# marella/ctransformers

Measured on NVIDIA H100. Metric: decode tokens/s Llama-2-7B Q4_K_M b=1, higher is better.
Workload: dtype int8 (q4_K/q6_K weights x q8_K activations, mma.sync u8 x s8 -> exact int32), fp32 combine in the reference's order

## Files before the change

ctransformers_b200/csrc/device_types.cuh:

```cuda
#pragma once
#include <cstdint>
#include <cuda_fp16.h>
#include <cuda_runtime.h>
#include <utility>

namespace ctb {

enum : int { GT_F32 = 0, GT_F16 = 1, GT_Q4_0 = 2, GT_Q4_1 = 3, GT_Q5_0 = 6, GT_Q5_1 = 7, GT_Q8_0 = 8, GT_Q3_K = 11, GT_Q4_K = 12, GT_Q5_K = 13, GT_Q6_K = 14 };

struct DevMat {
  int type = -1;
  int K = 0, M = 0;
  int nb = 0;
  const uint8_t* qs = nullptr;
  const uint8_t* qh = nullptr;
  const uint16_t* mn = nullptr;
  const uint16_t* d = nullptr;
  const uint8_t* st = nullptr;
  size_t bytes = 0;
};

__host__ __device__ inline bool type_is_kquant(int t) { return t == GT_Q3_K || t == GT_Q4_K || t == GT_Q5_K || t == GT_Q6_K; }
enum : int { ACT_Q8_K = 0, ACT_Q8_0 = 1, ACT_F16 = 2, ACT_F32 = 3, ACT_Q8_1 = 4 };
__host__ __device__ inline int act_format_for(int t) {
  if (type_is_kquant(t)) return ACT_Q8_K;
  if (t == GT_Q4_0 || t == GT_Q5_0 || t == GT_Q8_0) return ACT_Q8_0;
  if (t == GT_Q4_1 || t == GT_Q5_1) return ACT_Q8_1;
  if (t == GT_F16) return ACT_F16;
  return ACT_F32;
}

__device__ __forceinline__ float h2f(uint16_t h) { return __half2float(__ushort_as_half(h)); }
__device__ __forceinline__ uint16_t f2h(float f) { return __half_as_ushort(__float2half_rn(f)); }

__device__ __forceinline__ void pdl_trigger() { asm volatile("griddepcontrol.launch_dependents;"); }
__device__ __forceinline__ void pdl_wait() { asm volatile("griddepcontrol.wait;" ::: "memory"); }

template <typename... KArgs, typename... Args>
static inline cudaError_t launch_kernel(void (*kernel)(KArgs...), dim3 grid, dim3 block, size_t smem, cudaStream_t st, bool pdl, Args&&... args) {
  cudaLaunchConfig_t cfg{};
  cfg.gridDim = grid; cfg.blockDim = block; cfg.dynamicSmemBytes = smem; cfg.stream = st;
  cudaLaunchAttribute at[1];
  at[0].id = cudaLaunchAttributeProgrammaticStreamSerialization;
  at[0].val.programmaticStreamSerializationAllowed = 1;
  cfg.attrs = at; cfg.numAttrs = pdl ? 1 : 0;
  return cudaLaunchKernelEx(&cfg, kernel, std::forward<Args>(args)...);
}

template <typename Kernel>
static inline size_t max_dyn_smem(Kernel kernel) {
  cudaFuncAttributes fa{};
  if (cudaFuncGetAttributes(&fa, kernel) != cudaSuccess) return 0;
  int dev = 0, optin = 0;
  cudaGetDevice(&dev);
  cudaDeviceGetAttribute(&optin, cudaDevAttrMaxSharedMemoryPerBlockOptin, dev);
  return (size_t)optin > fa.sharedSizeBytes ? (size_t)optin - fa.sharedSizeBytes : 0;
}

template <int BAR, int NT>
__device__ __forceinline__ void bar_sync() { asm volatile("bar.sync %0, %1;" ::"n"(BAR), "n"(NT) : "memory"); }

__device__ __forceinline__ unsigned long long globaltimer_ns() {
  unsigned long long t;
  asm volatile("mov.u64 %0, %%globaltimer;" : "=l"(t));
  return t;
}

__device__ __forceinline__ float warp_sum(float v) {
#pragma unroll
  for (int o = 16; o > 0; o >>= 1) v += __shfl_xor_sync(0xffffffffu, v, o);
  return v;
}
__device__ __forceinline__ double warp_sum(double v) {
#pragma unroll
  for (int o = 16; o > 0; o >>= 1) v += __shfl_xor_sync(0xffffffffu, v, o);
  return v;
}
__device__ __forceinline__ float warp_max(float v) {
#pragma unroll
  for (int o = 16; o > 0; o >>= 1) v = fmaxf(v, __shfl_xor_sync(0xffffffffu, v, o));
  return v;
}

__host__ __device__ inline bool attn_head_dim_ok(int hd) { return hd >= 32 && hd <= 256 && hd % 2 == 0; }
__host__ __device__ inline bool attn_fast_hd(int hd) { return hd == 64 || hd == 128; }

}
```

ctransformers_b200/csrc/engine.cu:

```cuda
#include "engine.cuh"

#include <algorithm>
#include <chrono>
#include <cstdio>
#include <cstring>
#include <stdexcept>

#include "attention.cuh"
#include "grammar.hpp"
#include "grammar_gpu.cuh"
#include "matvec.cuh"
#include "prefill.cuh"
#include "repack.cuh"
#include "sample_gpu.cuh"
#include "score_gpu.cuh"
#include "stream.cuh"
#include "tables.hpp"
#include "tp_nccl.hpp"

namespace ctb {

#define CTB_CUDA(expr)                                                                                         \
  do {                                                                                                         \
    cudaError_t e__ = (expr);                                                                                  \
// ... 528 lines not shown
        MVParams p{};
        p.x = attn_; p.norm_mode = NORM_NONE; p.K = qw; p.act = act_format_for(L.wo.type); p.nseg = 1;
        p.seg[0] = (!tp || tp_lead) ? seg(L.wo, y, EPI_ADD, x) : seg(L.wo, y);
        push_matvec(p, MVK_WO);
        if (tp) push_xchg(y);
      }
      {
        MVParams p{};
        p.x = y; p.norm_w = L.ffn_norm; p.norm_mode = NORM_RMS; p.eps = hp_.eps; p.K = n_embd;
        const size_t first_op = ops_.size();
        take_input(p);
        p.act = act_format_for(L.w1.type); p.nseg = 2;
        p.seg[0] = seg(L.w1, ffn_, EPI_SILU); p.seg[1] = seg(L.w3, ffn2_);
        push_matvec(p, MVK_UP);
        mark_exchange(first_op);
      }
      {
        MVParams p{};
        p.x = ffn_; p.x2 = ffn2_; p.x_mode = 1; p.norm_mode = NORM_NONE; p.K = nff_; p.act = act_format_for(L.w2.type); p.nseg = 1;
        p.seg[0] = (!tp || tp_lead) ? seg(L.w2, x, EPI_ADD, y) : seg(L.w2, x);
        push_matvec(p, MVK_DOWN);
        if (tp) push_xchg(x);
      }
    } else {
      const int qkv_w = (hp_.n_head + 2 * n_kv) * hd;
      float* q = qkv_; float* k = qkv_ + (size_t)hp_.n_head * hd; float* v = k + (size_t)n_kv * hd;
      const bool two_norms = L.attn_norm2 != nullptr;
      const bool fuse = !two_norms && act_format_for(L.wqkv.type) == act_format_for(L.w3.type);
      {
        MVParams p{};
        p.x = x; p.norm_mode = NORM_LAYER; p.eps = hp_.eps; p.K = n_embd;
        p.norm_w = two_norms ? L.attn_norm2 : L.attn_norm; p.norm_b = two_norms ? L.attn_norm2_b : L.attn_norm_b;
        p.act = act_format_for(L.wqkv.type); p.nseg = 1;
        p.seg[0] = seg(L.wqkv, qkv_);
        if (fuse) { p.seg[1] = seg(L.w3, ffn_, EPI_GELU); p.nseg = 2; }
        ap.q = q; ap.k = k; ap.v = v; ap.q_stride = qkv_w; ap.kv_stride = qkv_w;
        push_matvec(p, MVK_QKV);
      }
      if (!fuse) {
        MVParams p{};
        p.x = x; p.norm_mode = NORM_LAYER; p.eps = hp_.eps; p.K = n_embd; p.norm_w = L.attn_norm; p.norm_b = L.attn_norm_b;
        p.act = act_format_for(L.w3.type); p.nseg = 1;
        p.seg[0] = seg(L.w3, ffn_, EPI_GELU);
        push_matvec(p, MVK_UP);
      }
      push_attn();
      {
        MVParams p{};
        p.x = attn_; p.norm_mode = NORM_NONE; p.K = n_embd; p.act = act_format_for(L.wo.type); p.nseg = 1;
        p.seg[0] = seg(L.wo, attn_o_);
        push_matvec(p, MVK_WO);
      }
      {
        MVParams p{};
        p.x = ffn_; p.norm_mode = NORM_NONE; p.K = hp_.n_ff; p.act = act_format_for(L.w2.type); p.nseg = 1;
        p.seg[0] = seg(L.w2, y, EPI_ADD2, attn_o_, x);
        push_matvec(p, MVK_DOWN);
      }
      std::swap(x, y);
    }
  }
  n_body_ = (int)ops_.size();
  {
    MVParams p{};
    p.x = x; p.norm_w = out_norm_; p.norm_b = out_norm_b_; p.norm_mode = hp_.falcon ? NORM_LAYER : NORM_RMS; p.eps = hp_.eps; p.K = n_embd;
    const size_t first_op = ops_.size();
    take_input(p);
    p.norm_out = d_embd_; p.act = act_format_for(output_.type); p.nseg = 1;
    p.seg[0] = seg(output_, d_logits_);
    push_matvec(p, MVK_OUT);
    mark_exchange(first_op);

  }
  {
    StepOp op{};
    op.ph.kind = PH_PICK;
    op.ph.pk.logits = d_logits_; op.ph.pk.state = d_state_; op.ph.pk.out_tokens = nullptr; op.ph.pk.n = hp_.n_vocab;
    ops_.push_back(op);
  }
  bool any_stream = false;
  for (const StepOp& op : ops_) any_stream |= op.ph.kind == PH_MATVEC && op.stream;
  std::vector<Phase> phs;
  for (const StepOp& op : ops_) if (op.ph.kind != PH_XCHG && (op.ph.kind != PH_MATVEC || op.stream)) phs.push_back(op.ph);
  const StepLaunch sl = step_launch_shape(phs.data(), (int)phs.size(), sm_count_, max_dyn_smem(k_step<true, false, false>));
  step_grid_ = sl.grid; step_slots_ = sl.n_slots; step_smem_ = sl.smem; step_q3_ = sl.q3;
  if (const char* e = getenv("CTB_ST_SLOTS")) {
    const int want = atoi(e);
    if (want >= ST_W && want < step_slots_ && want % ST_W == 0) { step_smem_ -= (size_t)(step_slots_ - want) * ST_SLOT; step_slots_ = want; }
  }
  ring_attn_ = st_attn_ring_ok(hp_.n_ctx, step_slots_) && !getenv("CTB_NO_RING_ATTN");
  for (StepOp& op : ops_) if (op.ph.kind == PH_ATTN) op.ph.q6 = ring_attn_ ? 1 : 0;
  if (any_stream && step_slots_ < ST_W) throw std::runtime_error("model rows are too long for the step kernel's shared memory");
  if (any_stream) CTB_CUDA(step_set_smem_limit(step_smem_));
  else fused_ = false;
  d_prog_ = (Phase*)alloc((ops_.size() + 1) * sizeof(Phase), 256);
  d_prog_mv_ = (Phase*)alloc((ops_.size() + 1) * sizeof(Phase), 256);
  d_bounds_ = (int*)alloc((ops_.size() + 1) * (size_t)(sm_count_ + 1) * 4, 256);
  d_bounds_mv_ = (int*)alloc((ops_.size() + 1) * (size_t)(sm_count_ + 1) * 4, 256);
}

void Engine::upload_prog(Phase* dst, int* dst_bounds, const std::vector<StepOp>& ops) {
  std::vector<Phase> phs(ops.size());
  for (size_t i = 0; i < ops.size(); i++) phs[i] = ops[i].ph;
  CTB_CUDA(cudaMemcpy(dst, phs.data(), phs.size() * sizeof(Phase), cudaMemcpyHostToDevice));
  std::vector<Phase> run = phs;
  for (size_t i = 0; i < ops.size(); i++) if (ops[i].ph.kind == PH_XCHG || (ops[i].ph.kind == PH_MATVEC && !ops[i].stream)) run[i].kind = -1;
  const std::vector<int> b = step_bounds(run.data(), (int)run.size(), sm_count_);
  CTB_CUDA(cudaMemcpy(dst_bounds, b.data(), b.size() * 4, cudaMemcpyHostToDevice));
}

struct ProfMark {
  Event ev;
  int kind;
};

long Engine::enqueue_ops(const std::vector<StepOp>& ops, const Phase* d_prog, const int* d_bounds, int n, cudaStream_t st, bool fused,
                         std::vector<ProfMark>* marks) {
  long launches = 0;
  auto mark = [&](int kind) {
    if (!marks) return;
    marks->push_back({Event(cudaEventDefault), kind});
    CTB_CUDA(cudaEventRecord(marks->back().ev, st));
  };
  StepLaunch step_shape_;
  step_shape_.grid = step_grid_; step_shape_.n_slots = step_slots_; step_shape_.smem = step_smem_; step_shape_.gen = !attn_fast_hd(hp_.head_dim());
  step_shape_.q3 = step_q3_;
  auto capable = [&](const StepOp& op) { return op.ph.kind != PH_XCHG && (op.ph.kind != PH_MATVEC || op.stream); };
  int i = 0;
  while (i < n) {
    const StepOp& op = ops[i];
    if (fused && capable(op)) {
      int j = i;
      while (j < n && capable(ops[j])) j++;
      mark(-1);
      CTB_CUDA(launch_step(step_shape_, st, d_prog + i, d_bounds + (size_t)i * (sm_count_ + 1), j - i, d_sync_, false, nullptr, tp_peer_));
      launches++;
      mark(0);
      i = j;
      continue;
    }
    mark(-1);
    switch (op.ph.kind) {
      case PH_EMBED:
        k_embed<<<1, 256, 0, st>>>(op.ph.em);
        launches++;
        mark(3);
        break;
      case PH_ATTN:
        CTB_CUDA(launch_kernel(attn_kernel(hp_.head_dim()), dim3(nh_, 1, attn_groups(hp_.head_dim())), dim3(ATTN_THREADS), attn_smem_bytes(hp_.n_ctx, hp_.head_dim()), st, pdl_, op.ph.at));
        launches++;
        mark(1);
        break;
      case PH_XCHG:
        tp_all_reduce(op.ph.em.out, op.ph.em.K, st);
        mark(3);
        break;
      case PH_PICK:
        k_argmax<<<1, ARGMAX_THREADS, 0, st>>>(d_logits_, hp_.n_vocab, d_state_ + 4);
        k_advance<<<1, 1, 0, st>>>(d_state_, d_tokens_out_.as<int>());
        launches += 2;
        mark(3);
        break;
      default:
        if (op.stream) {
          CTB_CUDA(launch_step(step_shape_, st, d_prog + i, d_bounds + (size_t)i * (sm_count_ + 1), 1, d_sync_));
        } else {
          const MVLaunch L = matvec_launch_shape(op.ph.mv, sm_count_);
          CTB_CUDA(launch_matvec_kernel(L, st, op.ph.mv, pdl_));
        }
        launches++;
        mark(0);
    }
    i++;
  }
  CTB_CUDA(cudaGetLastError());
  return launches;
}

int Engine::profile_step(int token, int n_past, double ms_by_kind[4], int count_by_kind[4]) {
  DeviceGuard dev_guard(device_);
  if (tp_.world > 1) throw std::runtime_error("not available in tensor-parallel mode (every rank must run the same launches)");
  drop_lookahead();
  put_step(token, n_past, n_past + 1);
  std::vector<ProfMark> marks;
  enqueue_ops(ops_, d_prog_, d_bounds_, n_body_ + 1, stream_, false, &marks);
  CTB_CUDA(cudaStreamSynchronize(stream_));
  int n = 0;
  for (size_t i = 1; i < marks.size(); i++) {
    float ms = 0;
    cudaEventElapsedTime(&ms, marks[i - 1].ev, marks[i].ev);
    const int k = marks[i].kind;
    if (k >= 0 && k < 4) { ms_by_kind[k] += ms; count_by_kind[k]++; n++; }
  }
  return n;
}

double Engine::time_matvec_only(int reps, long* launches, unsigned mask) {
  if (!mask) mask = ~0u;
  if (tp_.world > 1) throw std::runtime_error("not available in tensor-parallel mode (every rank must run the same launches)");
  drop_lookahead();
  DeviceGuard dev_guard(device_);
  std::vector<StepOp> sel;
  for (int i = 0; i <= n_body_; i++)
    if (ops_[i].ph.kind == PH_MATVEC && ((mask >> ops_[i].mvk) & 1)) sel.push_back(ops_[i]);
  if (sel.empty()) { if (launches) *launches = 0; return 0.0; }
  upload_prog(d_prog_mv_, d_bounds_mv_, sel);
  GraphExec ex;
  {
    const Stream cap(cudaStreamNonBlocking);
    cudaGraph_t g;
    CTB_CUDA(cudaStreamBeginCapture(cap, cudaStreamCaptureModeThreadLocal));
    enqueue_ops(sel, d_prog_mv_, d_bounds_mv_, (int)sel.size(), cap, fused_);
    CTB_CUDA(cudaStreamEndCapture(cap, &g));
    ex = GraphExec(g);
    cudaGraphDestroy(g);
  }
  if (launches) *launches = (long)sel.size();
  const Event e0(cudaEventDefault), e1(cudaEventDefault);
  for (int i = 0; i < 3; i++) CTB_CUDA(cudaGraphLaunch(ex, stream_));
  CTB_CUDA(cudaEventRecord(e0, stream_));
  for (int i = 0; i < reps; i++) CTB_CUDA(cudaGraphLaunch(ex, stream_));
  CTB_CUDA(cudaEventRecord(e1, stream_));
  CTB_CUDA(cudaStreamSynchronize(stream_));
  float ms = 0;
  cudaEventElapsedTime(&ms, e0, e1);
  return (double)ms / reps;
}

long Engine::trace_step(int token, int n_past, unsigned long long* out, long cap_words) {
  DeviceGuard dev_guard(device_);
  if (tp_.world > 1) throw std::runtime_error("not available in tensor-parallel mode (every rank must run the same launches)");
  drop_lookahead();
  const int n = n_body_ + 1;
  for (int i = 0; i < n; i++)
    if (ops_[i].ph.kind == PH_MATVEC && !ops_[i].stream) return 0;
  const long need = 2L * n + 8L * n * step_grid_;
  if (need > cap_words) return -need;
  const DevMem buf((size_t)n * step_grid_ * 64);
  CTB_CUDA(cudaMemset(buf.get(), 0, (size_t)n * step_grid_ * 64));
  StepLaunch L;
  L.grid = step_grid_; L.n_slots = step_slots_; L.smem = step_smem_; L.gen = !attn_fast_hd(hp_.head_dim()); L.q3 = step_q3_;
  for (int rep = 0; rep < 3; rep++) {
    put_step(token, n_past, n_past + 1);
    CTB_CUDA(launch_step(L, stream_, d_prog_, d_bounds_, n, d_sync_, false, buf.as<unsigned long long>()));
    CTB_CUDA(cudaStreamSynchronize(stream_));
  }
  for (int i = 0; i < n; i++) { out[2 * i] = (unsigned long long)ops_[i].ph.kind; out[2 * i + 1] = (unsigned long long)ops_[i].mvk; }
  CTB_CUDA(cudaMemcpy(out + 2 * n, buf.get(), (size_t)n * step_grid_ * 64, cudaMemcpyDeviceToHost));
  return n;
}

void Engine::build_graphs() {
  tokens_out_cap_ = std::max(hp_.n_ctx, 4096);
  d_tokens_out_ = DevMem((size_t)tokens_out_cap_ * 4);
  h_tokens_out_ = HostMem((size_t)tokens_out_cap_ * 4);
  const Stream cap(cudaStreamNonBlocking);
  ops_.back().ph.pk.out_tokens = d_tokens_out_.as<int>();
  upload_prog(d_prog_, d_bounds_, ops_);
  long launches = 0;
  auto capture = [&](bool logits, bool greedy) {
    cudaGraph_t g;
    CTB_CUDA(cudaStreamBeginCapture(cap, cudaStreamCaptureModeThreadLocal));
    launches = enqueue_ops(ops_, d_prog_, d_bounds_, n_body_ + (logits || tp_peer_ ? 1 : 0) + (greedy ? 1 : 0), cap, fused_);
    CTB_CUDA(cudaStreamEndCapture(cap, &g));
    GraphExec ex(g);
    cudaGraphDestroy(g);
    return ex;
  };
  graph_nolog_ = capture(false, false);
  graph_greedy_ = capture(true, true);
  graph_full_ = capture(true, false);
  stats.launches = launches;
}

void Engine::after_eval(int next_pos) {
  spec_pending_ = false;
  spec_deferred_ = false;
  spec_pos_ = -1;
  if (!spec_on_ || next_pos >= hp_.n_ctx || next_pos < kv_high_) return;
  k_argmax<<<1, ARGMAX_THREADS, 0, stream_>>>(d_logits_, hp_.n_vocab, d_state_ + 4);
  k_advance<<<1, 1, 0, stream_>>>(d_state_, d_tokens_out_.as<int>());
  CTB_CUDA(cudaMemcpyAsync(h_spec_tok_.get(), d_state_ + 4, 8, cudaMemcpyDeviceToHost, stream_));
  CTB_CUDA(cudaEventRecord(ev_pick_, stream_));
  spec_pos_ = next_pos;
  if (spec_streak_ >= 2) {
    if (sampler_mode_) spec_deferred_ = true;
    else {
      CTB_CUDA(cudaGraphLaunch(graph_full_, stream_));
      spec_pending_ = true;
    }
  }
}

void Engine::drop_lookahead() { spec_pending_ = false; spec_deferred_ = false; spec_pos_ = -1; spec_streak_ = 0; }

void Engine::launch_deferred_spec() {
  if (!spec_deferred_) return;
  spec_deferred_ = false;
  CTB_CUDA(cudaGraphLaunch(graph_full_, stream_));
  spec_pending_ = true;
}

int Engine::greedy_pick() {
  if (spec_pos_ < 0) return -1;
  DeviceGuard dev_guard(device_);
  CTB_CUDA(cudaEventSynchronize(ev_pick_));
  sampler_mode_ = false;
  launch_deferred_spec();
  const int* pick = h_spec_tok_.as<int>();
  return pick[1] == 1 ? pick[0] : -1;
}

void Engine::put_step(int token, int pos, int n_total) {
  CTB_CUDA(step_ring_.put(stream_, 4, [&](int* st) { st[0] = token; st[1] = pos; st[2] = 0; st[3] = n_total; }));
}

void Engine::decode_one(int token, int pos, int n_total, bool with_logits) {
  put_step(token, pos, n_total);
  CTB_CUDA(cudaGraphLaunch(with_logits ? graph_full_ : graph_nolog_, stream_));
  single_steps_++;
}

int Engine::paths(int* out, int cap) {
  const int v[6] = {fused_ ? 1 : 0, fused_ && ring_attn_ ? 1 : 0, step_slots_, ensure_prefill() ? 1 : 0, (int)prefill_launches_, (int)single_steps_};
// ... 705 lines not shown
```

ctransformers_b200/csrc/engine.cuh:

```cuda
#pragma once
#include <cmath>
#include <memory>
#include <string>
#include <vector>

#include "cuda_owned.cuh"
#include "device_types.cuh"
#include "gguf.hpp"

namespace ctb {

struct TPShard {
  int rank = 0, world = 1;
  int head0 = 0, head1 = 0, kv0 = 0, kv1 = 0, ff0 = 0, ff1 = 0;
  void* comm = nullptr;
};
TPShard tp_shard(int n_embd, int n_head, int n_head_kv, int n_ff, int rank, int world);

struct HParams {
  bool falcon = false;
  int n_vocab = 0, n_ctx_train = 0, n_embd = 0, n_ff = 0, n_head = 0, n_head_kv = 0, n_layer = 0, n_rot = 0;
  float eps = 1e-5f, rope_base = 10000.f, rope_scale = 1.f;
  int n_ctx = 512;
  int n_seq = 1;
  bool multi = false;
  int head_dim() const { return n_embd / n_head; }
  int n_embd_gqa() const { return head_dim() * n_head_kv; }
};

struct LayerW {
  DevMat wq, wk, wv, wqkv, wo, w1, w2, w3;
  const float* attn_norm = nullptr; const float* attn_norm_b = nullptr;
  const float* attn_norm2 = nullptr; const float* attn_norm2_b = nullptr;
  const float* ffn_norm = nullptr;
};

struct Phase;
struct StepOp;
struct ProfMark;
struct MVParams;
struct Uploader;
struct PrefillState;

struct MultiTok { int slot, token, pos, n_total; bool last; };
constexpr int MULTI_LAUNCH_TOKENS = 32;

struct SampleRow { int slot; const int* last; int n_last; float penalty; int k; };

struct Grammar;
struct GrammarState;
struct GrammarRow { int slot; const Grammar* g; const GrammarState* s; const int* last; int n_last; float penalty; int k; };

struct RowSink {
  float* host = nullptr;
  const int* targets = nullptr;
  double* logprob = nullptr;
  int* greedy = nullptr;
};

struct KvCopy { int src, dst, lo, hi; };

struct EvalStats { double last_eval_ms = 0; long launches = 0; size_t weight_bytes_per_token = 0; long spec_hits = 0; double load_ms = 0; size_t load_bytes = 0; };

class Engine {
 public:
  Engine(const GGUFFile& g, const HParams& hp, int device, const TPShard& tp = TPShard());
  ~Engine();
  Engine(const Engine&) = delete;
  Engine& operator=(const Engine&) = delete;

  void eval_list(const int* tokens, const int* pos, const int* n_total, int n, const RowSink* rows = nullptr);
  void score_kept(int target, double* logprob, int* greedy);
  double decode_greedy(int first_token, int n_past, int n_steps, int* out_tokens);
  double time_matvec_only(int reps, long* launches, unsigned mask = 0);
  int profile_step(int token, int n_past, double ms_by_kind[4], int count_by_kind[4]);
  long trace_step(int token, int n_past, unsigned long long* out, long cap_words);
  std::string multi_refusal();
  void multi_eval(const std::vector<MultiTok>& toks, const std::vector<int>& starts, const RowSink* rows = nullptr);
  void multi_fetch(int slot, float* logits, float* embd);
  const struct SampleGpuOut* multi_sample(const SampleRow* rows, int R, int* picks);
  void multi_reset(int slot);
  long multi_launches() const;
  size_t state_bytes(int n_past, bool results) const;
  int state_k_stride() const;
  void state_save(int slot, int n_past, bool results, void* out);
  void state_load(int slot, int n_past, bool results, const void* in, int last_token);
  void state_fork(int src, const int* dsts, int n);
  size_t kv_reparent(const std::vector<KvCopy>& copies);
  const float* multi_rows(int slot0, int n);
  int paths(int* out, int cap);

  float* logits() { host_views(); return h_logits_.as<float>(); }
  float* embeddings() { host_views(); return h_embd_.as<float>(); }
  bool lazy_logits() const { return !eager_; }
  std::vector<float> logits_copy();
  int topk_candidates(const int* last, int n_last, float penalty, int k, int* ids, float* logits);
  int greedy_pick();
  bool has_grammar_pieces() const { return pieces_ready_; }
  void grammar_pieces(const std::vector<int>& off, const std::vector<uint8_t>& bytes);
  const struct SampleGpuOut* grammar_rows(const GrammarRow* rows, int R, int eos, int* stats, unsigned* bits = nullptr);
  std::vector<std::vector<float>> grammar_scratch(const std::vector<int>& rows);
  std::vector<float> slot_logits(int slot);
  const HParams& hparams() const { return hp_; }
  EvalStats stats;
  void set_stream(cudaStream_t s);
  cudaStream_t stream() const { return stream_; }

 private:
  Engine(const HParams& hp, int device, const TPShard& tp);
  HParams hp_;
  TPShard tp_;
  int nh_ = 0, nkv_ = 0, nff_ = 0;
  void tp_all_reduce(float* buf, int n, cudaStream_t st);
  bool tp_peer_ = false;
  uint8_t* xc_region_ = nullptr;
  uint2* xc_ll_[8] = {nullptr};
  void tp_setup_peer();
  int device_ = 0;
  Stream stream_;
  DevMem arena_;
  size_t arena_size_ = 0, arena_used_ = 0;
  void* alloc(size_t bytes, size_t align = 256);

  DevMat output_;
  const uint8_t* tok_embd_ = nullptr; int tok_type_ = 0; size_t tok_row_bytes_ = 0;
  const float* out_norm_ = nullptr; const float* out_norm_b_ = nullptr;
  std::vector<LayerW> layers_;
  uint16_t *silu_tab_ = nullptr, *gelu_tab_ = nullptr, *exp_tab_ = nullptr;
  float2* rope_ = nullptr;
  uint16_t *kc_ = nullptr, *vc_ = nullptr;
  int* d_state_ = nullptr;
  float *xa_ = nullptr, *xb_ = nullptr, *qkv_ = nullptr, *attn_ = nullptr, *attn_o_ = nullptr, *ffn_ = nullptr, *ffn2_ = nullptr, *d_logits_ = nullptr, *d_embd_ = nullptr;
  float *kept_logits_ = nullptr, *kept_embd_ = nullptr;
  int* kept_pick_ = nullptr;
  float* kept_logits(int slot) const { return kept_logits_ + (size_t)slot * hp_.n_vocab; }
  float* kept_embd(int slot) const { return kept_embd_ + (size_t)slot * hp_.n_embd; }
  HostMem h_logits_, h_embd_;
  StateRing step_ring_;
  void put_step(int token, int pos, int n_total);
  HostMem h_tokens_out_;
  DevMem d_tokens_out_;
  int tokens_out_cap_ = 0;

  Event ev0_, ev1_, ev_pick_;
  bool spec_on_ = true, spec_pending_ = false;
  bool spec_deferred_ = false;
  bool sampler_mode_ = false;
  Event ev_sample_;
  void launch_deferred_spec();
  int spec_pos_ = -1, spec_streak_ = 0;
  void drop_lookahead();
  int kv_high_ = 0;
  HostMem h_spec_tok_;
  HostMem h_dbg_;
  void after_eval(int next_pos);
  int sm_count_ = 132;

  void init(const GGUFFile& g);
  DevMat upload_matrix(const GGUFTensor& t, struct Uploader& up, int want_K, int want_M, int row0 = 0, int row1 = -1, int k0 = 0, int k1 = -1);
  const float* upload_vector(const GGUFFile& g, const std::string& name, bool required, int want_n);
  std::vector<StepOp> ops_;
  int n_body_ = 0;
  Phase* d_prog_ = nullptr;
  Phase* d_prog_mv_ = nullptr;
  int *d_bounds_ = nullptr, *d_bounds_mv_ = nullptr;
  unsigned* d_sync_ = nullptr;
  int step_grid_ = 0, step_slots_ = 0;
  size_t step_smem_ = 0;
  bool fused_ = true;
  bool step_q3_ = false;
  bool ring_attn_ = false;
  void build_ops();
  void push_matvec(struct MVParams& p, int kind);
  void upload_prog(Phase* dst, int* dst_bounds, const std::vector<StepOp>& ops);
  long enqueue_ops(const std::vector<StepOp>& ops, const Phase* d_prog, const int* d_bounds, int n, cudaStream_t st, bool fused,
                   std::vector<ProfMark>* marks = nullptr);
  void build_graphs();
  bool eager_ = false;
  bool host_fresh_ = true;
  void host_views();
  DevMem d_sample_;
  HostMem h_sample_;
  void sample_enqueue(const SampleRow* rows, int R, bool picks);
  bool pieces_ready_ = false;
  DevMem d_pieces_, d_gm_, d_gm_rows_;
  HostMem h_gm_;
  std::unique_ptr<PrefillState> pf_;
  bool multi_ready();
  void need_multi();
  bool prefill_on_ = true;
  int prefill_min_ = 4;
  long prefill_launches_ = 0;
  long single_steps_ = 0;
  bool ensure_prefill();
  void prefill_batch(const int* tokens, const int* pos, const int* n_total, int n, bool last, bool rows = false);
  void launch_batch(const MultiTok* toks, int n, bool whole);
  const RowSink* sink_ = nullptr;
  DevMem d_rows_;
  int rows_pending_ = 0, rows_done_ = 0;
  int rows_n_ = 0;
  DevMem d_score_;
  HostMem h_score_;
  int score_cap_ = 0;
  double* d_lp_ = nullptr;
  int *d_tgt_ = nullptr, *d_gr_ = nullptr;
  struct SinkGuard { Engine* e; ~SinkGuard() { e->sink_ = nullptr; } };
  SinkGuard rows_begin(const RowSink* rows, int n);
  void rows_finish();
  void rows_take(const float* src, int m);
  void rows_push(const float* row);
  void rows_drain();
  void rows_end();
  void decode_one(int token, int pos, int n_total, bool with_logits);
  void head_from(const float* row);
  void finish_eval(int next_pos, bool hit);
  enum : int { MVK_QKV = 0, MVK_WO = 1, MVK_UP = 2, MVK_DOWN = 3, MVK_OUT = 4 };
  bool pdl_ = true;
  HostMem h_stage_;
  DevMem d_copies_;
  HostMem h_copies_;
  void kv_slot_elems(size_t& k, size_t& v) const;
  void zero_slot(int slot);
  void copy_results(int src, int dst);
  GraphExec graph_full_, graph_nolog_, graph_greedy_;
};

size_t engine_arena_bytes(const GGUFFile& g, const HParams& hp);

}
```

ctransformers_b200/csrc/llm_abi.cu:

```cuda
#include <algorithm>
#include <atomic>
#include <cctype>
#include <cmath>
#include <chrono>
#include <cstdio>
#include <cstring>
#include <ctime>
#include <memory>
#include <random>
#include <string>
#include <vector>

#include "../../include/ctransformers_b200.h"
#include "beam.hpp"
#include "engine.cuh"
#include "gguf.hpp"
#include "grammar.hpp"
#include "sample_gpu.cuh"
#include "sampler.hpp"
#include "tp_nccl.hpp"
#include "vocab.hpp"

using namespace ctb;

// ... 337 lines not shown
int ctransformers_llm_bos_token_id(LLM* llm) { return llm->vocab.bos; }
int ctransformers_llm_vocab_size(LLM* llm) { return llm->hp.n_vocab; }
int ctransformers_llm_context_length(LLM* llm) { return llm->hp.n_ctx; }
const char* ctransformers_llm_architecture(LLM* llm) { return llm->arch.c_str(); }

bool ctransformers_llm_batch_eval(LLM* llm, const int* tokens, const int n_tokens, const int n_past, const int batch_size, const int threads) {
  (void)threads;
  return llm_eval(llm, tokens, n_tokens, n_past, batch_size, nullptr, "eval") == 0;
}

float* ctransformers_llm_logits_data(LLM* llm) { return llm->engine->logits(); }
int ctransformers_llm_logits_size(LLM* llm) { return llm->has_logits ? llm->hp.n_vocab : 0; }
const float* ctransformers_llm_embeddings_data(LLM* llm) { return llm->engine->embeddings(); }
int ctransformers_llm_embeddings_size(LLM* llm) { return llm->has_logits ? llm->hp.n_embd : 0; }

int ctransformers_llm_sample(LLM* llm, const int* last_tokens, const int n_last, const int top_k, const float top_p, const float temperature,
                             const float repetition_penalty, int seed) {
  try {
    if (seed < 0) seed = (int)time(nullptr);
    llm->rng.seed((unsigned)seed);
    if (llm->engine->lazy_logits()) {
      Engine& e = *llm->engine;
      bool used_device = false;
      const int t = sample_lazy(
          llm->hp.n_vocab, last_tokens, n_last, top_k, top_p, temperature, repetition_penalty, llm->rng, used_device, [&] { return e.greedy_pick(); },
          [&](const int* last, int nl, float pen, int k, int* ids, float* lg) { return e.topk_candidates(last, nl, pen, k, ids, lg); },
          [&] { return e.logits_copy(); });
      if (used_device) llm->gpu_samples++;
      return t;
    }
    return sample_token(llm->engine->logits(), llm->hp.n_vocab, last_tokens, n_last, top_k, top_p, temperature, repetition_penalty, llm->rng);
  } catch (...) { return llm->vocab.eos; }
}

void ctransformers_llm_reset(LLM* llm) { (void)llm;  }

int ctb_abi_version(void) { return 1; }

double ctb_llm_last_eval_ms(LLM* llm) { return llm->engine->stats.last_eval_ms; }
long ctb_llm_launches_per_token(LLM* llm) { return llm->engine->stats.launches; }
long ctb_llm_speculative_hits(LLM* llm) { return llm->engine->stats.spec_hits; }
unsigned long long ctb_llm_weight_bytes_per_token(LLM* llm) { return (unsigned long long)llm->engine->stats.weight_bytes_per_token; }
long ctb_llm_device_samples(LLM* llm) { return llm->gpu_samples; }
double ctb_llm_load_ms(LLM* llm) { return llm->engine->stats.load_ms; }
void ctb_llm_set_stream(LLM* llm, void* cuda_stream) { llm->engine->set_stream((cudaStream_t)cuda_stream); }

double ctb_llm_decode_greedy(LLM* llm, int first_token, int n_past, int n_steps, int* out_tokens) {
  try {
    const double ms = llm->engine->decode_greedy(first_token, n_past, n_steps, out_tokens);
    llm->has_logits = true;
    return ms;
  } catch (const std::exception& e) {
    fprintf(stderr, "ctransformers-b200: decode_greedy failed: %s\n", e.what());
    return -1.0;
  }
}

int ctb_llm_profile_step(LLM* llm, int token, int n_past, double* ms_by_kind, int* count_by_kind) {
  try {
    return llm->engine->profile_step(token, n_past, ms_by_kind, count_by_kind);
  } catch (const std::exception& e) {
    fprintf(stderr, "ctransformers-b200: profile_step failed: %s\n", e.what());
    return -1;
  }
}

long ctb_llm_trace_step(LLM* llm, int token, int n_past, unsigned long long* out, long cap_words) {
  try {
    return llm->engine->trace_step(token, n_past, out, cap_words);
  } catch (const std::exception& e) {
    fprintf(stderr, "ctransformers-b200: trace_step failed: %s\n", e.what());
    return 0;
  }
}

long ctb_llm_paths(LLM* llm, int* out, int cap) {
  try {
    return llm->engine->paths(out, cap);
  } catch (const std::exception& e) {
    fprintf(stderr, "ctransformers-b200: paths failed: %s\n", e.what());
    return -100;
  }
}

double ctb_llm_time_matvec_only(LLM* llm, int reps, long* launches) { return ctb_llm_time_matvec_kinds(llm, reps, launches, 0); }

double ctb_llm_time_matvec_kinds(LLM* llm, int reps, long* launches, unsigned kind_mask) {
  try {
    return llm->engine->time_matvec_only(reps < 1 ? 1 : reps, launches, kind_mask);
  } catch (const std::exception& e) {
    fprintf(stderr, "ctransformers-b200: time_matvec_only failed: %s\n", e.what());
    return -1.0;
  }
}

int ctb_state_info(const void* buf, size_t size, ctb_state_header* out) {
  ctb_state_header s;
  const std::string why = state_check(buf, size, s);
  if (!why.empty()) {
    fprintf(stderr, "ctransformers-b200: %s\n", why.c_str());
    return -1;
  }
  if (out) *out = s;
  return 0;
}

size_t ctb_llm_state_size(LLM* llm, int n_tokens) {
  try {
    not_sharded(llm, "has no sequence states");
    return state_size_for(*llm, n_tokens);
  } catch (...) { return 0; }
}

int ctb_llm_save_state(LLM* llm, const int* tokens, int n_tokens, void* buf, size_t cap) {
  try {
    not_sharded(llm, "has no sequence states");
    save_state(*llm, 0, tokens, n_tokens, llm->has_logits, buf, cap);
    return 0;
  } catch (const std::exception& e) { return state_error("cannot save the state", e); }
}

int ctb_llm_load_state(LLM* llm, const void* buf, size_t size) {
  try {
    not_sharded(llm, "has no sequence states");
    llm->has_logits = restore_state(*llm, 0, buf, size).has_results != 0;
    return 0;
  } catch (const std::exception& e) { return state_error("cannot load the state", e); }
}

int ctb_llm_batch_eval_rows(LLM* llm, const int* tokens, int n_tokens, int n_past, int batch_size, float* rows) {
  RowSink s;
  s.host = rows;
  return llm_eval(llm, tokens, n_tokens, n_past, batch_size, &s, "eval with rows");
}

int ctb_llm_batch_eval_scored(LLM* llm, const int* tokens, int n_tokens, int n_past, int batch_size, const int* targets, double* logprob, int* greedy) {
  RowSink s;
  s.targets = targets; s.logprob = logprob; s.greedy = greedy;
  if (n_tokens > 0 && (!logprob || !greedy)) {
    fprintf(stderr, "ctransformers-b200: scored eval failed: no memory for the scores\n");
    return -1;
  }
  return llm_eval(llm, tokens, n_tokens, n_past, batch_size, &s, "scored eval");
}

int ctb_llm_score_last(LLM* llm, int target, double* logprob, int* greedy) {
  try {
    not_sharded(llm, "keeps no per-token rows");
    if (!llm->has_logits) throw std::invalid_argument("nothing has been evaluated");
    check_targets(&target, 1, llm->hp.n_vocab);
    llm->engine->score_kept(target, logprob, greedy);
    return 0;
  } catch (const std::exception& e) {
    fprintf(stderr, "ctransformers-b200: scoring the last logits failed: %s\n", e.what());
    return -1;
  } catch (...) { return -1; }
}

struct ctb_vocab { std::unique_ptr<GGUFFile> file; Vocab vocab; };

ctb_vocab* ctb_vocab_load(const char* gguf_path) {
  try {
    std::unique_ptr<ctb_vocab> v(new ctb_vocab);
    v->file.reset(new GGUFFile(gguf_path));
    v->vocab.load(*v->file);
    return v.release();
// ... 825 lines not shown
```

ctransformers_b200/csrc/matvec.cuh:

```cuda
#pragma once
#include "device_types.cuh"
#include "attention.cuh"

namespace ctb {

#ifndef CTB_THREADS
#define CTB_THREADS 512
#endif
constexpr int MV_THREADS = CTB_THREADS;
constexpr int MV_WARPS = MV_THREADS / 32;
constexpr int MV_ROWS = 4;
constexpr int MV_MAX_SEG = 3;

enum : int { NORM_NONE = 0, NORM_RMS = 1, NORM_LAYER = 2 };
enum : int { EPI_STORE = 0, EPI_ADD = 1, EPI_GELU = 2, EPI_ADD2 = 3, EPI_SILU = 4 };

#ifndef ST_WATCHDOG_NS
#define ST_WATCHDOG_NS 4000000000ull
#endif
#ifndef XC_WATCHDOG_NS
#define XC_WATCHDOG_NS 30000000000ull
#endif
enum WaitCode : int {
  W_GRID_BARRIER = 1, W_FOLD_FLAG, W_FREE_WEIGHT_SLOT, W_WEIGHT_ITEM, W_FREE_K_SLOT, W_FREE_V_SLOT, W_K_ITEM, W_V_ITEM, W_XCHG,
  W_PF_GRID_BARRIER, W_PF_FREE_SLOT, W_PF_WEIGHT_ITEM, W_CODES
};
constexpr const char* WAIT_TEXT[] = {"?", "grid barrier (aux = phase)", "fold hand-off flag (aux = chunk)", "producer: free weight slot (aux = item)",
                                     "consumer: weight item (aux = item)", "producer: free K slot (attention)", "producer: free V slot (attention)",
                                     "consumer: K item (attention)", "consumer: V item (attention)", "tensor-parallel exchange: a peer's element (aux = exchange number)",
                                     "prefill grid barrier (aux = phase)", "prefill producer: free slot (aux = item)", "prefill consumer: weight item (aux = item)"};
static_assert(sizeof(WAIT_TEXT) / sizeof(WAIT_TEXT[0]) == W_CODES, "one text per wait code");

static __device__ int* g_st_dbg = nullptr;
static __device__ __noinline__ void st_fail(WaitCode code, int aux) {
  int* d = g_st_dbg;
  if (d) { d[0] = code; d[1] = (int)blockIdx.x; d[2] = aux; d[3] = (int)threadIdx.x; __threadfence_system(); }
  __trap();
}
template <typename Done>
__device__ __forceinline__ void bounded_wait(Done&& done, WaitCode code, int aux, unsigned long long limit_ns = ST_WATCHDOG_NS) {
  if (done()) return;
  const unsigned long long t0 = globaltimer_ns();
  while (!done())
    if (globaltimer_ns() - t0 > limit_ns) st_fail(code, aux);
}

struct MVSeg {
  DevMat w;
  float* out;
  const float* res;
  const float* res2;
  int epi;
};

struct MVParams {
  const float* x;
  const float* x2;
  int x_mode;
  int x_parts, x_stride;
  float* sum_out;
  const float* norm_w;
  const float* norm_b;
  float* norm_out;
  float eps;
  int norm_mode;
  int K;
  int act;
  int nseg;
  MVSeg seg[MV_MAX_SEG];
  const uint16_t* silu_tab;
  const uint16_t* gelu_tab;
};

struct ActView {
  const int8_t* qs;
  const float* d;
  const int16_t* bs;
};

__host__ __device__ inline size_t act_smem_bytes(int act, int K) {
  switch (act) {
    case ACT_Q8_K: return (size_t)K + (((size_t)(K / 256) * 4 + 15) & ~(size_t)15) + (size_t)(K / 16) * 2 + 16;
    case ACT_Q8_0: return (size_t)K + (size_t)(K / 32) * 4 + 16;
    case ACT_Q8_1: return (size_t)K + (size_t)(K / 32) * 8 + 16;
    case ACT_F16: return (size_t)K * 2;
    default: return (size_t)K * 4;
  }
}

__host__ __device__ inline size_t q8k_d_bytes(int K) { return ((size_t)(K / 256) * 4 + 15) & ~(size_t)15; }

__device__ __forceinline__ ActView act_view(int act, int K, uint8_t* smem) {
  ActView a;
  a.qs = (const int8_t*)smem;
  const size_t off = ((size_t)K + 15) & ~(size_t)15;
  a.d = (const float*)(smem + off);
  a.bs = (const int16_t*)(smem + off + q8k_d_bytes(K));
  return a;
}

__device__ __forceinline__ int q8k_word_offset(int b, int s, int l) { return ((b * 2 + (s >> 2)) * 8 + l) * 16 + (s & 3) * 4; }


template <bool CG = false>
__device__ __forceinline__ void load16(const float* p, int valid, float (&v)[16]) {
  if (valid >= 16) {
    float4 a, b, c, d;
    if (CG) { a = __ldcg((const float4*)p); b = __ldcg((const float4*)p + 1); c = __ldcg((const float4*)p + 2); d = __ldcg((const float4*)p + 3); }
    else { a = __ldg((const float4*)p); b = __ldg((const float4*)p + 1); c = __ldg((const float4*)p + 2); d = __ldg((const float4*)p + 3); }
    v[0] = a.x; v[1] = a.y; v[2] = a.z; v[3] = a.w; v[4] = b.x; v[5] = b.y; v[6] = b.z; v[7] = b.w;
    v[8] = c.x; v[9] = c.y; v[10] = c.z; v[11] = c.w; v[12] = d.x; v[13] = d.y; v[14] = d.z; v[15] = d.w;
  } else {
#pragma unroll
    for (int e = 0; e < 16; e++) v[e] = e < valid ? (CG ? __ldcg(p + e) : __ldg(p + e)) : 0.f;
  }
}

template <int NT, int BAR>
__device__ __forceinline__ double block_sum_f64(double s, double* red ) {
  s = warp_sum(s);
  bar_sync<BAR, NT>();
  if ((threadIdx.x & 31) == 0) red[threadIdx.x >> 5] = s;
  bar_sync<BAR, NT>();
  double t = 0.0;
#pragma unroll
  for (int w = 0; w < NT / 32; w++) t += red[w];
  return t;
}
template <int NT, int BAR>
__device__ __forceinline__ void block_sum2_max_f64(double& s, double& a, double& g, double* red) {
  constexpr int NW = NT / 32;
#pragma unroll
  for (int o = 16; o > 0; o >>= 1) {
    s += __shfl_xor_sync(0xffffffffu, s, o);
    a += __shfl_xor_sync(0xffffffffu, a, o);
    g = fmax(g, __shfl_xor_sync(0xffffffffu, g, o));
  }
  bar_sync<BAR, NT>();
  if ((threadIdx.x & 31) == 0) { red[threadIdx.x >> 5] = s; red[NW + (threadIdx.x >> 5)] = a; red[2 * NW + (threadIdx.x >> 5)] = g; }
  bar_sync<BAR, NT>();
  s = 0.0;
  a = 0.0;
#pragma unroll
  for (int w = 0; w < NW; w++) { s += red[w]; a += red[NW + w]; g = fmax(g, red[2 * NW + w]); }
}

__device__ __forceinline__ uint32_t pack4(const int* q) {
  return (uint32_t)(q[0] & 0xff) | ((uint32_t)(q[1] & 0xff) << 8) | ((uint32_t)(q[2] & 0xff) << 16) | ((uint32_t)(q[3] & 0xff) << 24);
}

__device__ __forceinline__ void load16_ll(const uint2* p, unsigned epoch, float (&u)[16]) {
  uint4 q[8];
  bounded_wait([&] {
    bool ok = true;
#pragma unroll
    for (int j = 0; j < 8; j++) {
      asm volatile("ld.volatile.global.v4.u32 {%0,%1,%2,%3}, [%4];" : "=r"(q[j].x), "=r"(q[j].y), "=r"(q[j].z), "=r"(q[j].w) : "l"(p + 2 * j) : "memory");
    }
#pragma unroll
    for (int j = 0; j < 8; j++) ok &= q[j].y == epoch && q[j].w == epoch;
    return ok;
  }, W_XCHG, (int)epoch, XC_WATCHDOG_NS);
#pragma unroll
  for (int j = 0; j < 8; j++) { u[2 * j] = __uint_as_float(q[j].x); u[2 * j + 1] = __uint_as_float(q[j].z); }
}

template <bool XC = false>
__device__ __forceinline__ void load16x(const MVParams& xs, int base, int valid, float (&v)[16], unsigned epoch = 0) {
  if (XC && xs.x_mode == 2) {
    if (valid <= 0) {
#pragma unroll
      for (int e = 0; e < 16; e++) v[e] = 0.f;
      return;
    }
    const uint2* ll = (const uint2*)xs.x + (size_t)(epoch & 1u) * xs.x_parts * xs.x_stride;
    load16_ll(ll + base, epoch, v);
    for (int r = 1; r < xs.x_parts; r++) {
      float u[16];
      load16_ll(ll + (size_t)r * xs.x_stride + base, epoch, u);
#pragma unroll
      for (int e = 0; e < 16; e++) v[e] = __fadd_rn(v[e], u[e]);
    }
    return;
  }
  load16<true>(xs.x + base, valid, v);
  if (xs.x_mode == 1) {
    float u[16];
    load16<true>(xs.x2 + base, valid, u);
#pragma unroll
    for (int e = 0; e < 16; e++) v[e] = __fmul_rn(v[e], u[e]);
  }
}

struct NormPre { float w0[16], bias0[16]; };
__device__ __forceinline__ void preload_norm(NormPre& np, const MVParams& p) {
  const int t = threadIdx.x;
  if (p.norm_mode != NORM_NONE && p.norm_w) load16(p.norm_w + t * 16, p.K - t * 16, np.w0);
  if (p.norm_mode != NORM_NONE && p.norm_b) load16(p.norm_b + t * 16, p.K - t * 16, np.bias0);
}

__device__ __forceinline__ unsigned min_exp(unsigned emin, float t) {
  const unsigned bits = __float_as_uint(t) & 0x7fffffffu;
  return bits ? min(emin, max(bits >> 23, 1u)) : emin;
}
__device__ __forceinline__ double lsb_inv(unsigned emin) { return ldexp(1.0, 150 - (int)emin); }

enum : int { NORM_TERM_SQ = 0, NORM_TERM_X = 1, NORM_TERM_DEV = 2 };
template <bool XC>
static __device__ __noinline__ double seq_sum_warp0(const float* x, const float* x2, int x_mode, int x_parts, int x_stride, int K, int kind,
                                                    float mean, unsigned epoch) {
  MVParams xs;
  xs.x = x; xs.x2 = x2; xs.x_mode = x_mode; xs.x_parts = x_parts; xs.x_stride = x_stride;
  const int lane = threadIdx.x & 31;
  double seq = 0.0;
  for (int base = 0; base < K; base += 512) {
    float v[16];
    load16x<XC>(xs, base + lane * 16, K - base - lane * 16, v, epoch);
    for (int l = 0; l < 32; l++)
#pragma unroll
      for (int i = 0; i < 16; i++) {
        float t = __shfl_sync(0xffffffffu, v[i], l);
        if (kind == NORM_TERM_DEV) t = __fsub_rn(t, mean);
        if (base + l * 16 + i < K) seq += kind == NORM_TERM_X ? (double)t : (double)__fmul_rn(t, t);
      }
  }
  return seq;
}

template <int NT, int BAR, bool XC>
__device__ __forceinline__ float norm_stat(double s, double a, double g, bool a_is_s, int kind, float mean, const MVParams& xs, double* red,
                                           unsigned epoch) {
  const int K = xs.K;
  if (a_is_s) a = s = block_sum_f64<NT, BAR>(s, red);
  else block_sum2_max_f64<NT, BAR>(s, a, g, red);
  if (!isfinite(s) || (!a_is_s && __dmul_ru(a, g) < 0x1p52)) return (float)(s / (double)K);
  const double e = __dmul_ru(a, (double)K * 0x1.0000001p-52);
  const float lo = (float)(__dsub_rd(s, e) / (double)K), hi = (float)(__dadd_ru(s, e) / (double)K);
  if (lo == hi) return lo;
  const double seq = threadIdx.x < 32 ? seq_sum_warp0<XC>(xs.x, xs.x2, xs.x_mode, xs.x_parts, xs.x_stride, K, kind, mean, epoch) : 0.0;
  bar_sync<BAR, NT>();
  if (threadIdx.x == 0) red[0] = seq;
  bar_sync<BAR, NT>();
  return (float)(red[0] / (double)K);
}

template <int NT, int BAR, bool XC = false>
__device__ __forceinline__ void stage_activation(const MVParams& xs, const NormPre& np, int act, uint8_t* smem, double* red, bool write_norm, unsigned epoch = 0) {
  const float* nw = xs.norm_w;
  const float* nb_ = xs.norm_b;
  float* norm_out = xs.norm_out;
  const int norm_mode = xs.norm_mode, K = xs.K;
  const float eps = xs.eps;
  const int t = threadIdx.x, lane = t & 31;
  const int passes = (K + NT * 16 - 1) / (NT * 16);
  float mean = 0.f, scale = 1.f;
  float v0[16];
  load16x<XC>(xs, t * 16, K - t * 16, v0, epoch);
  if (norm_mode == NORM_RMS) {
    double ss = 0.0;
    for (int ps = 0; ps < passes; ps++) {
      const int base = (ps * NT + t) * 16;
      if ((base & ~511) >= K) continue;
      float v[16];
      if (ps == 0) {
#pragma unroll
        for (int e = 0; e < 16; e++) v[e] = v0[e];
      } else load16x<XC>(xs, base, K - base, v, epoch);
#pragma unroll
      for (int e = 0; e < 16; e++) ss += (double)__fmul_rn(v[e], v[e]);
    }
    const float m = norm_stat<NT, BAR, XC>(ss, ss, 0.0, true, NORM_TERM_SQ, 0.f, xs, red, epoch);
    scale = __fdiv_rn(1.0f, __fsqrt_rn(__fadd_rn(m, eps)));
  } else if (norm_mode == NORM_LAYER) {
    double s1 = 0.0, a1 = 0.0;
    unsigned emin = 255;
    for (int ps = 0; ps < passes; ps++) {
      const int base = (ps * NT + t) * 16;
      if ((base & ~511) >= K) continue;
      float v[16];
      load16x<XC>(xs, base, K - base, v, epoch);
#pragma unroll
      for (int e = 0; e < 16; e++) {
        s1 += (double)v[e];
        a1 += (double)fabsf(v[e]);
        emin = min_exp(emin, v[e]);
      }
    }
    mean = norm_stat<NT, BAR, XC>(s1, a1, lsb_inv(emin), false, NORM_TERM_X, 0.f, xs, red, epoch);
    double s2 = 0.0;
    for (int ps = 0; ps < passes; ps++) {
      const int base = (ps * NT + t) * 16;
      if ((base & ~511) >= K) continue;
      float v[16];
      load16x<XC>(xs, base, K - base, v, epoch);
#pragma unroll
      for (int e = 0; e < 16; e++) { const float d = (base + e < K) ? __fsub_rn(v[e], mean) : 0.f; s2 += (double)__fmul_rn(d, d); }
    }
    const float var = norm_stat<NT, BAR, XC>(s2, s2, 0.0, true, NORM_TERM_DEV, mean, xs, red, epoch);
    scale = __fdiv_rn(1.0f, __fsqrt_rn(__fadd_rn(var, eps)));
  }
  int8_t* qs = (int8_t*)smem;
  const size_t off = ((size_t)K + 15) & ~(size_t)15;
  float* dd = (float*)(smem + off);
  int16_t* bs = (int16_t*)(smem + off + q8k_d_bytes(K));
  for (int ps = 0; ps < passes; ps++) {
    const int base = (ps * NT + t) * 16;
    const int valid = K - base;
    if ((base & ~511) >= K) continue;
    float v[16];
    if (ps == 0) {
#pragma unroll
      for (int e = 0; e < 16; e++) v[e] = v0[e];
    } else load16x<XC>(xs, base, valid, v, epoch);
    if (XC && write_norm && xs.x_mode == 2 && xs.sum_out && valid > 0) {
#pragma unroll
      for (int e = 0; e < 16; e++) if (e < valid) xs.sum_out[base + e] = v[e];
    }
    if (norm_mode != NORM_NONE) {
      float w[16], bb[16];
      if (ps == 0) {
#pragma unroll
        for (int e = 0; e < 16; e++) { w[e] = np.w0[e]; bb[e] = np.bias0[e]; }
      } else {
        if (nw) load16(nw + base, valid, w);
        if (nb_) load16(nb_ + base, valid, bb);
      }
#pragma unroll
      for (int e = 0; e < 16; e++) {
        float y = v[e];
        if (norm_mode == NORM_LAYER) y = __fsub_rn(y, mean);
        y = __fmul_rn(y, scale);
        if (nw) y = __fmul_rn(y, w[e]);
        if (nb_) y = __fadd_rn(y, bb[e]);
        v[e] = y;
      }
    }
    if (write_norm && norm_out && valid > 0) {
#pragma unroll
      for (int e = 0; e < 16; e++) if (e < valid) norm_out[base + e] = v[e];
    }
    if (act == ACT_Q8_K) {
      float amax = 0.f, mx = 0.f;
#pragma unroll
      for (int e = 0; e < 16; e++) { const float ax = fabsf(v[e]); if (ax > amax) { amax = ax; mx = v[e]; } }
      float gmax = amax;
#pragma unroll
      for (int o = 8; o > 0; o >>= 1) gmax = fmaxf(gmax, __shfl_xor_sync(0xffffffffu, gmax, o));
      const unsigned who = __ballot_sync(0xffffffffu, amax == gmax);
      const int hbase = lane & 16, hl = lane & 15;
      const unsigned mine = (who >> hbase) & 0xffffu;
      const float maxv = __shfl_sync(0xffffffffu, mx, hbase + __ffs(mine) - 1);
      if (valid > 0) {
        const int b = base >> 8;
        int q[16];
        int sum = 0;
        if (gmax == 0.f) {
#pragma unroll
          for (int e = 0; e < 16; e++) q[e] = 0;
          if (hl == 0) dd[b] = 0.f;
        } else {
          const float iscale = __fdiv_rn(-128.f, maxv);
#pragma unroll
          for (int e = 0; e < 16; e++) {
            const float val = __fmaf_rn(iscale, v[e], 12582912.f);
            q[e] = min(127, (__float_as_int(val) & 0x007fffff) - 0x00400000);
            sum += q[e];
          }
          if (hl == 0) dd[b] = __fdiv_rn(1.f, iscale);
        }
        bs[b * 16 + hl] = (int16_t)sum;
#pragma unroll
        for (int j = 0; j < 4; j++) {
          const int wi = hl * 4 + j;
          *(uint32_t*)(qs + q8k_word_offset(b, wi >> 3, wi & 7)) = pack4(q + 4 * j);
        }
      }
    } else if (act == ACT_Q8_0) {
      float amax = 0.f;
#pragma unroll
      for (int e = 0; e < 16; e++) amax = fmaxf(amax, fabsf(v[e]));
      amax = fmaxf(amax, __shfl_xor_sync(0xffffffffu, amax, 1));
      if (valid > 0) {
        const float d = __fdiv_rn(amax, 127.f);
        const float id = amax != 0.f ? __fdiv_rn(127.f, amax) : 0.f;
        int q[16];
#pragma unroll
        for (int e = 0; e < 16; e++) q[e] = __float2int_rn(__fmul_rn(v[e], id));
        *(uint4*)(qs + base) = make_uint4(pack4(q), pack4(q + 4), pack4(q + 8), pack4(q + 12));
        if ((lane & 1) == 0) dd[base >> 5] = h2f(f2h(d));
      }
    } else if (act == ACT_Q8_1) {
      float amax = 0.f;
#pragma unroll
      for (int e = 0; e < 16; e++) amax = fmaxf(amax, fabsf(v[e]));
      amax = fmaxf(amax, __shfl_xor_sync(0xffffffffu, amax, 1));
      const float d = __fdiv_rn(amax, 127.f);
      const float id = amax != 0.f ? __fdiv_rn(127.f, amax) : 0.f;
      int q[16];
      int sum = 0;
#pragma unroll
      for (int e = 0; e < 16; e++) { q[e] = __float2int_rn(__fmul_rn(v[e], id)); sum += q[e]; }
      sum += __shfl_xor_sync(0xffffffffu, sum, 1);
      if (valid > 0) {
        *(uint4*)(qs + base) = make_uint4(pack4(q), pack4(q + 4), pack4(q + 8), pack4(q + 12));
        if ((lane & 1) == 0) *(float2*)(dd + (base >> 4)) = make_float2(d, __fmul_rn(d, (float)sum));
      }
    } else if (act == ACT_F16) {
      uint16_t* h = (uint16_t*)smem;
#pragma unroll
      for (int e = 0; e < 16; e++) if (e < valid) h[base + e] = f2h(v[e]);
    } else {
      float* f = (float*)smem;
#pragma unroll
      for (int e = 0; e < 16; e++) if (e < valid) f[base + e] = v[e];
    }
  }
  bar_sync<BAR, NT>();
}

__device__ __forceinline__ float group_hsum8(float v) {
  v = v + __shfl_xor_sync(0xffffffffu, v, 4);
  v = v + __shfl_xor_sync(0xffffffffu, v, 2);
  v = v + __shfl_xor_sync(0xffffffffu, v, 1);
  return v;
}

__device__ __forceinline__ float dot_q40(const DevMat& w, int row, const ActView& a, int l) {
  const int nb = w.nb;
  const uint8_t* qrow = w.qs + (size_t)row * nb * 16 + (l & 3) * 4;
  const uint16_t* drow = w.d + (size_t)row * nb;
  const int shift = (l >> 2) * 4;
  float acc = 0.f;
#pragma unroll 8
  for (int b = 0; b < nb; b++) {
    const uint32_t q = (uint32_t)__ldg((const int*)(qrow + (size_t)b * 16));
    const float dw = h2f(__ldg(drow + b));
    const int aw = *(const int*)(a.qs + b * 32 + l * 4);
    const float yd = a.d[b];
    const uint32_t nib = (q >> shift) & 0x0f0f0f0fu;
    const uint32_t bx = ((nib | 0x80808080u) - 0x08080808u) ^ 0x80808080u;
    acc = __fmaf_rn(__fmul_rn(dw, yd), (float)__dp4a((int)bx, aw, 0), acc);
  }
  return group_hsum8(acc);
}

__device__ __forceinline__ float dot_q50(const DevMat& w, int row, const ActView& a, int l) {
  const int nb = w.nb;
  const uint8_t* qrow = w.qs + (size_t)row * nb * 16 + (l & 3) * 4;
  const uint32_t* hrow = (const uint32_t*)w.qh + (size_t)row * nb;
  const uint16_t* drow = w.d + (size_t)row * nb;
  const int shift = (l >> 2) * 4;
  float acc = 0.f;
#pragma unroll 8
  for (int b = 0; b < nb; b++) {
    const uint32_t q = (uint32_t)__ldg((const int*)(qrow + (size_t)b * 16));
    const uint32_t h4 = (__ldg(hrow + b) >> (4 * l)) & 0xfu;
    const float dw = h2f(__ldg(drow + b));
    const int aw = *(const int*)(a.qs + b * 32 + l * 4);
    const float yd = a.d[b];
    const uint32_t nib = (q >> shift) & 0x0f0f0f0fu;
    const uint32_t set = (h4 * 0x00204081u) & 0x01010101u;
    const uint32_t bx = nib | ((set ^ 0x01010101u) * 0xf0u);
    acc = __fmaf_rn(__fmul_rn(dw, yd), (float)__dp4a((int)bx, aw, 0), acc);
  }
  return group_hsum8(acc);
}

__device__ __forceinline__ float dot_q80(const DevMat& w, int row, const ActView& a, int l) {
  const int nb = w.nb;
  const uint8_t* qrow = w.qs + (size_t)row * nb * 32 + l * 4;
  const uint16_t* drow = w.d + (size_t)row * nb;
  float acc = 0.f;
#pragma unroll 8
  for (int b = 0; b < nb; b++) {
    const int q = __ldg((const int*)(qrow + (size_t)b * 32));
    const float dw = h2f(__ldg(drow + b));
    const int aw = *(const int*)(a.qs + b * 32 + l * 4);
    acc = __fmaf_rn(__fmul_rn(dw, a.d[b]), (float)__dp4a(q, aw, 0), acc);
  }
  return group_hsum8(acc);
}

template <bool Q5>
__device__ __forceinline__ float dot_q1(const DevMat& w, int row, const ActView& a, int l) {
  const int nb = w.nb;
  const uint8_t* qrow = w.qs + (size_t)row * nb * 16 + (l & 3) * 4;
  const uint32_t* hrow = (const uint32_t*)w.qh + (size_t)row * nb;
  const uint16_t* drow = w.d + (size_t)row * nb;
  const uint16_t* mrow = w.mn + (size_t)row * nb;
  const int shift = (l >> 2) * 4;
  float acc = 0.f, summs = 0.f;
#pragma unroll 8
  for (int b = 0; b < nb; b++) {
    const uint32_t q = (uint32_t)__ldg((const int*)(qrow + (size_t)b * 16));
    const float dw = h2f(__ldg(drow + b));
    const float mw = h2f(__ldg(mrow + b));
    const int aw = *(const int*)(a.qs + b * 32 + l * 4);
    const float2 ds = *(const float2*)(a.d + 2 * b);
    uint32_t bx = (q >> shift) & 0x0f0f0f0fu;
    if (Q5) bx |= ((((__ldg(hrow + b) >> (4 * l)) & 0xfu) * 0x00204081u) & 0x01010101u) << 4;
// ... 111 lines not shown
```

ctransformers_b200/csrc/ops_abi.cu:

```cuda
#include <cmath>
#include <cstdio>
#include <cstring>
#include <ctime>
#include <functional>
#include <stdexcept>
#include <string>
#include <vector>

#include "../../include/ctransformers_b200.h"
#include "attention.cuh"
#include "cuda_owned.cuh"
#include "matvec.cuh"
#include "prefill.cuh"
#include "repack.cuh"
#include "sample_gpu.cuh"
#include "sampler.hpp"
#include "score_gpu.cuh"
#include "stream.cuh"
#include "tables.hpp"

using namespace ctb;

namespace {

#define OPS_CUDA(expr)                                                                                     \
  do {                                                                                                     \
    cudaError_t e__ = (expr);                                                                              \
    if (e__ != cudaSuccess) throw std::runtime_error(std::string("CUDA error: ") + cudaGetErrorString(e__) + " (" #expr ")"); \
  } while (0)

struct OpsTables {
  uint16_t *silu = nullptr, *gelu = nullptr, *ex = nullptr;
};

OpsTables& tables() {
  static OpsTables t;
  if (!t.silu) {
    const HostTables h = host_tables();
    OPS_CUDA(cudaMalloc(&t.silu, 65536 * 2)); OPS_CUDA(cudaMalloc(&t.gelu, 65536 * 2)); OPS_CUDA(cudaMalloc(&t.ex, 65536 * 2));
    OPS_CUDA(cudaMemcpy(t.silu, h.silu.data(), 65536 * 2, cudaMemcpyHostToDevice));
    OPS_CUDA(cudaMemcpy(t.gelu, h.gelu.data(), 65536 * 2, cudaMemcpyHostToDevice));
    OPS_CUDA(cudaMemcpy(t.ex, h.ex.data(), 65536 * 2, cudaMemcpyHostToDevice));
  }
  return t;
}

size_t raw_row_bytes(int type, int K) {
  switch (type) {
    case GT_F32: return (size_t)K * 4; case GT_F16: return (size_t)K * 2;
    case GT_Q4_0: return (size_t)K / 32 * 18; case GT_Q5_0: return (size_t)K / 32 * 22; case GT_Q8_0: return (size_t)K / 32 * 34;
    case GT_Q4_1: return (size_t)K / 32 * 20; case GT_Q5_1: return (size_t)K / 32 * 24;
    case GT_Q3_K: return (size_t)K / 256 * 110;
    case GT_Q4_K: return (size_t)K / 256 * 144; case GT_Q5_K: return (size_t)K / 256 * 176; case GT_Q6_K: return (size_t)K / 256 * 210;
  }
  throw std::runtime_error("unsupported ggml type " + std::to_string(type));
}
int block_elems(int type) {
  if (type_is_kquant(type)) return 256;
  return (type == GT_Q4_0 || type == GT_Q5_0 || type == GT_Q8_0 || type == GT_Q4_1 || type == GT_Q5_1) ? 32 : 1;
}

DevMat upload(std::vector<DevMem>& keep, int type, const void* blocks, int K, int M) {
  if (K % block_elems(type)) throw std::runtime_error("K is not a multiple of the block size");
  const size_t bytes = raw_row_bytes(type, K) * M;
  DevMem raw(bytes);
  OPS_CUDA(cudaMemcpy(raw.get(), blocks, bytes, cudaMemcpyHostToDevice));
  DevMat m;
  m.type = type; m.K = K; m.M = M; m.nb = K / block_elems(type); m.bytes = bytes;
  if (type_is_kquant(type)) {
    const size_t sb = st_matrix_bytes(type, M, m.nb);
    keep.emplace_back(sb);
    uint16_t* st = keep.back().as<uint16_t>();
    k_repack_stream<<<(int)std::min<size_t>((sb / 2 + 255) / 256, 4096), 256>>>(type, raw.as<uint8_t>(), M, m.nb, st);
    OPS_CUDA(cudaDeviceSynchronize());
    m.st = (const uint8_t*)st;
    return m;
  }
  const PlaneSizes ps = plane_sizes(type, M, m.nb, bytes);
  uint16_t* pl[4] = {nullptr, nullptr, nullptr, nullptr};
  const size_t sz[4] = {ps.qs, ps.qh, ps.d, ps.mn};
  for (int i = 0; i < 4; i++)
    if (sz[i]) { keep.emplace_back(sz[i]); pl[i] = keep.back().as<uint16_t>(); }
  k_repack<<<(int)std::min<size_t>((bytes / 2 + 255) / 256, 4096), 256>>>(type, raw.as<uint16_t>(), bytes / 2, pl[0], pl[1], pl[2], pl[3]);
  OPS_CUDA(cudaDeviceSynchronize());
  m.qs = (const uint8_t*)pl[0]; m.qh = (const uint8_t*)pl[1]; m.d = pl[2]; m.mn = pl[3];
  return m;
}

int sm_count() {
  int n_sm = 132;
  cudaDeviceGetAttribute(&n_sm, cudaDevAttrMultiProcessorCount, 0);
  return n_sm;
}

unsigned* sync_words() {
  static unsigned* d_sync = nullptr;
  if (!d_sync) { OPS_CUDA(cudaMalloc((void**)&d_sync, 64)); OPS_CUDA(cudaMemset(d_sync, 0, 64)); }
  return d_sync;
}

void run_phases(std::vector<Phase> phs) {
  unsigned* d_sync = sync_words();
  const StepLaunch L = step_launch_shape(phs.data(), (int)phs.size(), sm_count(), max_dyn_smem(k_step<true, false, false>));
  const std::vector<int> hb = step_bounds(phs.data(), (int)phs.size(), L.grid);
  DevMem dbounds(hb.size() * 4);
  OPS_CUDA(cudaMemcpy(dbounds.get(), hb.data(), hb.size() * 4, cudaMemcpyHostToDevice));
  if (L.n_slots < ST_W) throw std::runtime_error("rows too long for the step kernel's shared memory");
  OPS_CUDA(step_set_smem_limit(L.smem));
  DevMem dprog((phs.size() + 1) * sizeof(Phase));
  OPS_CUDA(cudaMemcpy(dprog.get(), phs.data(), phs.size() * sizeof(Phase), cudaMemcpyHostToDevice));
  OPS_CUDA(launch_step(L, 0, dprog.as<Phase>(), dbounds.as<int>(), (int)phs.size(), d_sync));
  OPS_CUDA(cudaGetLastError());
  OPS_CUDA(cudaDeviceSynchronize());
}

void run_matvec(MVParams& p) {
  p.silu_tab = tables().silu;
  p.gelu_tab = tables().gelu;
  if (step_supports(p)) {
    run_phases({matvec_phase(p)});
    return;
  }
  static bool attr = false;
  if (!attr) {
    OPS_CUDA(matvec_set_smem_limit(MV_SMEM_LIMIT));
    attr = true;
  }
  const MVLaunch L = matvec_launch_shape(p, sm_count());
  OPS_CUDA(launch_matvec_kernel(L, 0, p));
  OPS_CUDA(cudaGetLastError());
}

__global__ void __launch_bounds__(MV_THREADS) k_stage_dump(const __grid_constant__ MVParams q, int act, uint8_t* dump) {
  extern __shared__ __align__(16) uint8_t smem[];
  __shared__ double red[3 * MV_WARPS];
  NormPre np;
  preload_norm(np, q);
  stage_activation<MV_THREADS, 0>(q, np, act, smem, red, true);
  const size_t n = act_smem_bytes(act, q.K);
  for (size_t i = threadIdx.x; i < n; i += MV_THREADS) dump[i] = smem[i];
}

__global__ void __launch_bounds__(MV_THREADS) k_gate_dump(const __grid_constant__ MVParams q, float* out) {
  extern __shared__ __align__(16) uint8_t smem[];
  __shared__ double red[3 * MV_WARPS];
  NormPre np;
  preload_norm(np, q);
  stage_activation<MV_THREADS, 0>(q, np, ACT_F32, smem, red, false);
  const float* f = (const float*)smem;
  for (int i = threadIdx.x; i < q.K; i += MV_THREADS) out[i] = f[i];
}

__global__ void k_rope_dump(float* x, const float2* rope, int pos, int hd, int neox) {
  float* row = x + (size_t)blockIdx.x * hd;
  int i0, i1;
  float o0, o1;
  rope_head_pair(row, threadIdx.x, hd, neox, rope[(size_t)pos * (hd / 2) + threadIdx.x], i0, i1, o0, o1);
  row[i0] = o0; row[i1] = o1;
}

int guarded(const char* what, const std::function<void()>& fn) {
  try {
    int ndev = 0;
    if (cudaGetDeviceCount(&ndev) != cudaSuccess || ndev == 0) throw std::runtime_error("no CUDA device available (no CPU fallback)");
    fn();
    return 0;
  } catch (const std::exception& e) {
    fprintf(stderr, "ctransformers-b200: %s failed: %s\n", what, e.what());
    return -1;
  }
}

void stage_to_host(const float* x, const float* w, const float* b, float* y_norm, int mode, float eps, int K, int act, std::vector<uint8_t>& dump) {
  DevMem dx((size_t)K * 4), dw((size_t)K * 4), db((size_t)K * 4), dy((size_t)K * 4);
  OPS_CUDA(cudaMemcpy(dx.get(), x, (size_t)K * 4, cudaMemcpyHostToDevice));
  if (w) OPS_CUDA(cudaMemcpy(dw.get(), w, (size_t)K * 4, cudaMemcpyHostToDevice));
  if (b) OPS_CUDA(cudaMemcpy(db.get(), b, (size_t)K * 4, cudaMemcpyHostToDevice));
  const size_t n = act_smem_bytes(act, K);
  DevMem dd(n);
  if (n > 48 * 1024) OPS_CUDA(cudaFuncSetAttribute(k_stage_dump, cudaFuncAttributeMaxDynamicSharedMemorySize, (int)n));
  MVParams q{};
  q.x = dx.as<float>(); q.norm_w = w ? dw.as<float>() : nullptr; q.norm_b = b ? db.as<float>() : nullptr; q.norm_out = dy.as<float>();
  q.norm_mode = mode; q.eps = eps; q.K = K;
  k_stage_dump<<<1, MV_THREADS, n>>>(q, act, dd.as<uint8_t>());
  OPS_CUDA(cudaGetLastError());
  dump.resize(n);
  OPS_CUDA(cudaMemcpy(dump.data(), dd.get(), n, cudaMemcpyDeviceToHost));
  if (y_norm) OPS_CUDA(cudaMemcpy(y_norm, dy.get(), (size_t)K * 4, cudaMemcpyDeviceToHost));
}

void kv_to_device(const uint16_t* kref, const uint16_t* vref, int v_ld, int n_pos, int n_kv, int hd, int n_ctx, std::vector<uint16_t>& kp,
// ... 79 lines not shown
  return guarded("ctb_quantize_row_q8_K", [&] {
    if (k % 256) throw std::runtime_error("k must be a multiple of 256");
    std::vector<uint8_t> dump;
    stage_to_host(x, nullptr, nullptr, nullptr, NORM_NONE, 0.f, k, ACT_Q8_K, dump);
    const int nb = k / 256;
    const size_t off = ((size_t)k + 15) & ~(size_t)15;
    const float* d = (const float*)(dump.data() + off);
    const int16_t* bs = (const int16_t*)(dump.data() + off + q8k_d_bytes(k));
    uint8_t* out = (uint8_t*)y;
    for (int b = 0; b < nb; b++) {
      memcpy(out + (size_t)b * 292, d + b, 4);
      for (int e = 0; e < 256; e++) {
        const int wd = e >> 2, sb = wd >> 3, ln = wd & 7;
        out[(size_t)b * 292 + 4 + e] = dump[(size_t)((b * 2 + (sb >> 2)) * 8 + ln) * 16 + (sb & 3) * 4 + (e & 3)];
      }
      memcpy(out + (size_t)b * 292 + 260, bs + (size_t)b * 16, 32);
    }
  });
}

int ctb_quantize_row_q8_0(const float* x, void* y, int k) {
  return guarded("ctb_quantize_row_q8_0", [&] {
    if (k % 32) throw std::runtime_error("k must be a multiple of 32");
    std::vector<uint8_t> dump;
    stage_to_host(x, nullptr, nullptr, nullptr, NORM_NONE, 0.f, k, ACT_Q8_0, dump);
    const int nb = k / 32;
    const size_t off = ((size_t)k + 15) & ~(size_t)15;
    const float* d = (const float*)(dump.data() + off);
    uint8_t* out = (uint8_t*)y;
    for (int b = 0; b < nb; b++) {
      const uint16_t h = __half_as_ushort(__float2half_rn(d[b]));
      memcpy(out + (size_t)b * 34, &h, 2);
      memcpy(out + (size_t)b * 34 + 2, dump.data() + (size_t)b * 32, 32);
    }
  });
}

int ctb_quantize_row_q8_1(const float* x, void* y, int k) {
  return guarded("ctb_quantize_row_q8_1", [&] {
    if (k % 32) throw std::runtime_error("k must be a multiple of 32");
    std::vector<uint8_t> dump;
    stage_to_host(x, nullptr, nullptr, nullptr, NORM_NONE, 0.f, k, ACT_Q8_1, dump);
    const size_t off = ((size_t)k + 15) & ~(size_t)15;
    uint8_t* out = (uint8_t*)y;
    for (int b = 0; b < k / 32; b++) {
      memcpy(out + (size_t)b * 40, dump.data() + off + (size_t)b * 8, 8);
      memcpy(out + (size_t)b * 40 + 8, dump.data() + (size_t)b * 32, 32);
    }
  });
}

int ctb_norm(int mode, const float* x, const float* w, const float* b, float* y, int n, float eps) {
  return guarded("ctb_norm", [&] {
    std::vector<uint8_t> dump;
    stage_to_host(x, w, b, y, mode, eps, n, ACT_F32, dump);
  });
}

int ctb_norm_path(int path, int mode, const float* x, const float* w, const float* b, float* y, int n, float eps) {
  return guarded("ctb_norm_path", [&] {
    if (path < 0 || path > 1) throw std::runtime_error("unknown norm path " + std::to_string(path));
    if (mode != NORM_RMS && mode != NORM_LAYER) throw std::runtime_error("norm mode 1 or 2");
    if (path == 0) {
      std::vector<uint8_t> dump;
      stage_to_host(x, w, b, y, mode, eps, n, ACT_F32, dump);
      return;
    }
    if (n < 256 || n % 256) throw std::runtime_error("the step kernel takes n a positive multiple of 256");
    const std::vector<uint8_t> zeros(raw_row_bytes(GT_Q4_K, n) * 16, 0);
    std::vector<DevMem> keep;
    const DevMat wm = upload(keep, GT_Q4_K, zeros.data(), n, 16);
    DevMem dx((size_t)n * 4), dw((size_t)n * 4), db((size_t)n * 4), dy((size_t)n * 4), dout(16 * 4);
    OPS_CUDA(cudaMemcpy(dx.get(), x, (size_t)n * 4, cudaMemcpyHostToDevice));
    if (w) OPS_CUDA(cudaMemcpy(dw.get(), w, (size_t)n * 4, cudaMemcpyHostToDevice));
    if (b) OPS_CUDA(cudaMemcpy(db.get(), b, (size_t)n * 4, cudaMemcpyHostToDevice));
    MVParams p{};
    p.x = dx.as<float>(); p.norm_w = w ? dw.as<float>() : nullptr; p.norm_b = b && mode == NORM_LAYER ? db.as<float>() : nullptr;
    p.norm_out = dy.as<float>(); p.norm_mode = mode; p.eps = eps; p.K = n; p.act = ACT_Q8_K; p.nseg = 1;
    p.seg[0].w = wm; p.seg[0].out = dout.as<float>(); p.seg[0].epi = EPI_STORE;
    p.silu_tab = tables().silu; p.gelu_tab = tables().gelu;
    run_phases({matvec_phase(p)});
    OPS_CUDA(cudaMemcpy(y, dy.get(), (size_t)n * 4, cudaMemcpyDeviceToHost));
  });
}

int ctb_rope(float* x, int n_heads, int head_dim, int pos, int mode, float freq_base, float freq_scale) {
  return guarded("ctb_rope", [&] {
    const int half = head_dim / 2;
    const std::vector<float2> tab = rope_table(pos + 1, head_dim, head_dim, freq_base, freq_scale);
    const size_t nq = (size_t)n_heads * head_dim;
    DevMem dq(nq * 4), dtab(tab.size() * 8);
    OPS_CUDA(cudaMemcpy(dq.get(), x, nq * 4, cudaMemcpyHostToDevice));
    OPS_CUDA(cudaMemcpy(dtab.get(), tab.data(), tab.size() * 8, cudaMemcpyHostToDevice));
    k_rope_dump<<<n_heads, half>>>(dq.as<float>(), dtab.as<float2>(), pos, head_dim, (mode & 2) ? 1 : 0);
    OPS_CUDA(cudaGetLastError());
    OPS_CUDA(cudaMemcpy(x, dq.get(), nq * 4, cudaMemcpyDeviceToHost));
  });
}

int ctb_attention(const float* q, const uint16_t* kcache, const uint16_t* vcache, float* out, int n_head, int n_kv, int head_dim, int T,
                  int n_total, float kq_scale) {
  return guarded("ctb_attention", [&] {
    if (!attn_head_dim_ok(head_dim)) throw std::runtime_error("head_dim must be even, from 32 to 256");
    if (n_total < T) n_total = T;
    const size_t nq = (size_t)n_head * head_dim;
    std::vector<uint16_t> kp, vp;
    kv_to_device(kcache, vcache, T, T, n_kv, head_dim, n_total, kp, vp);
    const int pos = T - 1;
    std::vector<float> kcur((size_t)n_kv * head_dim), vcur((size_t)n_kv * head_dim);
    for (int kh = 0; kh < n_kv; kh++)
      for (int e = 0; e < head_dim; e++) {
        kcur[(size_t)kh * head_dim + e] = __half2float(__ushort_as_half(kcache[((size_t)pos * n_kv + kh) * head_dim + e]));
        vcur[(size_t)kh * head_dim + e] = __half2float(__ushort_as_half(vcache[((size_t)kh * head_dim + e) * T + pos]));
      }
    std::vector<float2> ident((size_t)n_total * (head_dim / 2), make_float2(1.f, 0.f));
    DevMem dq(nq * 4), dk(kp.size() * 2), dv(vp.size() * 2), dout(nq * 4), dst(16), dkc(kcur.size() * 4), dvc(vcur.size() * 4), dtab(ident.size() * 8);
    OPS_CUDA(cudaMemcpy(dq.get(), q, nq * 4, cudaMemcpyHostToDevice));
    OPS_CUDA(cudaMemcpy(dk.get(), kp.data(), kp.size() * 2, cudaMemcpyHostToDevice));
    OPS_CUDA(cudaMemcpy(dv.get(), vp.data(), vp.size() * 2, cudaMemcpyHostToDevice));
    OPS_CUDA(cudaMemcpy(dkc.get(), kcur.data(), kcur.size() * 4, cudaMemcpyHostToDevice));
    OPS_CUDA(cudaMemcpy(dvc.get(), vcur.data(), vcur.size() * 4, cudaMemcpyHostToDevice));
    OPS_CUDA(cudaMemcpy(dtab.get(), ident.data(), ident.size() * 8, cudaMemcpyHostToDevice));
    const int st[4] = {0, pos, 0, n_total};
    OPS_CUDA(cudaMemcpy(dst.get(), st, 16, cudaMemcpyHostToDevice));
    AttnParams ap{};
    ap.q = dq.as<float>(); ap.k = dkc.as<float>(); ap.v = dvc.as<float>(); ap.kc = dk.as<uint16_t>(); ap.vc = dv.as<uint16_t>();
    ap.out = dout.as<float>(); ap.exp_tab = tables().ex; ap.rope = dtab.as<float2>(); ap.state = dst.as<int>(); ap.kq_scale = kq_scale;
    ap.n_head = n_head; ap.n_kv = n_kv; ap.hd = head_dim; ap.n_ctx = n_total; ap.q_stride = (int)nq; ap.kv_stride = n_kv * head_dim; ap.neox = 0;
    const size_t smem = attn_smem_bytes(n_total, head_dim);
    OPS_CUDA(cudaFuncSetAttribute(attn_kernel(head_dim), cudaFuncAttributeMaxDynamicSharedMemorySize, (int)std::max<size_t>(smem, 48 * 1024)));
    attn_kernel(head_dim)<<<dim3(n_head, 1, attn_groups(head_dim)), ATTN_THREADS, smem>>>(ap);
    OPS_CUDA(cudaGetLastError());
    OPS_CUDA(cudaMemcpy(out, dout.get(), nq * 4, cudaMemcpyDeviceToHost));
  });
}

int ctb_attention_path(int path, const float* q, const float* k_new, const float* v_new, uint16_t* kcache, uint16_t* vcache, float* out,
                       int n_head, int n_kv, int head_dim, int n_ctx, int pos0, int n_tok, const int* n_total, int rope_mode, float freq_base,
                       float kq_scale) {
  return guarded("ctb_attention_path", [&] {
    const int hd = head_dim;
    if (path < 0 || path > 3) throw std::runtime_error("unknown attention path " + std::to_string(path));
    if (!attn_head_dim_ok(hd)) throw std::runtime_error("head_dim must be even, from 32 to 256");
    if (n_head < 1 || n_kv < 1 || n_head % n_kv) throw std::runtime_error("n_head must be a multiple of n_kv");
    if (n_tok < 1 || pos0 < 0 || pos0 + n_tok > n_ctx) throw std::runtime_error("the tokens' positions must lie inside the context");
    for (int i = 0; i < n_tok; i++)
      if (n_total[i] <= pos0 + i || n_total[i] > n_ctx) throw std::runtime_error("n_total[i] must lie in [position + 1, n_ctx]");
    const size_t nq = (size_t)n_head * hd, nkv = (size_t)n_kv * hd;
    std::vector<uint16_t> kp, vp;
    kv_to_device(kcache, vcache, n_ctx, n_ctx, n_kv, hd, n_ctx, kp, vp);
    const std::vector<float2> tab = rope_table(n_ctx, hd, hd, freq_base, 1.0f);
    std::vector<int> st((size_t)std::max(n_tok, PB_T) * 4 + 4, 0);
    for (int i = 0; i < std::max(n_tok, PB_T); i++) {
      const int k = std::min(i, n_tok - 1);
      st[(size_t)i * 4 + 1] = pos0 + k; st[(size_t)i * 4 + 3] = n_total[k];
    }
    if (path == 3) st[(size_t)PB_T * 4] = n_tok;
    DevMem dq(nq * n_tok * 4), dk(nkv * n_tok * 4), dv(nkv * n_tok * 4), dkc(kp.size() * 2), dvc(vp.size() * 2), dout(nq * n_tok * 4),
        dtab(tab.size() * 8), dst(st.size() * 4);
    OPS_CUDA(cudaMemcpy(dq.get(), q, nq * n_tok * 4, cudaMemcpyHostToDevice));
    OPS_CUDA(cudaMemcpy(dk.get(), k_new, nkv * n_tok * 4, cudaMemcpyHostToDevice));
    OPS_CUDA(cudaMemcpy(dv.get(), v_new, nkv * n_tok * 4, cudaMemcpyHostToDevice));
    OPS_CUDA(cudaMemcpy(dkc.get(), kp.data(), kp.size() * 2, cudaMemcpyHostToDevice));
    OPS_CUDA(cudaMemcpy(dvc.get(), vp.data(), vp.size() * 2, cudaMemcpyHostToDevice));
    OPS_CUDA(cudaMemcpy(dtab.get(), tab.data(), tab.size() * 8, cudaMemcpyHostToDevice));
    OPS_CUDA(cudaMemcpy(dst.get(), st.data(), st.size() * 4, cudaMemcpyHostToDevice));
    OPS_CUDA(cudaMemset(dout.get(), 0, nq * n_tok * 4));
    AttnParams ap{};
    ap.q = dq.as<float>(); ap.k = dk.as<float>(); ap.v = dv.as<float>(); ap.kc = dkc.as<uint16_t>(); ap.vc = dvc.as<uint16_t>();
    ap.out = dout.as<float>(); ap.exp_tab = tables().ex; ap.rope = dtab.as<float2>(); ap.state = dst.as<int>(); ap.kq_scale = kq_scale;
    ap.n_head = n_head; ap.n_kv = n_kv; ap.hd = hd; ap.n_ctx = n_ctx; ap.q_stride = (int)nq; ap.kv_stride = (int)nkv; ap.neox = (rope_mode & 2) ? 1 : 0;
    if (path == 3) {
      if (n_tok > PB_T) throw std::runtime_error("the batched kernel takes at most 32 tokens");
      int n_slots = 0;
      size_t smem = 0;
      if (!pstep_shape(pb_work_bytes((int)nq, n_ctx, hd), n_slots, smem)) throw std::runtime_error("n_ctx too long for the batched kernel's attention scratch");
      PPhase ph{};
      ph.at = ap; ph.state = dst.as<int>();
      PPhase prog[2] = {ph, ph};
      prog[0].kind = PP_KV; prog[1].kind = PP_ATTN;
      DevMem dprog(sizeof(prog));
      OPS_CUDA(cudaMemcpy(dprog.get(), prog, sizeof(prog), cudaMemcpyHostToDevice));
      OPS_CUDA(pstep_set_smem_limit(smem));
      OPS_CUDA(launch_pstep(sm_count(), n_slots, smem, 0, dprog.as<PPhase>(), 2, sync_words()));
    } else {
      if (path == 1) {
        Phase ph{};
        ph.kind = PH_ATTN; ph.q6 = 1; ph.at = ap;
        const StepLaunch L = step_launch_shape(&ph, 1, sm_count(), max_dyn_smem(k_step<true, false, false>));
        if (!st_attn_ring_ok(n_ctx, L.n_slots)) throw std::runtime_error("the step kernel's ring cannot carry K / V at this n_ctx");
      }
      const size_t smem = attn_smem_bytes(n_ctx, hd);
      if (path == 0) OPS_CUDA(cudaFuncSetAttribute(attn_kernel(hd), cudaFuncAttributeMaxDynamicSharedMemorySize, (int)std::max<size_t>(smem, 48 * 1024)));
      for (int i = 0; i < n_tok; i++) {
        AttnParams a = ap;
        a.q += (size_t)i * nq; a.k += (size_t)i * nkv; a.v += (size_t)i * nkv; a.out += (size_t)i * nq; a.state += (size_t)i * 4;
        if (path == 0) {
          attn_kernel(hd)<<<dim3(n_head, 1, attn_groups(hd)), ATTN_THREADS, smem>>>(a);
          OPS_CUDA(cudaGetLastError());
        } else {
          Phase ph{};
          ph.kind = PH_ATTN; ph.q6 = path == 1 ? 1 : 0; ph.at = a;
          run_phases({ph});
        }
      }
    }
    OPS_CUDA(cudaDeviceSynchronize());
    OPS_CUDA(cudaMemcpy(out, dout.get(), nq * n_tok * 4, cudaMemcpyDeviceToHost));
    OPS_CUDA(cudaMemcpy(kp.data(), dkc.get(), kp.size() * 2, cudaMemcpyDeviceToHost));
    OPS_CUDA(cudaMemcpy(vp.data(), dvc.get(), vp.size() * 2, cudaMemcpyDeviceToHost));
    kv_from_device(kp, vp, n_kv, hd, n_ctx, kcache, vcache);
  });
}

int ctb_prefill_mul_mat(int nseg, const int* types, const void* const* w_blocks, const int* rows, int K, int n_tok, const float* x,
                        const float* x2, int norm_mode, const float* norm_w, const float* norm_b, float eps, const int* epi,
                        const float* res, const float* res2, float* out, int n_ctx, int head_dim, int* n_slots) {
  return guarded("ctb_prefill_mul_mat", [&] {
    if (nseg < 1 || nseg > MV_MAX_SEG) throw std::runtime_error("1 to 3 segments");
    if (K < 256 || K % 256) throw std::runtime_error("K must be a positive multiple of 256");
    if (n_tok < 1) throw std::runtime_error("n_tok must be at least 1");
    if (norm_mode < NORM_NONE || norm_mode > NORM_LAYER || (x2 && norm_mode != NORM_NONE)) throw std::runtime_error("norm mode 0, 1 or 2, and 0 with x2");
    if ((norm_mode != NORM_NONE && !norm_w) || (norm_mode == NORM_LAYER && !norm_b)) throw std::runtime_error("RMSNorm needs norm_w, LayerNorm norm_w and norm_b");
    if (norm_mode == NORM_NONE) norm_w = nullptr;
    if (norm_mode != NORM_LAYER) norm_b = nullptr;
    if (!attn_head_dim_ok(head_dim)) throw std::runtime_error("head_dim must be even, from 32 to 256");
    if (n_ctx < 1) throw std::runtime_error("n_ctx must be at least 1");
    int off[MV_MAX_SEG + 1] = {0};
    for (int s = 0; s < nseg; s++) {
      if (!type_is_kquant(types[s])) throw std::runtime_error("the batched kernel takes K-quant weights only");
      if (rows[s] < 1) throw std::runtime_error("every segment needs at least one row");
      if (epi[s] < EPI_STORE || epi[s] > EPI_SILU) throw std::runtime_error("unknown epilogue");
      if ((epi[s] == EPI_ADD || epi[s] == EPI_ADD2) && !res) throw std::runtime_error("ADD / ADD2 need res");
      if (epi[s] == EPI_ADD2 && !res2) throw std::runtime_error("ADD2 needs res2");
      off[s + 1] = off[s] + rows[s];
    }
    const int W = off[nseg];
    int slots = 0;
    size_t smem = 0;
    if (!pstep_shape(pb_work_bytes(K, n_ctx, head_dim), slots, smem)) throw std::runtime_error("no batched prefill at this n_ctx: its attention scratch does not fit");
    std::vector<DevMem> keep;
    DevMat mats[MV_MAX_SEG];
    for (int s = 0; s < nseg; s++) mats[s] = upload(keep, types[s], w_blocks[s], K, rows[s]);
    DevMem dx((size_t)PB_T * K * 4), dx2((size_t)PB_T * K * 4), dout((size_t)PB_T * W * 4), dres((size_t)PB_T * W * 4), dres2((size_t)PB_T * W * 4),
        dnw((size_t)K * 4), dnb((size_t)K * 4), dq(pb_qbuf_bytes(K)), dst((PB_T * 4 + 4) * 4);
    OPS_CUDA(cudaMemset(dq.get(), 0, pb_qbuf_bytes(K)));
    OPS_CUDA(cudaMemset(dout.get(), 0, (size_t)PB_T * W * 4));
    if (norm_w) OPS_CUDA(cudaMemcpy(dnw.get(), norm_w, (size_t)K * 4, cudaMemcpyHostToDevice));
    if (norm_b) OPS_CUDA(cudaMemcpy(dnb.get(), norm_b, (size_t)K * 4, cudaMemcpyHostToDevice));
    MVParams m{};
    m.x = dx.as<float>(); m.x2 = x2 ? dx2.as<float>() : nullptr; m.x_mode = x2 ? 1 : 0;
    m.norm_w = norm_w ? dnw.as<float>() : nullptr; m.norm_b = norm_b ? dnb.as<float>() : nullptr; m.norm_mode = norm_mode; m.eps = eps;
    m.K = K; m.act = ACT_Q8_K; m.nseg = nseg; m.silu_tab = tables().silu; m.gelu_tab = tables().gelu;
    for (int s = 0; s < nseg; s++) {
      m.seg[s].w = mats[s]; m.seg[s].out = dout.as<float>() + off[s]; m.seg[s].epi = epi[s];
      if (epi[s] == EPI_ADD || epi[s] == EPI_ADD2) m.seg[s].res = dres.as<float>() + off[s];
      if (epi[s] == EPI_ADD2) m.seg[s].res2 = dres2.as<float>() + off[s];
    }
    struct Rows { const float* p; int ld; };
    const Rows bufs[5] = {{dx.as<float>(), K}, {dx2.as<float>(), K}, {dout.as<float>(), W}, {dres.as<float>(), W}, {dres2.as<float>(), W}};
    auto bat = [&](const float* p, int& ld) -> float* {
      ld = 0;
      if (!p) return nullptr;
      for (const Rows& b : bufs)
        if (p >= b.p && p < b.p + (size_t)PB_T * b.ld) { ld = b.ld; return const_cast<float*>(p); }
      throw std::runtime_error("pointer outside the token buffers");
    };
    std::vector<PPhase> prog;
    pb_matvec_phases(m, dq.as<uint8_t>(), dst.as<int>(), bat, prog);
    DevMem dprog((prog.size() + 1) * sizeof(PPhase));
    OPS_CUDA(cudaMemcpy(dprog.get(), prog.data(), prog.size() * sizeof(PPhase), cudaMemcpyHostToDevice));
    OPS_CUDA(pstep_set_smem_limit(smem));
    for (int b = 0; b < n_tok; b += PB_T) {
      const int n = std::min(PB_T, n_tok - b);
      std::vector<int> st(PB_T * 4 + 4, 0);
      for (int i = 0; i < PB_T; i++) {
        const int k = std::min(i, n - 1);
        st[i * 4 + 1] = b + k; st[i * 4 + 3] = b + k + 1;
      }
      st[PB_T * 4] = n;
      OPS_CUDA(cudaMemcpy(dst.get(), st.data(), st.size() * 4, cudaMemcpyHostToDevice));
      OPS_CUDA(cudaMemcpy(dx.get(), x + (size_t)b * K, (size_t)n * K * 4, cudaMemcpyHostToDevice));
      if (x2) OPS_CUDA(cudaMemcpy(dx2.get(), x2 + (size_t)b * K, (size_t)n * K * 4, cudaMemcpyHostToDevice));
      if (res) OPS_CUDA(cudaMemcpy(dres.get(), res + (size_t)b * W, (size_t)n * W * 4, cudaMemcpyHostToDevice));
      if (res2) OPS_CUDA(cudaMemcpy(dres2.get(), res2 + (size_t)b * W, (size_t)n * W * 4, cudaMemcpyHostToDevice));
      OPS_CUDA(launch_pstep(sm_count(), slots, smem, 0, dprog.as<PPhase>(), (int)prog.size(), sync_words(), pstep_q3(prog)));
      OPS_CUDA(cudaDeviceSynchronize());
      OPS_CUDA(cudaMemcpy(out + (size_t)b * W, dout.get(), (size_t)n * W * 4, cudaMemcpyDeviceToHost));
    }
    if (n_slots) *n_slots = slots;
  });
}

int ctb_ffn_gate(int type, const void* w1_blocks, const void* w3_blocks, const float* x, float* out, int K, int M) {
  return guarded("ctb_ffn_gate", [&] {
    std::vector<DevMem> keep;
    const DevMat w1 = upload(keep, type, w1_blocks, K, M), w3 = upload(keep, type, w3_blocks, K, M);
    DevMem dx((size_t)K * 4), dg((size_t)M * 4), du((size_t)M * 4), dy((size_t)M * 4);
    OPS_CUDA(cudaMemcpy(dx.get(), x, (size_t)K * 4, cudaMemcpyHostToDevice));
    MVParams p{};
    p.x = dx.as<float>(); p.norm_mode = NORM_NONE; p.K = K; p.act = act_format_for(type); p.nseg = 2;
    p.seg[0].w = w1; p.seg[0].out = dg.as<float>(); p.seg[0].epi = EPI_SILU; p.seg[1].w = w3; p.seg[1].out = du.as<float>();
    run_matvec(p);
    const size_t smem = (size_t)M * 4 + 64;
    OPS_CUDA(cudaFuncSetAttribute(k_gate_dump, cudaFuncAttributeMaxDynamicSharedMemorySize, (int)std::max<size_t>(smem, 48 * 1024)));
    MVParams q{};
    q.x = dg.as<float>(); q.x2 = du.as<float>(); q.x_mode = 1; q.norm_mode = NORM_NONE; q.K = M;
    k_gate_dump<<<1, MV_THREADS, smem>>>(q, dy.as<float>());
    OPS_CUDA(cudaGetLastError());
    OPS_CUDA(cudaMemcpy(out, dy.get(), (size_t)M * 4, cudaMemcpyDeviceToHost));
  });
}

int ctb_matvec_partition(const int* types, const int* rows, int nseg, int K, int n_sm, int* first_tile, int* meta) {
  if (nseg < 1 || nseg > MV_MAX_SEG || K <= 0 || K % 256 != 0 || n_sm < 1) return -1;
  MVParams p{};
  p.K = K; p.nseg = nseg; p.act = ACT_Q8_K;
  for (int s = 0; s < nseg; s++) {
    if (!type_is_kquant(types[s]) || rows[s] < 1) return -1;
    p.seg[s].w.type = types[s]; p.seg[s].w.K = K; p.seg[s].w.M = rows[s]; p.seg[s].w.nb = K / 256;
  }
  TileSpace ts;
  ts.init(p);
  const int nb = K / 256;
  long max_items = 0;
  for (int c = 0; c <= n_sm; c++) first_tile[c] = ts.boundary(c, n_sm);
  for (int c = 0; c < n_sm; c++) {
    long items = 0;
    for (int tile = first_tile[c]; tile < first_tile[c + 1]; tile++) {
      int tl = tile;
      items += st_chunks(types[ts.locate(tl)], nb);
    }
    max_items = std::max(max_items, items);
  }
  meta[0] = n_sm; meta[1] = ST_SLOT; meta[2] = ST_MAXT; meta[3] = ts.ntiles; meta[4] = ST_W; meta[5] = ST_ROWS; meta[6] = (int)max_items;
  meta[7] = st_chunk_blocks(GT_Q4_K) | (st_chunk_blocks(GT_Q5_K) << 8) | (st_chunk_blocks(GT_Q6_K) << 16) | (st_chunk_blocks(GT_Q3_K) << 24);
  return 0;
}

int ctb_get_row(int type, const void* table_blocks, int K, int n_rows, int row, float* out) {
  return guarded("ctb_get_row", [&] {
    const size_t rb = raw_row_bytes(type, K);
    DevMem dt(rb * n_rows), dtok(4), dout((size_t)K * 4);
    OPS_CUDA(cudaMemcpy(dt.get(), table_blocks, rb * n_rows, cudaMemcpyHostToDevice));
    OPS_CUDA(cudaMemcpy(dtok.get(), &row, 4, cudaMemcpyHostToDevice));
    EmbedParams em{};
    em.table = dt.as<uint8_t>(); em.row_bytes = rb; em.tokens = dtok.as<int>(); em.out = dout.as<float>(); em.type = type; em.K = K; em.n_vocab = n_rows;
    k_embed<<<1, 256>>>(em);
    OPS_CUDA(cudaGetLastError());
    OPS_CUDA(cudaMemcpy(out, dout.get(), (size_t)K * 4, cudaMemcpyDeviceToHost));
  });
}

int ctb_argmax_path(int path, const float* logits, int n, int* out) {
  return guarded("ctb_argmax_path", [&] {
    if (path < 0 || path > 1) throw std::runtime_error("unknown argmax path " + std::to_string(path));
    if (n < 1) throw std::runtime_error("no logits");
    DevMem dlog((size_t)n * 4);
    OPS_CUDA(cudaMemcpy(dlog.get(), logits, (size_t)n * 4, cudaMemcpyHostToDevice));
    if (path == 0) {
      argmax_on_device(dlog.as<float>(), n, out);
      return;
    }
    const int step = out[2];
    if (step < 0 || step >= (1 << 20)) throw std::runtime_error("step out of range");
    DevMem dstate(5 * 4), dtok((size_t)(step + 1) * 4);
    OPS_CUDA(cudaMemcpy(dstate.get(), out, 5 * 4, cudaMemcpyHostToDevice));
    OPS_CUDA(cudaMemset(dtok.get(), 0xff, (size_t)(step + 1) * 4));
    Phase ph{};
    ph.kind = PH_PICK;
    ph.pk.logits = dlog.as<float>(); ph.pk.state = dstate.as<int>(); ph.pk.out_tokens = dtok.as<int>(); ph.pk.n = n;
    run_phases({ph});
    OPS_CUDA(cudaMemcpy(out, dstate.get(), 5 * 4, cudaMemcpyDeviceToHost));
    OPS_CUDA(cudaMemcpy(out + 5, dtok.as<int>() + step, 4, cudaMemcpyDeviceToHost));
  });
}

int ctb_sample_topk(const float* logits, int n, const int* last_tokens, int n_last, float repetition_penalty, int k, int* ids, float* lg) {
  int count = -1;
  const int rc = guarded("ctb_sample_topk", [&] {
    if (n < 1 || !sg_accepts(n_last, k)) throw std::runtime_error("n < 1, or a window or k the device sampler does not take");
    DevMem dlog((size_t)n * 4);
    OPS_CUDA(cudaMemcpy(dlog.get(), logits, (size_t)n * 4, cudaMemcpyHostToDevice));
    const SampleGpuOut o = topk_on_device(dlog.as<float>(), n, last_tokens, n_last, repetition_penalty, k);
    if (o.nan) { count = -2; return; }
    count = o.count;
    for (int i = 0; i < std::min(o.count, SG_MAX_OUT); i++) { ids[i] = o.id[i]; lg[i] = o.logit[i]; }
  });
  return rc == 0 ? count : -1;
}

int ctb_sample_device(const float* logits, int n, const int* last_tokens, int n_last, int top_k, float top_p, float temperature,
                      float repetition_penalty, int seed, int* used_device) {
  int tok = -1;
  const int rc = guarded("ctb_sample_device", [&] {
    if (n < 1) throw std::runtime_error("no logits");
    if (seed < 0) seed = (int)time(nullptr);
    std::mt19937 rng((unsigned)seed);
    DevMem dlog((size_t)n * 4);
    OPS_CUDA(cudaMemcpy(dlog.get(), logits, (size_t)n * 4, cudaMemcpyHostToDevice));
    bool dev = false;
    tok = sample_lazy(
        n, last_tokens, n_last, top_k, top_p, temperature, repetition_penalty, rng, dev,
        [&] {
          int pk[2];
          argmax_on_device(dlog.as<float>(), n, pk);
          return pk[1] == 1 ? pk[0] : -1;
        },
        [&](const int* last, int nl, float pen, int k, int* i, float* l) {
          if (!sg_accepts(nl, k)) return -1;
          return sg_take(topk_on_device(dlog.as<float>(), n, last, nl, pen, k), i, l);
        },
        [&] { return std::vector<float>(logits, logits + n); });
    *used_device = dev ? 1 : 0;
  });
  return rc == 0 ? tok : -1;
}

int ctb_sample_topk_rows(const float* logits, int n_rows, int n, const int* last_off, const int* last_tokens, const float* repetition_penalty,
                         const int* k, int* count, int* ids, float* lg) {
  return guarded("ctb_sample_topk_rows", [&] {
    check_rows(n_rows, n, last_off, last_tokens);
// ... 65 lines not shown
```

ctransformers_b200/csrc/stream.cuh:

```cuda
#pragma once
#include "matvec.cuh"

namespace ctb {

#ifndef CTB_ST_WARPS
#define CTB_ST_WARPS 10
#endif
constexpr int ST_W = CTB_ST_WARPS;
constexpr int ST_NT = ST_W * 32;
constexpr int ST_THREADS = ST_NT + 32;
constexpr int ST_SLOT = 9216;
#ifndef CTB_ST_DEPTH
#define CTB_ST_DEPTH 2
#endif
constexpr int ST_MAX_DEPTH = CTB_ST_DEPTH;
constexpr int ST_MAX_SLOTS = ST_W * ST_MAX_DEPTH;
constexpr int ST_MAXT = 16;
constexpr int ST_ROWS = 16;
constexpr int ST_BAR = 1;
constexpr int ST_STATE = 6;

#ifndef CTB_CHUNK_Q3
#define CTB_CHUNK_Q3 5
#endif
#ifndef CTB_CHUNK_Q4
#define CTB_CHUNK_Q4 4
#endif
#ifndef CTB_CHUNK_Q5
#define CTB_CHUNK_Q5 3
#endif
#ifndef CTB_CHUNK_Q6
#define CTB_CHUNK_Q6 2
#endif
struct StType { int rb, kb, nm; };
template <bool Q3 = true>
__host__ __device__ constexpr StType st_type(int type) {
  return Q3 && type == GT_Q3_K ? StType{110, CTB_CHUNK_Q3, 0}
                               : (type == GT_Q4_K ? StType{144, CTB_CHUNK_Q4, 2} : (type == GT_Q5_K ? StType{176, CTB_CHUNK_Q5, 1} : StType{210, CTB_CHUNK_Q6, 0}));
}
template <int TYPE> struct StTraits {
  static constexpr int KB = st_type(TYPE).kb, BB = ST_ROWS * st_type(TYPE).rb, NM = st_type(TYPE).nm;
  static_assert(KB * BB <= ST_SLOT, "a work item must fit one ring slot");
};
__host__ __device__ inline int st_row_block_bytes(int type) { return st_type(type).rb; }
template <bool Q3 = true>
__host__ __device__ inline int st_block_bytes(int type) { return ST_ROWS * st_type<Q3>(type).rb; }
template <bool Q3 = true>
__host__ __device__ inline int st_chunk_blocks(int type) { return st_type<Q3>(type).kb; }
template <bool Q3 = true>
__host__ __device__ inline int st_tile_cost(int type) { return st_type<Q3>(type).rb / 2; }
template <bool Q3 = true>
__host__ __device__ inline int st_chunks(int type, int nb) {
  constexpr int K3 = StTraits<GT_Q3_K>::KB, K4 = StTraits<GT_Q4_K>::KB, K5 = StTraits<GT_Q5_K>::KB, K6 = StTraits<GT_Q6_K>::KB;
  if (Q3 && type == GT_Q3_K) return (nb + K3 - 1) / K3;
  return type == GT_Q4_K ? (nb + K4 - 1) / K4 : (type == GT_Q5_K ? (nb + K5 - 1) / K5 : (nb + K6 - 1) / K6);
}
__host__ __device__ inline size_t st_matrix_bytes(int type, int M, int nb) { return (size_t)((M + ST_ROWS - 1) / ST_ROWS) * nb * st_block_bytes(type); }

__device__ __forceinline__ void st_decode(int type, int o, int& rl, int& src) {
  if (type == GT_Q3_K) {
    if (o < 1536) {
      const bool qs = o < 1024;
      const int r = qs ? o : o - 1024, q = qs ? r >> 3 : r >> 2, hr = q >> 5, lane = q & 31, h = hr >> 1, rr = hr & 1, g = lane >> 2, t = lane & 3;
      rl = rr * 8 + g;
      src = (qs ? 32 + ((r >> 2) & 1) * 32 : 0) + 4 * (t + 4 * h) + (r & 3);
      return;
    }
    if (o < 1728) { const int r = o - 1536; rl = r / 12; src = 96 + r % 12; return; }
    rl = (o - 1728) >> 1; src = 108; return;
  }
  const int q4 = (type == GT_Q6_K) ? 0 : (type == GT_Q5_K ? 48 : 16);
  if (o < 2048) {
    const int q = o >> 4, hr = q >> 5, lane = q & 31, h = hr >> 1, rr = hr & 1, g = lane >> 2, t = lane & 3, l = t + 4 * h;
    const int wi = (o >> 2) & 3, byte = o & 3;
    rl = rr * 8 + g;
    src = type == GT_Q6_K ? ((wi >> 1) * 64 + (wi & 1) * 32 + 4 * l + byte) : (q4 + 32 * wi + 4 * l + byte);
    return;
  }
  if (type == GT_Q4_K) { const int r = o - 2048; rl = r >> 4; src = r & 15; return; }
  if (type == GT_Q5_K) {
    if (o < 2560) {
      const int q = (o - 2048) >> 2, hr = q >> 5, lane = q & 31, h = hr >> 1, rr = hr & 1, g = lane >> 2, t = lane & 3;
      rl = rr * 8 + g; src = 16 + 4 * (t + 4 * h) + (o & 3);
// ... 532 lines not shown
    for (int i0 = 0; i0 < g.n_k; i0 += step) {
      const int i = i0 + lane;
      if (lane < step && i < g.n_k) {
        const uint32_t n = seq + (uint32_t)i;
        const RingPos rp = st_ring(n, S);
        const int rows = min(g.rpi, g.pos - i * g.rpi);
        mbar_wait(&empty_bar[rp.slot], rp.parity ^ 1u, W_FREE_K_SLOT, (int)n);
        mbar_expect_tx(&full_bar[rp.slot], (uint32_t)(rows * row_bytes));
        bulk_g2s(ring + (size_t)rp.slot * ST_SLOT, p.kc + k_row<GEN>(kvh, i * g.rpi, p.n_ctx, p.hd), (uint32_t)(rows * row_bytes), &full_bar[rp.slot]);
      }
      __syncwarp();
    }
    seq += (uint32_t)g.n_k;
    const int n_v = attn_ring_nv<GEN>(g, p.hd, cg), ch_g = GEN ? attn_group_ch(p.hd, cg) : ATTN_CH;
    for (int iv = lane; iv < n_v; iv += 32) {
      const uint32_t n = seq + (uint32_t)iv;
      const RingPos rp = st_ring(n, S);
      const int nch = min(g.cv, ch_g - iv * g.cv);
      const uint32_t bytes = (uint32_t)(g.nchv * 512);
      mbar_wait(&empty_bar[rp.slot], rp.parity ^ 1u, W_FREE_V_SLOT, (int)n);
      mbar_expect_tx(&full_bar[rp.slot], bytes * nch);
      for (int q = 0; q < nch; q++)
        bulk_g2s(ring + (size_t)rp.slot * ST_SLOT + (size_t)q * bytes, p.vc + v_chan(kvh, cg * ATTN_CH + iv * g.cv + q, p.n_ctx, p.hd), bytes,
                 &full_bar[rp.slot]);
    }
    __syncwarp();
    seq += (uint32_t)n_v;
  }
}

template <bool GEN>
__device__ __forceinline__ void st_attn_task(const AttnParams& p, uint8_t* smem, const uint8_t* ring, uint64_t* full_bar, uint64_t* empty_bar, uint32_t S, uint32_t seq0,
                                             const AttnRing& g, int h, int cg, float* red_f, double* red_d) {
  const int warp = threadIdx.x >> 5, lane = threadIdx.x & 31, nch = GEN ? attn_group_ch(p.hd, cg) : ATTN_CH;
  const AttnScratch s = attn_scratch<GEN>(smem, p.n_ctx, p.hd, true);
  attn_stage<ST_NT, GEN>(p, s, 0, h, cg, g.pos, attn_cs0<ST_NT>(p, g.pos));
  bar_sync<ST_BAR, ST_NT>();
  for (int i = (int)(((uint32_t)warp + ST_W - seq0 % ST_W) % ST_W); i < g.n_k; i += ST_W) {
    const uint32_t n = seq0 + (uint32_t)i;
    const RingPos rp = st_ring(n, S);
    const int r0 = i * g.rpi;
    mbar_wait(&full_bar[rp.slot], rp.parity, W_K_ITEM, (int)n);
    attn_scores<GEN>(p.hd, (const uint16_t*)(ring + (size_t)rp.slot * ST_SLOT), min(g.rpi, g.pos - r0), 0, 8, s.q16, p.kq_scale, s.sc + r0);
    __syncwarp();
    if (lane == 0) mbar_arrive(&empty_bar[rp.slot]);
  }
  if (warp == (int)((seq0 + (uint32_t)g.n_k) % ST_W)) attn_scores<GEN>(p.hd, s.k16, 1, 0, 8, s.q16, p.kq_scale, s.sc + g.pos);
  bar_sync<ST_BAR, ST_NT>();
  attn_softmax<ST_NT, ST_BAR>(s.sc, s.p16, g.T, p.exp_tab, red_f, red_d);
  for (int cc = warp; cc < nch; cc += ST_W) {
    const int c = cg * ATTN_CH + cc;
    const uint32_t n = seq0 + (uint32_t)(g.n_k + cc / g.cv);
    const RingPos rp = st_ring(n, S);
    mbar_wait(&full_bar[rp.slot], rp.parity, W_V_ITEM, (int)n);
    const uint16_t* vrow = (const uint16_t*)(ring + (size_t)rp.slot * ST_SLOT + (size_t)(cc % g.cv) * g.nchv * 512);
    const float o = attn_vp(vrow, s.p16, g, g.pos, s.v16[c]);
    if (lane == 0) p.out[(size_t)h * p.hd + c] = o;
  }
  bar_sync<ST_BAR, ST_NT>();
  if ((int)threadIdx.x < attn_ring_nv<GEN>(g, p.hd, cg)) {
    const uint32_t n = seq0 + (uint32_t)(g.n_k + threadIdx.x);
    mbar_arrive(&empty_bar[st_ring(n, S).slot]);
  }
}

template <bool GEN>
__device__ __forceinline__ void st_attn_phase(const Phase& ph, uint8_t* act_smem, uint8_t* ring, uint64_t* full_bar, uint64_t* empty_bar, int n_slots,
                                              uint32_t& seq, float* pick_v, double* red) {
  const int n_cg = GEN ? attn_groups(ph.at.hd) : ph.at.hd / ATTN_CH, n_tasks = ph.at.n_head * n_cg, G = (int)gridDim.x;
  if (ph.q6) {
    const AttnRing ag = attn_ring_geom<GEN>(ph.at);
    for (int task = blockIdx.x; task < n_tasks; task += G) {
      if (task != (int)blockIdx.x) bar_sync<ST_BAR, ST_NT>();
      if (ag.T > 0) st_attn_task<GEN>(ph.at, act_smem, ring, full_bar, empty_bar, (uint32_t)(n_slots / ST_W), seq, ag, task / n_cg, task % n_cg, pick_v, red);
      seq += (uint32_t)(ag.n_k + attn_ring_nv<GEN>(ag, ph.at.hd, task % n_cg));
    }
  } else {
    for (int task = blockIdx.x; task < n_tasks; task += G) {
      if (task != (int)blockIdx.x) bar_sync<ST_BAR, ST_NT>();
      attn_body<ST_NT, ST_BAR, false, GEN>(ph.at, act_smem, task / n_cg, 0, task % n_cg, ph.at.state);
    }
  }
}
template <bool Q3>
static __device__ __noinline__ uint32_t st_attn_phase_gen(const Phase& ph, uint8_t* act_smem, uint8_t* ring, uint64_t* full_bar, uint64_t* empty_bar, int n_slots,
                                                   uint32_t seq, float* pick_v, double* red) {
  st_attn_phase<true>(ph, act_smem, ring, full_bar, empty_bar, n_slots, seq, pick_v, red);
  return seq;
}

template <bool XC, bool GEN, bool Q3>
__device__ __forceinline__ void st_producer(const StepArgs& args, uint8_t* ring, uint64_t* full_bar, uint64_t* empty_bar) {
  const int lane = threadIdx.x & 31;
  const uint32_t S = (uint32_t)(args.n_slots / ST_W);
  const uint64_t weight_pol = l2_policy_evict_first();
  uint32_t seq = 0;
  for (int ip = 0; ip < args.n_phases; ip++) {
    const Phase* ph = args.prog + ip;
    if (ph->kind == PH_ATTN) {
      if (ph->q6) {
        if (GEN) st_attn_produce<true>(ph->at, ring, full_bar, empty_bar, S, seq);
        else st_attn_produce<false>(ph->at, ring, full_bar, empty_bar, S, seq);
      }
      continue;
    }
    if (ph->kind != PH_MATVEC) continue;
    const MVParams& p = ph->mv;
    TileSpace ts;
    ts.init<Q3>(p);
    const int* bnd = args.bounds + (size_t)ip * (gridDim.x + 1) + blockIdx.x;
    const int T0 = __ldg(bnd), T1 = __ldg(bnd + 1);
    const int nb = p.K >> 8;
    for (int w0 = T0; w0 < T1; w0 += ST_MAXT) {
      const int ntw = min(ST_MAXT, T1 - w0);
      const TileInfo ti = tile_info<Q3>(ts, p, w0 + lane, nb, lane < ntw);
      for (int kc = 0;; kc++) {
        const unsigned mask = __ballot_sync(0xffffffffu, kc < ti.nch);
        if (!mask) break;
        const int rank = __popc(mask & ((1u << lane) - 1u)), cnt = __popc(mask);
        for (int base = 0; base < cnt; base += ST_W * (int)S) {
          if (((mask >> lane) & 1u) && rank >= base && rank < base + ST_W * (int)S) {
            const uint32_t n = seq + (uint32_t)rank;
            const RingPos rp = st_ring(n, S);
            const StItem it = st_item<Q3>(p, ti.seg, ti.type, ti.til, kc, nb);
            mbar_wait(&empty_bar[rp.slot], rp.parity ^ 1u, W_FREE_WEIGHT_SLOT, (int)n);
            mbar_expect_tx(&full_bar[rp.slot], it.bytes);
            bulk_g2s_hint(ring + (size_t)rp.slot * ST_SLOT, it.src, it.bytes, &full_bar[rp.slot], weight_pol);
          }
          __syncwarp();
        }
        __syncwarp();
        seq += (uint32_t)__popc(mask);
      }
    }
  }
}

template <bool XC, bool Q3>
__device__ __forceinline__ void st_matvec_phase(const Phase& ph, const NormPre& np, uint8_t* ring, uint8_t* act_smem, double* red, uint64_t* full_bar, uint64_t* empty_bar,
                                                float (*mailbox)[ST_STATE * 32], int* flags, uint32_t S, uint32_t& seq, const int* tb, unsigned long long* tr,
                                                unsigned xc_base) {
  const MVParams& p = ph.mv;
  const int warp = threadIdx.x >> 5, lane = threadIdx.x & 31;
  const unsigned epoch = XC ? xc_base + (unsigned)ph.xc.index + 1u : 0u;
  stage_activation<ST_NT, ST_BAR, XC>(p, np, ACT_Q8_K, act_smem, red, blockIdx.x == 0, epoch);
  StAct a = st_act_extras<ST_NT, ST_BAR>(act_smem, p.K, ph.q6 != 0);
  a.xc = XC && ph.xc.role == 2 ? &ph.xc : nullptr;
  a.epoch = epoch;
  if (tr && threadIdx.x == 0) tr[1] = globaltimer_ns();
  bool first_item = tr != nullptr && threadIdx.x == 0;
  TileSpace ts;
  ts.init<Q3>(p);
  const int nb = p.K >> 8;
  const int T0 = tb[0], T1 = tb[1];
#pragma unroll 1
  for (int w0 = T0; w0 < T1; w0 += ST_MAXT) {
    if (w0 != T0) {
      bar_sync<ST_BAR, ST_NT>();
      if (threadIdx.x < ST_MAXT) flags[threadIdx.x] = 0;
      bar_sync<ST_BAR, ST_NT>();
    }
    const int ntw = min(ST_MAXT, T1 - w0);
    const TileInfo ti = tile_info<Q3>(ts, p, w0 + lane, nb, lane < ntw);
#pragma unroll 1
    for (int kc = 0;; kc++) {
      const unsigned mask = __ballot_sync(0xffffffffu, kc < ti.nch);
      if (!mask) break;
      const int cnt = __popc(mask);
#pragma unroll 1
      for (int r = (int)(((uint32_t)warp + ST_W - seq % ST_W) % ST_W); r < cnt; r += ST_W) {
        unsigned mr = mask;
        for (int q = 0; q < r; q++) mr &= mr - 1;
        const int j = __ffs(mr) - 1;
        const int seg = __shfl_sync(0xffffffffu, ti.seg, j), til = __shfl_sync(0xffffffffu, ti.til, j), type = __shfl_sync(0xffffffffu, ti.type, j);
        const int nch = __shfl_sync(0xffffffffu, ti.nch, j);
        const uint32_t n = seq + (uint32_t)r;
        const RingPos rp = st_ring(n, S);
        const int kb = st_chunk_blocks<Q3>(type);
        const int b0 = kc * kb, nblk = min(kb, nb - b0);
        const MVSeg& sg = p.seg[seg];
        const uint8_t* sp = ring + (size_t)rp.slot * ST_SLOT;
        mbar_wait(&full_bar[rp.slot], rp.parity, W_WEIGHT_ITEM, (int)n);
        if (first_item) { tr[2] = globaltimer_ns(); first_item = false; }
        volatile float* mail = mailbox[j];
        volatile int* flag = flags + j;
        const bool last = kc == nch - 1;
        if (type == GT_Q4_K) run_item<GT_Q4_K, XC>(sp, &empty_bar[rp.slot], nblk, b0, kc, last, a, lane, mail, flag, sg, p, til * ST_ROWS);
        else if (type == GT_Q6_K) run_item<GT_Q6_K, XC>(sp, &empty_bar[rp.slot], nblk, b0, kc, last, a, lane, mail, flag, sg, p, til * ST_ROWS);
        else if (Q3 && type == GT_Q3_K) run_item<GT_Q3_K, XC>(sp, &empty_bar[rp.slot], nblk, b0, kc, last, a, lane, mail, flag, sg, p, til * ST_ROWS);
        else run_item<GT_Q5_K, XC>(sp, &empty_bar[rp.slot], nblk, b0, kc, last, a, lane, mail, flag, sg, p, til * ST_ROWS);
      }
      seq += (uint32_t)cnt;
    }
  }
}

__device__ __forceinline__ void st_pick_phase(const PickParams& pk, float* bv, int* bi) {
  float best;
  int idx;
  block_argmax<ST_NT, ST_BAR, true>(pk.logits, pk.n, bv, bi, best, idx);
  if (threadIdx.x == 0) {
    pk.state[4] = idx;
    advance_state(pk.state, pk.out_tokens, idx);
  }
}

__device__ __forceinline__ void grid_rearm(unsigned* sync, bool set_xc = false, unsigned xc = 0) {
  if (threadIdx.x == 0) {
    __threadfence();
    if (atomicAdd(sync + 1, 1u) == gridDim.x - 1) {
      sync[0] = 0u;
      sync[1] = 0u;
      if (set_xc) sync[2] = xc;
      __threadfence();
    }
  }
}

template <bool XC, bool GEN, bool Q3>
static __global__ void __launch_bounds__(ST_THREADS, 1) k_step(const __grid_constant__ StepArgs args) {
  extern __shared__ __align__(16) uint8_t smem[];
  __shared__ __align__(8) uint64_t full_bar[ST_MAX_SLOTS];
  __shared__ __align__(8) uint64_t empty_bar[ST_MAX_SLOTS];
  __shared__ double red[3 * ST_W];
  __shared__ __align__(16) float mailbox[ST_MAXT][ST_STATE * 32];
  __shared__ int flags[ST_MAXT];
  __shared__ float pick_v[ST_W];
  __shared__ int pick_i[ST_W];
  __shared__ __align__(16) Phase ph_s[2];
  __shared__ int tb_s[2][2];
  const int warp = threadIdx.x >> 5;
  uint8_t* ring = smem;
  uint8_t* act_smem = smem + (size_t)args.n_slots * ST_SLOT;
  ring_init(full_bar, empty_bar, args.n_slots, 1);
  pdl_trigger();
  pdl_wait();
  if (warp == ST_W) {
    st_producer<XC, GEN, Q3>(args, ring, full_bar, empty_bar);
    return;
  }
  const unsigned G = gridDim.x;
  uint32_t seq = 0;
  const unsigned xc_base = XC ? ld_relaxed_u32(args.sync + 2) : 0u;
  unsigned xc_done = 0;
  auto fetch_phase = [&](int ip) {
    if (ip >= args.n_phases) return;
    const uint4* src = (const uint4*)(args.prog + ip);
    const uint32_t dst = st_smem(&ph_s[ip & 1]);
    const int i = (int)threadIdx.x - 32;
    if (i >= 0 && i < (int)(sizeof(Phase) / 16)) asm volatile("cp.async.ca.shared.global [%0], [%1], 16;" ::"r"(dst + i * 16), "l"(src + i) : "memory");
    if (i >= 64 && i < 66)
      asm volatile("cp.async.ca.shared.global [%0], [%1], 4;" ::"r"(st_smem(&tb_s[ip & 1][i - 64])), "l"(args.bounds + (size_t)ip * (gridDim.x + 1) + blockIdx.x + (i - 64)) : "memory");
    asm volatile("cp.async.commit_group;" ::: "memory");
  };
  fetch_phase(0);
#pragma unroll 1
  for (int ip = 0; ip < args.n_phases; ip++) {
    bar_sync<ST_BAR, ST_NT>();
    unsigned long long* const tr = args.trace ? args.trace + ((size_t)ip * G + blockIdx.x) * 8 : nullptr;
    if (tr && threadIdx.x == 0) tr[4] = globaltimer_ns();
    if (threadIdx.x == 0 && ip > 0) {
      const unsigned target = (unsigned)ip * G;
      asm volatile("red.release.gpu.global.add.u32 [%0], 1;" ::"l"(args.sync) : "memory");
      if (tr) tr[5] = globaltimer_ns();
      bounded_wait([&] { return ld_relaxed_u32(args.sync) >= target; }, W_GRID_BARRIER, ip);
      if (tr) { tr[6] = globaltimer_ns(); tr[7] = tr[6]; }
    } else {
      asm volatile("cp.async.wait_all;" ::: "memory");
      if (threadIdx.x >= 32 && threadIdx.x < 32 + ST_MAXT) flags[threadIdx.x - 32] = 0;
    }
    bar_sync<ST_BAR, ST_NT>();
    const Phase& ph = ph_s[ip & 1];
    fetch_phase(ip + 1);
    NormPre np;
    if (ph.kind == PH_MATVEC) preload_norm(np, ph.mv);
    if (tr && threadIdx.x == 0) tr[0] = globaltimer_ns();
    if (XC && ph.kind == PH_MATVEC && ph.xc.role == 1) xc_done++;
    if (ph.kind == PH_MATVEC) {
      st_matvec_phase<XC, Q3>(ph, np, ring, act_smem, red, full_bar, empty_bar, mailbox, flags, (uint32_t)(args.n_slots / ST_W), seq, &tb_s[ip & 1][0], tr, xc_base);
    } else if (ph.kind == PH_ATTN) {
      if (GEN) seq = st_attn_phase_gen<Q3>(ph, act_smem, ring, full_bar, empty_bar, args.n_slots, seq, pick_v, red);
      else st_attn_phase<false>(ph, act_smem, ring, full_bar, empty_bar, args.n_slots, seq, pick_v, red);
    } else if (ph.kind == PH_EMBED) {
      if (blockIdx.x == 0) embed_row<Q3>(ph.em, ph.em.tokens[0], ph.em.out, threadIdx.x, ST_NT);
    } else if (ph.kind == PH_PICK) {
      if (blockIdx.x == 0) st_pick_phase(ph.pk, pick_v, pick_i);
    }
    if (tr) {
      bar_sync<ST_BAR, ST_NT>();
      if (threadIdx.x == 0) tr[3] = globaltimer_ns();
    }
  }
  bar_sync<ST_BAR, ST_NT>();
  grid_rearm(args.sync, XC, xc_base + xc_done);
}

struct StepLaunch { int grid; int n_slots; size_t smem; bool gen = false, q3 = false;  };

inline StepLaunch step_launch_shape(const Phase* phases, int n, int n_sm, size_t max_dyn_smem, size_t extra_act = 0) {
  size_t act = extra_act;
  for (int i = 0; i < n; i++) {
    if (phases[i].kind == PH_MATVEC) act = std::max(act, st_act_bytes(phases[i].mv.K, phases[i].q6 != 0));
    if (phases[i].kind == PH_ATTN) act = std::max(act, attn_smem_bytes(phases[i].at.n_ctx, phases[i].at.hd));
  }
  bool gen = false, q3 = false;
  for (int i = 0; i < n; i++) {
    gen |= phases[i].kind == PH_ATTN && !attn_fast_hd(phases[i].at.hd);
    if (phases[i].kind == PH_MATVEC)
      for (int s = 0; s < phases[i].mv.nseg; s++) q3 |= phases[i].mv.seg[s].w.type == GT_Q3_K;
    q3 |= phases[i].kind == PH_EMBED && phases[i].em.type == GT_Q3_K;
  }
  act = (act + 127) & ~(size_t)127;
  StepLaunch L;
  L.grid = n_sm;
  L.gen = gen;
  L.q3 = q3;
  if (act + (size_t)ST_W * ST_SLOT > max_dyn_smem) { L.n_slots = 0; L.smem = 0; return L; }
  L.n_slots = ST_W * (int)std::min<size_t>(ST_MAX_DEPTH, (max_dyn_smem - act) / ((size_t)ST_W * ST_SLOT));
  L.smem = (size_t)L.n_slots * ST_SLOT + act;
  return L;
}

inline std::vector<int> step_bounds(const Phase* phs, int n, int grid) {
  std::vector<int> b((size_t)n * (grid + 1), 0);
  for (int i = 0; i < n; i++) {
    if (phs[i].kind != PH_MATVEC) continue;
    TileSpace ts;
    ts.init(phs[i].mv);
    for (int c = 0; c <= grid; c++) b[(size_t)i * (grid + 1) + c] = ts.boundary(c, grid);
  }
  return b;
}

inline bool st_attn_ring_ok(int n_ctx, int n_slots) { return attn_ring_v(n_ctx).n_v <= n_slots; }

inline bool step_supports(const MVParams& p) {
  if (p.K % 256) return false;
  for (int s = 0; s < p.nseg; s++)
    if (!type_is_kquant(p.seg[s].w.type) || !p.seg[s].w.st) return false;
  return p.nseg >= 1;
}
inline Phase matvec_phase(const MVParams& p) {
  Phase ph{};
  ph.kind = PH_MATVEC;
  ph.mv = p;
  ph.mv.act = ACT_Q8_K;
  for (int s = 0; s < p.nseg; s++) ph.q6 |= p.seg[s].w.type == GT_Q6_K || p.seg[s].w.type == GT_Q3_K;
  return ph;
}

static inline cudaError_t st_set_debug_words(int* dev_ptr) { return cudaMemcpyToSymbol(g_st_dbg, &dev_ptr, sizeof(int*)); }
static inline cudaError_t step_set_smem_limit(size_t bytes) {
  void (*const kernels[])(StepArgs) = {k_step<false, false, false>, k_step<false, true, false>, k_step<true, false, false>,
                                        k_step<false, false, true>, k_step<false, true, true>, k_step<true, false, true>};
  for (auto k : kernels) {
    const cudaError_t e = cudaFuncSetAttribute(k, cudaFuncAttributeMaxDynamicSharedMemorySize, (int)bytes);
    if (e != cudaSuccess) return e;
  }
  return cudaSuccess;
}

static inline cudaError_t launch_step(const StepLaunch& L, cudaStream_t st, const Phase* d_prog, const int* d_bounds, int n_phases, unsigned* d_sync, bool pdl = false,
                                      unsigned long long* trace = nullptr, bool xchg = false) {
  StepArgs a;
  a.prog = d_prog; a.bounds = d_bounds; a.n_phases = n_phases; a.n_slots = L.n_slots; a.sync = d_sync; a.trace = trace;
  auto kernel = L.q3 ? (xchg ? k_step<true, false, true> : (L.gen ? k_step<false, true, true> : k_step<false, false, true>))
                     : (xchg ? k_step<true, false, false> : (L.gen ? k_step<false, true, false> : k_step<false, false, false>));
  return launch_kernel(kernel, dim3(L.grid), dim3(ST_THREADS), L.smem, st, pdl, a);
}

}
```

ctransformers_b200/lib.py:

```python
import ctypes as C
from pathlib import Path
from typing import Optional

LIB_DIR = Path(__file__).resolve().parent / "lib"
LIB_NAME = "libctransformers.so"


class ConfigStruct(C.Structure):
    _fields_ = [("context_length", C.c_int), ("gpu_layers", C.c_int), ("mmap", C.c_bool), ("mlock", C.c_bool)]


def find_library(path: Optional[str] = None) -> str:
    if path:
        return str(path)
    lib = LIB_DIR / LIB_NAME
    if not lib.is_file():
        raise OSError(
            f"{lib} has not been built. Build it with `python -m ctransformers_b200.build` "
            "(needs nvcc; compiles for sm_90a). There is no CPU fallback library."
        )
    return str(lib)


_P = C.c_void_p
_IP = C.POINTER(C.c_int)
_FP = C.POINTER(C.c_float)
_DP = C.POINTER(C.c_double)

PROTOTYPES = {
    "ctransformers_llm_create": (_P, [C.c_char_p, C.c_char_p, ConfigStruct]),
    "ctransformers_llm_delete": (None, [_P]),
    "ctransformers_llm_tokenize": (C.c_int, [_P, C.c_char_p, C.c_bool, _IP]),
    "ctransformers_llm_detokenize": (C.c_char_p, [_P, C.c_int]),
    "ctransformers_llm_is_eos_token": (C.c_bool, [_P, C.c_int]),
    "ctransformers_llm_eos_token_id": (C.c_int, [_P]),
    "ctransformers_llm_bos_token_id": (C.c_int, [_P]),
    "ctransformers_llm_vocab_size": (C.c_int, [_P]),
    "ctransformers_llm_context_length": (C.c_int, [_P]),
    "ctransformers_llm_architecture": (C.c_char_p, [_P]),
    "ctransformers_llm_batch_eval": (C.c_bool, [_P, _IP, C.c_int, C.c_int, C.c_int, C.c_int]),
    "ctransformers_llm_logits_data": (_FP, [_P]),
    "ctransformers_llm_logits_size": (C.c_int, [_P]),
    "ctransformers_llm_embeddings_data": (_FP, [_P]),
    "ctransformers_llm_embeddings_size": (C.c_int, [_P]),
    "ctransformers_llm_sample": (C.c_int, [_P, _IP, C.c_int, C.c_int, C.c_float, C.c_float, C.c_float, C.c_int]),
    "ctransformers_llm_reset": (None, [_P]),
}
EXTRA_PROTOTYPES = {
    "ctb_abi_version": (C.c_int, []),
    "ctb_llm_last_eval_ms": (C.c_double, [_P]),
    "ctb_llm_launches_per_token": (C.c_long, [_P]),
    "ctb_llm_speculative_hits": (C.c_long, [_P]),
    "ctb_llm_weight_bytes_per_token": (C.c_ulonglong, [_P]),
    "ctb_llm_trace_step": (C.c_long, [_P, C.c_int, C.c_int, C.POINTER(C.c_ulonglong), C.c_long]),
    "ctb_llm_load_ms": (C.c_double, [_P]),
    "ctb_llm_device_samples": (C.c_long, [_P]),
    "ctb_llm_set_stream": (None, [_P, C.c_void_p]),
    "ctb_tp_unique_id": (C.c_int, [_P, C.c_int]),
    "ctb_llm_create_tp": (_P, [C.c_char_p, C.c_char_p, ConfigStruct, C.c_int, C.c_int, _P]),
    "ctb_tp_shard": (C.c_int, [C.c_int, C.c_int, C.c_int, C.c_int, C.c_int, C.c_int, _IP]),
    "ctb_llm_decode_greedy": (C.c_double, [_P, C.c_int, C.c_int, C.c_int, _IP]),
    "ctb_llm_profile_step": (C.c_int, [_P, C.c_int, C.c_int, C.POINTER(C.c_double), _IP]),
    "ctb_llm_time_matvec_only": (C.c_double, [_P, C.c_int, C.POINTER(C.c_long)]),
    "ctb_llm_time_matvec_kinds": (C.c_double, [_P, C.c_int, C.POINTER(C.c_long), C.c_uint]),
    "ctb_mul_mat": (C.c_int, [C.c_int, _P, _P, _P, C.c_int, C.c_int, C.c_int]),
    "ctb_quantize_row_q8_K": (C.c_int, [_P, _P, C.c_int]),
    "ctb_quantize_row_q8_0": (C.c_int, [_P, _P, C.c_int]),
    "ctb_quantize_row_q8_1": (C.c_int, [_P, _P, C.c_int]),
    "ctb_norm": (C.c_int, [C.c_int, _P, _P, _P, _P, C.c_int, C.c_float]),
    "ctb_norm_path": (C.c_int, [C.c_int, C.c_int, _P, _P, _P, _P, C.c_int, C.c_float]),
    "ctb_rope": (C.c_int, [_P, C.c_int, C.c_int, C.c_int, C.c_int, C.c_float, C.c_float]),
    "ctb_attention": (C.c_int, [_P, _P, _P, _P, C.c_int, C.c_int, C.c_int, C.c_int, C.c_int, C.c_float]),
    "ctb_attention_path": (C.c_int, [C.c_int, _P, _P, _P, _P, _P, _P, C.c_int, C.c_int, C.c_int, C.c_int, C.c_int, C.c_int, _P, C.c_int,
                                     C.c_float, C.c_float]),
    "ctb_prefill_mul_mat": (C.c_int, [C.c_int, _P, _P, _P, C.c_int, C.c_int, _P, _P, C.c_int, _P, _P, C.c_float, _P, _P, _P, _P, C.c_int,
                                      C.c_int, _P]),
    "ctb_llm_paths": (C.c_long, [_P, _IP, C.c_int]),
    "ctb_ffn_gate": (C.c_int, [C.c_int, _P, _P, _P, _P, C.c_int, C.c_int]),
    "ctb_matvec_partition": (C.c_int, [_IP, _IP, C.c_int, C.c_int, C.c_int, _IP, _IP]),
    "ctb_get_row": (C.c_int, [C.c_int, _P, C.c_int, C.c_int, C.c_int, _P]),
    "ctb_argmax_path": (C.c_int, [C.c_int, _P, C.c_int, _IP]),
    "ctb_sample_topk": (C.c_int, [_P, C.c_int, _IP, C.c_int, C.c_float, C.c_int, _IP, _P]),
    "ctb_sample_device": (C.c_int, [_P, C.c_int, _IP, C.c_int, C.c_int, C.c_float, C.c_float, C.c_float, C.c_int, _IP]),
    "ctb_sample_topk_rows": (C.c_int, [_P, C.c_int, C.c_int, _IP, _IP, _FP, _IP, _IP, _IP, _FP]),
    "ctb_sample_device_rows": (C.c_int, [_P, C.c_int, C.c_int, _IP, _IP, _IP, _FP, _FP, _FP, _IP, _IP, _IP]),
    "ctb_vocab_load": (_P, [C.c_char_p]),
    "ctb_vocab_free": (None, [_P]),
    "ctb_vocab_size": (C.c_int, [_P]),
    "ctb_vocab_tokenize": (C.c_int, [_P, C.c_char_p, C.c_bool, _IP, C.c_int]),
    "ctb_vocab_piece": (C.c_int, [_P, C.c_int, C.c_char_p, C.c_int]),
    "ctb_sample": (C.c_int, [_FP, C.c_int, _IP, C.c_int, C.c_int, C.c_float, C.c_float, C.c_float, C.c_int]),
    "ctb_multi_create": (_P, [C.c_char_p, C.c_char_p, ConfigStruct, C.c_int]),
    "ctb_multi_delete": (None, [_P]),
    "ctb_multi_info": (C.c_int, [_P, _IP]),
    "ctb_multi_eval": (C.c_bool, [_P, C.c_int, _IP, _IP, _IP, _IP, C.c_int]),
    "ctb_multi_logits": (_FP, [_P, C.c_int]),
    "ctb_multi_embeddings": (_FP, [_P, C.c_int]),
    "ctb_multi_greedy": (C.c_int, [_P, C.c_int, _IP, _IP]),
    "ctb_multi_sample": (C.c_int, [_P, C.c_int, _IP, C.c_int, C.c_int, C.c_float, C.c_float, C.c_float, C.c_int]),
    "ctb_multi_sample_many": (C.c_int, [_P, C.c_int, _IP, _IP, _IP, _IP, _FP, _FP, _FP, _IP, _IP]),
    "ctb_multi_device_samples": (C.c_long, [_P]),
    "ctb_multi_reset": (C.c_int, [_P, C.c_int]),
    "ctb_multi_launches": (C.c_long, [_P]),
    "ctb_multi_last_eval_ms": (C.c_double, [_P]),
    "ctb_multi_pack": (C.c_int, [C.c_int, _IP, _IP, _IP, C.c_int, C.c_int, _IP, C.c_int]),
    "ctb_state_info": (C.c_int, [_P, C.c_size_t, _P]),
    "ctb_llm_state_size": (C.c_size_t, [_P, C.c_int]),
    "ctb_llm_save_state": (C.c_int, [_P, _IP, C.c_int, _P, C.c_size_t]),
    "ctb_llm_load_state": (C.c_int, [_P, _P, C.c_size_t]),
    "ctb_multi_state_size": (C.c_size_t, [_P, C.c_int]),
    "ctb_multi_save": (C.c_int, [_P, C.c_int, _IP, C.c_int, _P, C.c_size_t]),
    "ctb_multi_restore": (C.c_int, [_P, C.c_int, _P, C.c_size_t]),
    "ctb_multi_fork": (C.c_int, [_P, C.c_int, C.c_int, _IP]),
    "ctb_llm_batch_eval_rows": (C.c_int, [_P, _IP, C.c_int, C.c_int, C.c_int, _FP]),
    "ctb_llm_batch_eval_scored": (C.c_int, [_P, _IP, C.c_int, C.c_int, C.c_int, _IP, _DP, _IP]),
    "ctb_llm_score_last": (C.c_int, [_P, C.c_int, _DP, _IP]),
    "ctb_row_logprob": (C.c_int, [_P, C.c_int, C.c_int, _IP, _DP, _IP]),
    "ctb_multi_eval_rows": (C.c_int, [_P, C.c_int, _IP, _IP, _IP, _IP, C.c_int, _FP]),
    "ctb_multi_eval_scored": (C.c_int, [_P, C.c_int, _IP, _IP, _IP, _IP, C.c_int, _IP, _DP, _IP]),
    "ctb_beam_step": (C.c_int, [C.c_int, C.c_int, C.c_int, _FP, _P, _FP, C.c_int, _IP, _IP, _FP, _P]),
    "ctb_multi_reparent": (C.c_long, [_P, C.c_int, _IP, _IP, _IP, _IP]),
    "ctb_multi_beam_search": (C.c_int, [_P, C.c_int, _IP, _IP, C.c_int, C.c_int, C.c_int, _IP, _IP, _FP]),
    "ctb_multi_beam_stats": (C.c_int, [_P, _DP]),
    "ctb_grammar_parse": (_P, [C.c_char_p, C.c_char_p, C.c_int, C.POINTER(C.c_long)]),
    "ctb_grammar_free": (None, [_P]),
    "ctb_grammar_info": (C.c_int, [_P, _IP]),
    "ctb_grammar_rules": (C.c_int, [_P, _IP, C.POINTER(C.c_uint)]),
    "ctb_grammar_symbol": (C.c_int, [_P, C.c_int, C.c_char_p, C.c_int, C.POINTER(C.c_uint)]),
    "ctb_grammar_start": (_P, [_P]),
    "ctb_grammar_state_copy": (_P, [_P]),
    "ctb_grammar_state_free": (None, [_P]),
    "ctb_grammar_state_eos_ok": (C.c_int, [_P]),
    "ctb_grammar_state_stacks": (C.c_int, [_P, _IP, C.c_int, _IP]),
    "ctb_grammar_accept_piece": (C.c_int, [_P, C.c_char_p, C.c_int, C.c_int]),
    "ctb_llm_grammar_accept": (C.c_int, [_P, _P, C.c_int]),
    "ctb_multi_grammar_accept": (C.c_int, [_P, _P, C.c_int]),
    "ctb_grammar_mask_pieces": (C.c_int, [_P, C.c_int, _IP, C.c_char_p, C.c_int, _P]),
    "ctb_llm_grammar_mask": (C.c_int, [_P, _P, _P]),
    "ctb_multi_grammar_mask": (C.c_int, [_P, C.c_int, _P, _P]),
    "ctb_llm_sample_grammar": (C.c_int, [_P, _IP, C.c_int, C.c_int, C.c_float, C.c_float, C.c_float, C.c_int, _P]),
    "ctb_multi_sample_grammar_many": (C.c_int, [_P, C.c_int, _IP, _IP, _IP, _IP, _FP, _FP, _FP, _IP, C.POINTER(_P), _IP]),
    "ctb_llm_grammar_paths": (C.c_int, [_P, C.POINTER(C.c_long)]),
    "ctb_multi_grammar_paths": (C.c_int, [_P, C.POINTER(C.c_long)]),
}


class StateHeader(C.Structure):
    _fields_ = [("magic", C.c_uint32), ("version", C.c_uint32), ("n_layer", C.c_int32), ("n_head_kv", C.c_int32), ("head_dim", C.c_int32),
                ("k_stride", C.c_int32), ("n_embd", C.c_int32), ("n_vocab", C.c_int32), ("n_tokens", C.c_int32), ("has_results", C.c_int32),
                ("fingerprint", C.c_uint64)]


def load_library(path: Optional[str] = None):
    lib = C.CDLL(find_library(path))
    for table, required in ((PROTOTYPES, True), (EXTRA_PROTOTYPES, False)):
        for name, (res, args) in table.items():
            try:
                fn = getattr(lib, name)
            except AttributeError:
                if required:
                    raise OSError(f"{path or LIB_NAME} does not export '{name}'")
                continue
# ... 3 lines not shown
```

include/ctransformers_b200.h:

```cpp
#ifndef CTRANSFORMERS_B200_H_
#define CTRANSFORMERS_B200_H_

#include <stdbool.h>
#include <stddef.h>
#include <stdint.h>

#ifdef __cplusplus
extern "C" {
#endif

typedef struct LLM LLM;

typedef struct ctransformers_config {
  int context_length;
  int gpu_layers;
  bool mmap;
  bool mlock;
} ctransformers_config;

LLM* ctransformers_llm_create(const char* model_path, const char* model_type, const ctransformers_config config);
void ctransformers_llm_delete(LLM* llm);
int ctransformers_llm_tokenize(LLM* llm, const char* text, const bool add_bos_token, int* output);
const char* ctransformers_llm_detokenize(LLM* llm, const int token);
bool ctransformers_llm_is_eos_token(LLM* llm, const int token);
int ctransformers_llm_eos_token_id(LLM* llm);
int ctransformers_llm_bos_token_id(LLM* llm);
int ctransformers_llm_vocab_size(LLM* llm);
int ctransformers_llm_context_length(LLM* llm);
const char* ctransformers_llm_architecture(LLM* llm);
bool ctransformers_llm_batch_eval(LLM* llm, const int* tokens, const int n_tokens, const int n_past, const int batch_size,
                                  const int threads);
float* ctransformers_llm_logits_data(LLM* llm);
int ctransformers_llm_logits_size(LLM* llm);
const float* ctransformers_llm_embeddings_data(LLM* llm);
int ctransformers_llm_embeddings_size(LLM* llm);
int ctransformers_llm_sample(LLM* llm, const int* last_tokens, const int n_last, const int top_k, const float top_p,
                             const float temperature, const float repetition_penalty, int seed);
void ctransformers_llm_reset(LLM* llm);

int ctb_abi_version(void);
double ctb_llm_last_eval_ms(LLM* llm);
long ctb_llm_launches_per_token(LLM* llm);
long ctb_llm_speculative_hits(LLM* llm);
unsigned long long ctb_llm_weight_bytes_per_token(LLM* llm);
long ctb_llm_device_samples(LLM* llm);
double ctb_llm_load_ms(LLM* llm);
int ctb_tp_unique_id(void* out, int cap);
LLM* ctb_llm_create_tp(const char* model_path, const char* model_type, const ctransformers_config config, int rank, int world,
                       const void* unique_id);
int ctb_tp_shard(int n_embd, int n_head, int n_head_kv, int n_ff, int rank, int world, int* out6);
void ctb_llm_set_stream(LLM* llm, void* cuda_stream);
double ctb_llm_decode_greedy(LLM* llm, int first_token, int n_past, int n_steps, int* out_tokens);

int ctb_llm_profile_step(LLM* llm, int token, int n_past, double* ms_by_kind, int* count_by_kind);
long ctb_llm_trace_step(LLM* llm, int token, int n_past, unsigned long long* out, long cap_words);
double ctb_llm_time_matvec_only(LLM* llm, int reps, long* launches);
double ctb_llm_time_matvec_kinds(LLM* llm, int reps, long* launches, unsigned kind_mask);
long ctb_llm_paths(LLM* llm, int* out, int cap);

typedef struct ctb_vocab ctb_vocab;
ctb_vocab* ctb_vocab_load(const char* gguf_path);
void ctb_vocab_free(ctb_vocab* v);
int ctb_vocab_size(ctb_vocab* v);
int ctb_vocab_tokenize(ctb_vocab* v, const char* text, bool add_bos, int* out, int cap);
int ctb_vocab_piece(ctb_vocab* v, int token, char* buf, int cap);
int ctb_sample(const float* logits, int n_vocab, const int* last_tokens, int n_last, int top_k, float top_p, float temperature,
               float repetition_penalty, int seed);

int ctb_mul_mat(int type, const void* w_blocks, const float* x, float* dst, int K, int M, int N);
int ctb_quantize_row_q8_K(const float* x, void* y, int k);
int ctb_quantize_row_q8_0(const float* x, void* y, int k);
int ctb_quantize_row_q8_1(const float* x, void* y, int k);
int ctb_norm(int mode, const float* x, const float* w, const float* b, float* y, int n, float eps);
int ctb_norm_path(int path, int mode, const float* x, const float* w, const float* b, float* y, int n, float eps);
int ctb_rope(float* x, int n_heads, int head_dim, int pos, int mode, float freq_base, float freq_scale);
int ctb_attention(const float* q, const uint16_t* kcache, const uint16_t* vcache, float* out, int n_head, int n_kv, int head_dim,
                  int T, int n_total, float kq_scale);
int ctb_attention_path(int path, const float* q, const float* k_new, const float* v_new, uint16_t* kcache, uint16_t* vcache,
                       float* out, int n_head, int n_kv, int head_dim, int n_ctx, int pos0, int n_tok, const int* n_total,
                       int rope_mode, float freq_base, float kq_scale);
int ctb_prefill_mul_mat(int nseg, const int* types, const void* const* w_blocks, const int* rows, int K, int n_tok, const float* x,
                        const float* x2, int norm_mode, const float* norm_w, const float* norm_b, float eps, const int* epi,
                        const float* res, const float* res2, float* out, int n_ctx, int head_dim, int* n_slots);
int ctb_ffn_gate(int type, const void* w1_blocks, const void* w3_blocks, const float* x, float* out, int K, int M);
int ctb_matvec_partition(const int* types, const int* rows, int nseg, int K, int n_sm, int* first_tile, int* meta);

int ctb_get_row(int type, const void* table_blocks, int K, int n_rows, int row, float* out);

int ctb_argmax_path(int path, const float* logits, int n, int* out);
int ctb_sample_topk(const float* logits, int n, const int* last_tokens, int n_last, float repetition_penalty, int k, int* ids, float* lg);
int ctb_sample_device(const float* logits, int n, const int* last_tokens, int n_last, int top_k, float top_p, float temperature,
                      float repetition_penalty, int seed, int* used_device);
int ctb_sample_topk_rows(const float* logits, int n_rows, int n, const int* last_off, const int* last_tokens, const float* repetition_penalty,
                         const int* k, int* count, int* ids, float* lg);
int ctb_sample_device_rows(const float* logits, int n_rows, int n, const int* last_off, const int* last_tokens, const int* top_k, const float* top_p,
                           const float* temperature, const float* repetition_penalty, const int* seed, int* tokens, int* used_device);

typedef struct ctb_multi ctb_multi;
ctb_multi* ctb_multi_create(const char* model_path, const char* model_type, const ctransformers_config config, int n_slots);
void ctb_multi_delete(ctb_multi* m);
int ctb_multi_info(ctb_multi* m, int* out6);
bool ctb_multi_eval(ctb_multi* m, int n, const int* slots, const int* off, const int* tokens, const int* n_past, int batch_size);
const float* ctb_multi_logits(ctb_multi* m, int slot);
const float* ctb_multi_embeddings(ctb_multi* m, int slot);
int ctb_multi_greedy(ctb_multi* m, int n, const int* slots, int* out);
int ctb_multi_sample(ctb_multi* m, int slot, const int* last_tokens, int n_last, int top_k, float top_p, float temperature,
                     float repetition_penalty, int seed);
int ctb_multi_sample_many(ctb_multi* m, int n, const int* slots, const int* last_off, const int* last_tokens, const int* top_k, const float* top_p,
                          const float* temperature, const float* repetition_penalty, const int* seed, int* out);
long ctb_multi_device_samples(ctb_multi* m);
int ctb_multi_reset(ctb_multi* m, int slot);
long ctb_multi_launches(ctb_multi* m);
double ctb_multi_last_eval_ms(ctb_multi* m);
int ctb_multi_pack(int n, const int* slots, const int* off, const int* n_past, int batch_size, int n_ctx, int* out, int cap);

#define CTB_STATE_MAGIC 0x53425443u
#define CTB_STATE_VERSION 1u
typedef struct ctb_state_header {
  uint32_t magic, version;
  int32_t n_layer, n_head_kv, head_dim, k_stride, n_embd, n_vocab;
  int32_t n_tokens;
  int32_t has_results;
  uint64_t fingerprint;
} ctb_state_header;
int ctb_state_info(const void* buf, size_t size, ctb_state_header* out);
size_t ctb_llm_state_size(LLM* llm, int n_tokens);
int ctb_llm_save_state(LLM* llm, const int* tokens, int n_tokens, void* buf, size_t cap);
int ctb_llm_load_state(LLM* llm, const void* buf, size_t size);
size_t ctb_multi_state_size(ctb_multi* m, int n_tokens);
int ctb_multi_save(ctb_multi* m, int slot, const int* tokens, int n_tokens, void* buf, size_t cap);
int ctb_multi_restore(ctb_multi* m, int slot, const void* buf, size_t size);
int ctb_multi_fork(ctb_multi* m, int src, int n, const int* dsts);

int ctb_multi_beam_search(ctb_multi* m, int n_prompts, const int* prompt_off, const int* prompt_tokens, int n_beams, int n_predict, int batch_size,
                          int* out_off, int* out_tokens, float* out_p);
int ctb_multi_beam_stats(ctb_multi* m, double* out8);
int ctb_beam_step(int n_beams, int n_in, int n_next, const float* in_p, const unsigned char* in_eob, const float* rows, int n_vocab, int* out_parent,
                  int* out_token, float* out_p, unsigned char* out_eob);
long ctb_multi_reparent(ctb_multi* m, int n, const int* src, const int* dst, const int* lo, const int* hi);

int ctb_llm_batch_eval_rows(LLM* llm, const int* tokens, int n_tokens, int n_past, int batch_size, float* rows);
int ctb_llm_batch_eval_scored(LLM* llm, const int* tokens, int n_tokens, int n_past, int batch_size, const int* targets, double* logprob,
                              int* greedy);
int ctb_llm_score_last(LLM* llm, int target, double* logprob, int* greedy);
int ctb_row_logprob(const float* rows, int n_rows, int n_vocab, const int* targets, double* logprob, int* greedy);
int ctb_multi_eval_rows(ctb_multi* m, int n, const int* slots, const int* off, const int* tokens, const int* n_past, int batch_size, float* rows);
int ctb_multi_eval_scored(ctb_multi* m, int n, const int* slots, const int* off, const int* tokens, const int* n_past, int batch_size,
                          const int* targets, double* logprob, int* greedy);

typedef struct ctb_grammar ctb_grammar;
typedef struct ctb_grammar_state ctb_grammar_state;
ctb_grammar* ctb_grammar_parse(const char* text, char* err, int cap, long* err_pos);
void ctb_grammar_free(ctb_grammar* g);
int ctb_grammar_info(const ctb_grammar* g, int* out3);
int ctb_grammar_rules(const ctb_grammar* g, int* off, unsigned* elems);
int ctb_grammar_symbol(const ctb_grammar* g, int i, char* name, int cap, unsigned* id);
ctb_grammar_state* ctb_grammar_start(const ctb_grammar* g);
ctb_grammar_state* ctb_grammar_state_copy(const ctb_grammar_state* s);
void ctb_grammar_state_free(ctb_grammar_state* s);
int ctb_grammar_state_eos_ok(const ctb_grammar_state* s);
int ctb_grammar_state_stacks(const ctb_grammar_state* s, int* out, int cap, int* partial2);
int ctb_grammar_accept_piece(ctb_grammar_state* s, const char* piece, int len, int is_eos);
int ctb_llm_grammar_accept(LLM* llm, ctb_grammar_state* s, int token);
int ctb_multi_grammar_accept(ctb_multi* m, ctb_grammar_state* s, int token);
int ctb_grammar_mask_pieces(const ctb_grammar_state* s, int n_vocab, const int* off, const char* bytes, int eos, unsigned char* allowed);
int ctb_llm_grammar_mask(LLM* llm, const ctb_grammar_state* s, unsigned char* allowed);
int ctb_multi_grammar_mask(ctb_multi* m, int slot, const ctb_grammar_state* s, unsigned char* allowed);
int ctb_llm_sample_grammar(LLM* llm, const int* last_tokens, int n_last, int top_k, float top_p, float temperature, float repetition_penalty,
// ... 12 lines not shown
```

Measured before the change: 364.4.

## Pair step-kernel CTAs into 2-CTA clusters sharing activation staging via DSMEM

Launches the persistent step kernel as clusters of two CTAs. Each CTA normalizes and quantizes half of the input vector to q8_K and writes the result into both its own and its peer's shared memory, with norm statistics reduced across the pair through DSMEM and an mbarrier. This halves the per-CTA staging work that every CTA previously repeated over the full activation row before each matvec phase. In exchange it adds cluster barriers on each phase and constrains scheduling; pairing is used only when occupancy allows every cluster to be resident.

New measurement: 376.9 (median of 6 runs). +3.4%, better.

```diff
diff --git a/ctransformers_b200/csrc/device_types.cuh b/ctransformers_b200/csrc/device_types.cuh
--- a/ctransformers_b200/csrc/device_types.cuh
+++ b/ctransformers_b200/csrc/device_types.cuh
@@ -37,14 +37,26 @@
 __device__ __forceinline__ void pdl_wait() { asm volatile("griddepcontrol.wait;" ::: "memory"); }
 
 template <typename... KArgs, typename... Args>
-static inline cudaError_t launch_kernel(void (*kernel)(KArgs...), dim3 grid, dim3 block, size_t smem, cudaStream_t st, bool pdl, Args&&... args) {
+static inline cudaError_t launch_kernel_cluster(void (*kernel)(KArgs...), dim3 grid, dim3 block, size_t smem, cudaStream_t st, bool pdl, unsigned cluster,
+                                                Args&&... args) {
   cudaLaunchConfig_t cfg{};
   cfg.gridDim = grid; cfg.blockDim = block; cfg.dynamicSmemBytes = smem; cfg.stream = st;
-  cudaLaunchAttribute at[1];
-  at[0].id = cudaLaunchAttributeProgrammaticStreamSerialization;
-  at[0].val.programmaticStreamSerializationAllowed = 1;
-  cfg.attrs = at; cfg.numAttrs = pdl ? 1 : 0;
+  cudaLaunchAttribute at[2];
+  unsigned n = 0;
+  if (pdl) {
+    at[n].id = cudaLaunchAttributeProgrammaticStreamSerialization;
+    at[n++].val.programmaticStreamSerializationAllowed = 1;
+  }
+  if (cluster > 1) {
+    at[n].id = cudaLaunchAttributeClusterDimension;
+    at[n].val.clusterDim.x = cluster; at[n].val.clusterDim.y = 1; at[n++].val.clusterDim.z = 1;
+  }
+  cfg.attrs = at; cfg.numAttrs = n;
   return cudaLaunchKernelEx(&cfg, kernel, std::forward<Args>(args)...);
+}
+template <typename... KArgs, typename... Args>
+static inline cudaError_t launch_kernel(void (*kernel)(KArgs...), dim3 grid, dim3 block, size_t smem, cudaStream_t st, bool pdl, Args&&... args) {
+  return launch_kernel_cluster(kernel, grid, block, smem, st, pdl, 1u, std::forward<Args>(args)...);
 }
 
 template <typename Kernel>
diff --git a/ctransformers_b200/csrc/engine.cu b/ctransformers_b200/csrc/engine.cu
--- a/ctransformers_b200/csrc/engine.cu
+++ b/ctransformers_b200/csrc/engine.cu
@@ -634,7 +634,7 @@
   for (const StepOp& op : ops_) any_stream |= op.ph.kind == PH_MATVEC && op.stream;
   std::vector<Phase> phs;
   for (const StepOp& op : ops_) if (op.ph.kind != PH_XCHG && (op.ph.kind != PH_MATVEC || op.stream)) phs.push_back(op.ph);
-  const StepLaunch sl = step_launch_shape(phs.data(), (int)phs.size(), sm_count_, max_dyn_smem(k_step<true, false, false>));
+  const StepLaunch sl = step_launch_plan(phs.data(), (int)phs.size(), sm_count_);
   step_grid_ = sl.grid; step_slots_ = sl.n_slots; step_smem_ = sl.smem; step_q3_ = sl.q3;
   if (const char* e = getenv("CTB_ST_SLOTS")) {
     const int want = atoi(e);
@@ -643,8 +643,14 @@
   ring_attn_ = st_attn_ring_ok(hp_.n_ctx, step_slots_) && !getenv("CTB_NO_RING_ATTN");
   for (StepOp& op : ops_) if (op.ph.kind == PH_ATTN) op.ph.q6 = ring_attn_ ? 1 : 0;
   if (any_stream && step_slots_ < ST_W) throw std::runtime_error("model rows are too long for the step kernel's shared memory");
-  if (any_stream) CTB_CUDA(step_set_smem_limit(step_smem_));
-  else fused_ = false;
+  if (any_stream) {
+    CTB_CUDA(step_set_smem_limit(step_smem_));
+    StepLaunch pl = sl;
+    pl.n_slots = step_slots_; pl.smem = step_smem_;
+    step_pair_ = step_pair_choose(pl, phs.data(), (int)phs.size());
+  } else {
+    fused_ = false;
+  }
   d_prog_ = (Phase*)alloc((ops_.size() + 1) * sizeof(Phase), 256);
   d_prog_mv_ = (Phase*)alloc((ops_.size() + 1) * sizeof(Phase), 256);
   d_bounds_ = (int*)alloc((ops_.size() + 1) * (size_t)(sm_count_ + 1) * 4, 256);
@@ -677,6 +683,7 @@
   StepLaunch step_shape_;
   step_shape_.grid = step_grid_; step_shape_.n_slots = step_slots_; step_shape_.smem = step_smem_; step_shape_.gen = !attn_fast_hd(hp_.head_dim());
   step_shape_.q3 = step_q3_;
+  step_shape_.pair = step_pair_;
   auto capable = [&](const StepOp& op) { return op.ph.kind != PH_XCHG && (op.ph.kind != PH_MATVEC || op.stream); };
   int i = 0;
   while (i < n) {
@@ -791,7 +798,7 @@
   const DevMem buf((size_t)n * step_grid_ * 64);
   CTB_CUDA(cudaMemset(buf.get(), 0, (size_t)n * step_grid_ * 64));
   StepLaunch L;
-  L.grid = step_grid_; L.n_slots = step_slots_; L.smem = step_smem_; L.gen = !attn_fast_hd(hp_.head_dim()); L.q3 = step_q3_;
+  L.grid = step_grid_; L.n_slots = step_slots_; L.smem = step_smem_; L.gen = !attn_fast_hd(hp_.head_dim()); L.q3 = step_q3_; L.pair = step_pair_;
   for (int rep = 0; rep < 3; rep++) {
     put_step(token, n_past, n_past + 1);
     CTB_CUDA(launch_step(L, stream_, d_prog_, d_bounds_, n, d_sync_, false, buf.as<unsigned long long>()));
diff --git a/ctransformers_b200/csrc/engine.cuh b/ctransformers_b200/csrc/engine.cuh
--- a/ctransformers_b200/csrc/engine.cuh
+++ b/ctransformers_b200/csrc/engine.cuh
@@ -89,6 +89,7 @@
   size_t kv_reparent(const std::vector<KvCopy>& copies);
   const float* multi_rows(int slot0, int n);
   int paths(int* out, int cap);
+  int step_cluster() const { return step_pair_ ? 2 : 1; }
 
   float* logits() { host_views(); return h_logits_.as<float>(); }
   float* embeddings() { host_views(); return h_embd_.as<float>(); }
@@ -169,6 +170,7 @@
   size_t step_smem_ = 0;
   bool fused_ = true;
   bool step_q3_ = false;
+  bool step_pair_ = false;
   bool ring_attn_ = false;
   void build_ops();
   void push_matvec(struct MVParams& p, int kind);
diff --git a/ctransformers_b200/csrc/llm_abi.cu b/ctransformers_b200/csrc/llm_abi.cu
--- a/ctransformers_b200/csrc/llm_abi.cu
+++ b/ctransformers_b200/csrc/llm_abi.cu
@@ -443,6 +443,8 @@
     return -100;
   }
 }
+
+int ctb_llm_step_cluster(LLM* llm) { return llm->engine->step_cluster(); }
 
 double ctb_llm_time_matvec_only(LLM* llm, int reps, long* launches) { return ctb_llm_time_matvec_kinds(llm, reps, launches, 0); }
 
diff --git a/ctransformers_b200/csrc/matvec.cuh b/ctransformers_b200/csrc/matvec.cuh
--- a/ctransformers_b200/csrc/matvec.cuh
+++ b/ctransformers_b200/csrc/matvec.cuh
@@ -23,12 +23,13 @@
 #endif
 enum WaitCode : int {
   W_GRID_BARRIER = 1, W_FOLD_FLAG, W_FREE_WEIGHT_SLOT, W_WEIGHT_ITEM, W_FREE_K_SLOT, W_FREE_V_SLOT, W_K_ITEM, W_V_ITEM, W_XCHG,
-  W_PF_GRID_BARRIER, W_PF_FREE_SLOT, W_PF_WEIGHT_ITEM, W_CODES
+  W_PF_GRID_BARRIER, W_PF_FREE_SLOT, W_PF_WEIGHT_ITEM, W_PAIR, W_CODES
 };
 constexpr const char* WAIT_TEXT[] = {"?", "grid barrier (aux = phase)", "fold hand-off flag (aux = chunk)", "producer: free weight slot (aux = item)",
                                      "consumer: weight item (aux = item)", "producer: free K slot (attention)", "producer: free V slot (attention)",
                                      "consumer: K item (attention)", "consumer: V item (attention)", "tensor-parallel exchange: a peer's element (aux = exchange number)",
-                                     "prefill grid barrier (aux = phase)", "prefill producer: free slot (aux = item)", "prefill consumer: weight item (aux = item)"};
+                                     "prefill grid barrier (aux = phase)", "prefill producer: free slot (aux = item)", "prefill consumer: weight item (aux = item)",
+                                     "cluster peer: its half of the staged input (aux = exchange round)"};
 static_assert(sizeof(WAIT_TEXT) / sizeof(WAIT_TEXT[0]) == W_CODES, "one text per wait code");
 
 static __device__ int* g_st_dbg = nullptr;
@@ -193,10 +194,76 @@
 }
 
 struct NormPre { float w0[16], bias0[16]; };
-__device__ __forceinline__ void preload_norm(NormPre& np, const MVParams& p) {
-  const int t = threadIdx.x;
-  if (p.norm_mode != NORM_NONE && p.norm_w) load16(p.norm_w + t * 16, p.K - t * 16, np.w0);
-  if (p.norm_mode != NORM_NONE && p.norm_b) load16(p.norm_b + t * 16, p.K - t * 16, np.bias0);
+__device__ __forceinline__ void preload_norm(NormPre& np, const MVParams& p, int lo = 0) {
+  const int t = lo + (int)threadIdx.x * 16;
+  if (p.norm_mode != NORM_NONE && p.norm_w) load16(p.norm_w + t, p.K - t, np.w0);
+  if (p.norm_mode != NORM_NONE && p.norm_b) load16(p.norm_b + t, p.K - t, np.bias0);
+}
+
+__device__ __forceinline__ uint32_t cluster_ctarank() {
+  uint32_t r;
+  asm volatile("mov.u32 %0, %%cluster_ctarank;" : "=r"(r));
+  return r;
+}
+__device__ __forceinline__ uint32_t dsmem_map(const void* p, uint32_t rank) {
+  uint32_t a;
+  asm volatile("mapa.shared::cluster.u32 %0, %1, %2;" : "=r"(a) : "r"((uint32_t)__cvta_generic_to_shared(p)), "r"(rank));
+  return a;
+}
+__device__ __forceinline__ void dsmem_st_u32(uint32_t a, uint32_t v) { asm volatile("st.shared::cluster.u32 [%0], %1;" ::"r"(a), "r"(v) : "memory"); }
+__device__ __forceinline__ void dsmem_st_u16(uint32_t a, uint16_t v) { asm volatile("st.shared::cluster.u16 [%0], %1;" ::"r"(a), "h"(v) : "memory"); }
+__device__ __forceinline__ void dsmem_st_f64(uint32_t a, double v) { asm volatile("st.shared::cluster.f64 [%0], %1;" ::"r"(a), "d"(v) : "memory"); }
+
+struct PairX {
+  uint64_t* bar;
+  double* red;
+  uint32_t rank;
+  uint32_t round;
+};
+__host__ __device__ inline int pair_block0(int nb, int rank) { return rank <= 0 ? 0 : (rank == 1 ? (nb + 1) / 2 : nb); }
+
+template <int NT, int BAR>
+__device__ __forceinline__ void pair_round(PairX& px) {
+  bar_sync<BAR, NT>();
+  uint64_t* bar = px.bar + (px.round & 1u);
+  if (threadIdx.x == 0) asm volatile("mbarrier.arrive.release.cluster.shared::cluster.b64 _, [%0];" ::"r"(dsmem_map(bar, px.rank ^ 1u)) : "memory");
+  const uint32_t addr = (uint32_t)__cvta_generic_to_shared(bar), parity = (px.round >> 1) & 1u;
+  bounded_wait([&] {
+    uint32_t ok;
+    asm volatile("{\n .reg .pred p;\n mbarrier.try_wait.parity.acquire.cluster.shared::cta.b64 p, [%1], %2;\n selp.u32 %0, 1, 0, p;\n}"
+                 : "=r"(ok) : "r"(addr), "r"(parity) : "memory");
+    return ok != 0;
+  }, W_PAIR, (int)px.round);
+  px.round++;
+}
+
+template <int NT, int BAR>
+__device__ __forceinline__ void pair_sum2_max_f64(double& s, double& a, double& g, bool a_is_s, PairX& px) {
+  constexpr int NW = NT / 32;
+#pragma unroll
+  for (int o = 16; o > 0; o >>= 1) {
+    s += __shfl_xor_sync(0xffffffffu, s, o);
+    if (!a_is_s) {
+      a += __shfl_xor_sync(0xffffffffu, a, o);
+      g = fmax(g, __shfl_xor_sync(0xffffffffu, g, o));
+    }
+  }
+  double* buf = px.red + (px.round & 1u) * (2 * 3 * NW);
+  if ((threadIdx.x & 31) == 0) {
+    const int w = threadIdx.x >> 5;
+    double* mine = buf + px.rank * (3 * NW);
+    mine[w] = s; mine[NW + w] = a; mine[2 * NW + w] = g;
+    const uint32_t peer = dsmem_map(mine, px.rank ^ 1u);
+    dsmem_st_f64(peer + 8 * w, s); dsmem_st_f64(peer + 8 * (NW + w), a); dsmem_st_f64(peer + 8 * (2 * NW + w), g);
+  }
+  pair_round<NT, BAR>(px);
+  s = 0.0;
+  a = 0.0;
+#pragma unroll
+  for (int r = 0; r < 2; r++)
+#pragma unroll
+    for (int w = 0; w < NW; w++) { s += buf[r * 3 * NW + w]; a += buf[r * 3 * NW + NW + w]; g = fmax(g, buf[r * 3 * NW + 2 * NW + w]); }
+  if (a_is_s) a = s;
 }
 
 __device__ __forceinline__ unsigned min_exp(unsigned emin, float t) {
@@ -227,11 +294,12 @@
   return seq;
 }
 
-template <int NT, int BAR, bool XC>
+template <int NT, int BAR, bool XC, bool PAIR = false>
 __device__ __forceinline__ float norm_stat(double s, double a, double g, bool a_is_s, int kind, float mean, const MVParams& xs, double* red,
-                                           unsigned epoch) {
+                                           unsigned epoch, PairX* px = nullptr) {
   const int K = xs.K;
-  if (a_is_s) a = s = block_sum_f64<NT, BAR>(s, red);
+  if constexpr (PAIR) pair_sum2_max_f64<NT, BAR>(s, a, g, a_is_s, *px);
+  else if (a_is_s) a = s = block_sum_f64<NT, BAR>(s, red);
   else block_sum2_max_f64<NT, BAR>(s, a, g, red);
   if (!isfinite(s) || (!a_is_s && __dmul_ru(a, g) < 0x1p52)) return (float)(s / (double)K);
   const double e = __dmul_ru(a, (double)K * 0x1.0000001p-52);
@@ -242,6 +310,68 @@
   if (threadIdx.x == 0) red[0] = seq;
   bar_sync<BAR, NT>();
   return (float)(red[0] / (double)K);
+}
+
+__device__ __forceinline__ void norm_apply16(float (&v)[16], const float (&w)[16], const float (&bb)[16], int norm_mode, float mean, float scale, bool has_w,
+                                             bool has_b) {
+#pragma unroll
+  for (int e = 0; e < 16; e++) {
+    float y = v[e];
+    if (norm_mode == NORM_LAYER) y = __fsub_rn(y, mean);
+    y = __fmul_rn(y, scale);
+    if (has_w) y = __fmul_rn(y, w[e]);
+    if (has_b) y = __fadd_rn(y, bb[e]);
+    v[e] = y;
+  }
+}
+
+template <bool PAIR = false>
+__device__ __forceinline__ void quant_q8k16(const float (&v)[16], int base, int valid, int lane, int8_t* qs, float* dd, int16_t* bs, uint32_t pqs = 0,
+                                            uint32_t pdd = 0, uint32_t pbs = 0) {
+  float amax = 0.f, mx = 0.f;
+#pragma unroll
+  for (int e = 0; e < 16; e++) { const float ax = fabsf(v[e]); if (ax > amax) { amax = ax; mx = v[e]; } }
+  float gmax = amax;
+#pragma unroll
+  for (int o = 8; o > 0; o >>= 1) gmax = fmaxf(gmax, __shfl_xor_sync(0xffffffffu, gmax, o));
+  const unsigned who = __ballot_sync(0xffffffffu, amax == gmax);
+  const int hbase = lane & 16, hl = lane & 15;
+  const unsigned mine = (who >> hbase) & 0xffffu;
+  const float maxv = __shfl_sync(0xffffffffu, mx, hbase + __ffs(mine) - 1);
+  if (valid > 0) {
+    const int b = base >> 8;
+    int q[16];
+    int sum = 0;
+    if (gmax == 0.f) {
+#pragma unroll
+      for (int e = 0; e < 16; e++) q[e] = 0;
+      if (hl == 0) {
+        dd[b] = 0.f;
+        if (PAIR) dsmem_st_u32(pdd + 4 * b, 0u);
+      }
+    } else {
+      const float iscale = __fdiv_rn(-128.f, maxv);
+#pragma unroll
+      for (int e = 0; e < 16; e++) {
+        const float val = __fmaf_rn(iscale, v[e], 12582912.f);
+        q[e] = min(127, (__float_as_int(val) & 0x007fffff) - 0x00400000);
+        sum += q[e];
+      }
+      if (hl == 0) {
+        const float d = __fdiv_rn(1.f, iscale);
+        dd[b] = d;
+        if (PAIR) dsmem_st_u32(pdd + 4 * b, __float_as_uint(d));
+      }
+    }
+    bs[b * 16 + hl] = (int16_t)sum;
+    if (PAIR) dsmem_st_u16(pbs + 2 * (b * 16 + hl), (uint16_t)(int16_t)sum);
+#pragma unroll
+    for (int j = 0; j < 4; j++) {
+      const int wi = hl * 4 + j, o = q8k_word_offset(b, wi >> 3, wi & 7);
+      *(uint32_t*)(qs + o) = pack4(q + 4 * j);
+      if (PAIR) dsmem_st_u32(pqs + o, pack4(q + 4 * j));
+    }
+  }
 }
 
 template <int NT, int BAR, bool XC = false>
@@ -325,56 +455,14 @@
         if (nw) load16(nw + base, valid, w);
         if (nb_) load16(nb_ + base, valid, bb);
       }
-#pragma unroll
-      for (int e = 0; e < 16; e++) {
-        float y = v[e];
-        if (norm_mode == NORM_LAYER) y = __fsub_rn(y, mean);
-        y = __fmul_rn(y, scale);
-        if (nw) y = __fmul_rn(y, w[e]);
-        if (nb_) y = __fadd_rn(y, bb[e]);
-        v[e] = y;
-      }
+      norm_apply16(v, w, bb, norm_mode, mean, scale, nw != nullptr, nb_ != nullptr);
     }
     if (write_norm && norm_out && valid > 0) {
 #pragma unroll
       for (int e = 0; e < 16; e++) if (e < valid) norm_out[base + e] = v[e];
     }
     if (act == ACT_Q8_K) {
-      float amax = 0.f, mx = 0.f;
-#pragma unroll
-      for (int e = 0; e < 16; e++) { const float ax = fabsf(v[e]); if (ax > amax) { amax = ax; mx = v[e]; } }
-      float gmax = amax;
-#pragma unroll
-      for (int o = 8; o > 0; o >>= 1) gmax = fmaxf(gmax, __shfl_xor_sync(0xffffffffu, gmax, o));
-      const unsigned who = __ballot_sync(0xffffffffu, amax == gmax);
-      const int hbase = lane & 16, hl = lane & 15;
-      const unsigned mine = (who >> hbase) & 0xffffu;
-      const float maxv = __shfl_sync(0xffffffffu, mx, hbase + __ffs(mine) - 1);
-      if (valid > 0) {
-        const int b = base >> 8;
-        int q[16];
-        int sum = 0;
-        if (gmax == 0.f) {
-#pragma unroll
-          for (int e = 0; e < 16; e++) q[e] = 0;
-          if (hl == 0) dd[b] = 0.f;
-        } else {
-          const float iscale = __fdiv_rn(-128.f, maxv);
-#pragma unroll
-          for (int e = 0; e < 16; e++) {
-            const float val = __fmaf_rn(iscale, v[e], 12582912.f);
-            q[e] = min(127, (__float_as_int(val) & 0x007fffff) - 0x00400000);
-            sum += q[e];
-          }
-          if (hl == 0) dd[b] = __fdiv_rn(1.f, iscale);
-        }
-        bs[b * 16 + hl] = (int16_t)sum;
-#pragma unroll
-        for (int j = 0; j < 4; j++) {
-          const int wi = hl * 4 + j;
-          *(uint32_t*)(qs + q8k_word_offset(b, wi >> 3, wi & 7)) = pack4(q + 4 * j);
-        }
-      }
+      quant_q8k16(v, base, valid, lane, qs, dd, bs);
     } else if (act == ACT_Q8_0) {
       float amax = 0.f;
 #pragma unroll
@@ -416,6 +504,73 @@
     }
   }
   bar_sync<BAR, NT>();
+}
+
+template <int NT, int BAR>
+__device__ __forceinline__ void stage_q8k_pair(const MVParams& xs, const NormPre& np, uint8_t* smem, double* red, PairX& px, bool write_norm) {
+  const int K = xs.K, nb = K >> 8, norm_mode = xs.norm_mode, t = threadIdx.x, lane = t & 31;
+  const int lo = pair_block0(nb, (int)px.rank) * 256, hi = pair_block0(nb, (int)px.rank + 1) * 256;
+  const int base[2] = {lo + t * 16, lo + (t + NT) * 16};
+  float v[2][16];
+  load16x(xs, base[0], hi - base[0], v[0]);
+  load16x(xs, base[1], hi - base[1], v[1]);
+  float mean = 0.f, scale = 1.f;
+  if (norm_mode == NORM_RMS) {
+    double ss = 0.0;
+#pragma unroll
+    for (int h = 0; h < 2; h++)
+#pragma unroll
+      for (int e = 0; e < 16; e++) ss += (double)__fmul_rn(v[h][e], v[h][e]);
+    const float m = norm_stat<NT, BAR, false, true>(ss, ss, 0.0, true, NORM_TERM_SQ, 0.f, xs, red, 0, &px);
+    scale = __fdiv_rn(1.0f, __fsqrt_rn(__fadd_rn(m, xs.eps)));
+  } else if (norm_mode == NORM_LAYER) {
+    double s1 = 0.0, a1 = 0.0;
+    unsigned emin = 255;
+#pragma unroll
+    for (int h = 0; h < 2; h++)
+#pragma unroll
+      for (int e = 0; e < 16; e++) {
+        s1 += (double)v[h][e];
+        a1 += (double)fabsf(v[h][e]);
+        emin = min_exp(emin, v[h][e]);
+      }
+    mean = norm_stat<NT, BAR, false, true>(s1, a1, lsb_inv(emin), false, NORM_TERM_X, 0.f, xs, red, 0, &px);
+    double s2 = 0.0;
+#pragma unroll
+    for (int h = 0; h < 2; h++)
+      if (base[h] < hi) {
+#pragma unroll
+        for (int e = 0; e < 16; e++) { const float d = __fsub_rn(v[h][e], mean); s2 += (double)__fmul_rn(d, d); }
+      }
+    const float var = norm_stat<NT, BAR, false, true>(s2, s2, 0.0, true, NORM_TERM_DEV, mean, xs, red, 0, &px);
+    scale = __fdiv_rn(1.0f, __fsqrt_rn(__fadd_rn(var, xs.eps)));
+  }
+  int8_t* qs = (int8_t*)smem;
+  float* dd = (float*)(smem + (((size_t)K + 15) & ~(size_t)15));
+  int16_t* bs = (int16_t*)((uint8_t*)dd + q8k_d_bytes(K));
+  const uint32_t peer = px.rank ^ 1u, pqs = dsmem_map(qs, peer), pdd = dsmem_map(dd, peer), pbs = dsmem_map(bs, peer);
+#pragma unroll
+  for (int h = 0; h < 2; h++) {
+    if (lo + (((h * NT + t) * 16) & ~511) >= hi) continue;
+    const int valid = hi - base[h];
+    if (norm_mode != NORM_NONE) {
+      float w[16], bb[16];
+      if (h == 0) {
+#pragma unroll
+        for (int e = 0; e < 16; e++) { w[e] = np.w0[e]; bb[e] = np.bias0[e]; }
+      } else {
+        if (xs.norm_w) load16(xs.norm_w + base[h], valid, w);
+        if (xs.norm_b) load16(xs.norm_b + base[h], valid, bb);
+      }
+      norm_apply16(v[h], w, bb, norm_mode, mean, scale, xs.norm_w != nullptr, xs.norm_b != nullptr);
+    }
+    if (write_norm && xs.norm_out && valid > 0) {
+#pragma unroll
+      for (int e = 0; e < 16; e++) xs.norm_out[base[h] + e] = v[h][e];
+    }
+    quant_q8k16<true>(v[h], base[h], valid, lane, qs, dd, bs, pqs, pdd, pbs);
+  }
+  pair_round<NT, BAR>(px);
 }
 
 __device__ __forceinline__ float group_hsum8(float v) {
diff --git a/ctransformers_b200/csrc/ops_abi.cu b/ctransformers_b200/csrc/ops_abi.cu
--- a/ctransformers_b200/csrc/ops_abi.cu
+++ b/ctransformers_b200/csrc/ops_abi.cu
@@ -99,14 +99,20 @@
   return d_sync;
 }
 
+StepLaunch plan_phases(const std::vector<Phase>& phs) {
+  StepLaunch L = step_launch_plan(phs.data(), (int)phs.size(), sm_count());
+  if (L.n_slots < ST_W) throw std::runtime_error("rows too long for the step kernel's shared memory");
+  OPS_CUDA(step_set_smem_limit(L.smem));
+  step_pair_choose(L, phs.data(), (int)phs.size());
+  return L;
+}
+
 void run_phases(std::vector<Phase> phs) {
   unsigned* d_sync = sync_words();
-  const StepLaunch L = step_launch_shape(phs.data(), (int)phs.size(), sm_count(), max_dyn_smem(k_step<true, false, false>));
+  const StepLaunch L = plan_phases(phs);
   const std::vector<int> hb = step_bounds(phs.data(), (int)phs.size(), L.grid);
   DevMem dbounds(hb.size() * 4);
   OPS_CUDA(cudaMemcpy(dbounds.get(), hb.data(), hb.size() * 4, cudaMemcpyHostToDevice));
-  if (L.n_slots < ST_W) throw std::runtime_error("rows too long for the step kernel's shared memory");
-  OPS_CUDA(step_set_smem_limit(L.smem));
   DevMem dprog((phs.size() + 1) * sizeof(Phase));
   OPS_CUDA(cudaMemcpy(dprog.get(), phs.data(), phs.size() * sizeof(Phase), cudaMemcpyHostToDevice));
   OPS_CUDA(launch_step(L, 0, dprog.as<Phase>(), dbounds.as<int>(), (int)phs.size(), d_sync));
@@ -352,6 +358,18 @@
     run_phases({matvec_phase(p)});
     OPS_CUDA(cudaMemcpy(y, dy.get(), (size_t)n * 4, cudaMemcpyDeviceToHost));
   });
+}
+
+int ctb_norm_path_cluster(int n) {
+  int cluster = -1;
+  const int rc = guarded("ctb_norm_path_cluster", [&] {
+    if (n < 256 || n % 256) throw std::runtime_error("the step kernel takes n a positive multiple of 256");
+    MVParams p{};
+    p.K = n; p.act = ACT_Q8_K; p.nseg = 1; p.norm_mode = NORM_RMS;
+    p.seg[0].w.type = GT_Q4_K; p.seg[0].w.K = n; p.seg[0].w.M = 16; p.seg[0].w.nb = n / 256;
+    cluster = step_paired(plan_phases({matvec_phase(p)}), false) ? 2 : 1;
+  });
+  return rc == 0 ? cluster : rc;
 }
 
 int ctb_rope(float* x, int n_heads, int head_dim, int pos, int mode, float freq_base, float freq_scale) {
@@ -457,7 +475,7 @@
       if (path == 1) {
         Phase ph{};
         ph.kind = PH_ATTN; ph.q6 = 1; ph.at = ap;
-        const StepLaunch L = step_launch_shape(&ph, 1, sm_count(), max_dyn_smem(k_step<true, false, false>));
+        const StepLaunch L = step_launch_plan(&ph, 1, sm_count());
         if (!st_attn_ring_ok(n_ctx, L.n_slots)) throw std::runtime_error("the step kernel's ring cannot carry K / V at this n_ctx");
       }
       const size_t smem = attn_smem_bytes(n_ctx, hd);
@@ -608,6 +626,15 @@
   return 0;
 }
 
+int ctb_stage_pair_split(int K, int* block0) {
+  if (K <= 0 || K % 256 != 0) return -1;
+  for (int r = 0; r < 3; r++) block0[r] = pair_block0(K / 256, r);
+  Phase ph{};
+  ph.kind = PH_MATVEC;
+  ph.mv.K = K;
+  return step_pair_fits(&ph, 1) ? 1 : 0;
+}
+
 int ctb_get_row(int type, const void* table_blocks, int K, int n_rows, int row, float* out) {
   return guarded("ctb_get_row", [&] {
     const size_t rb = raw_row_bytes(type, K);
diff --git a/ctransformers_b200/csrc/stream.cuh b/ctransformers_b200/csrc/stream.cuh
--- a/ctransformers_b200/csrc/stream.cuh
+++ b/ctransformers_b200/csrc/stream.cuh
@@ -1,4 +1,6 @@
 #pragma once
+#include <stdexcept>
+#include <string>
 #include "matvec.cuh"
 
 namespace ctb {
@@ -697,7 +699,7 @@
     }
   }
 }
-template <bool Q3>
+template <bool Q3, bool PAIR>
 static __device__ __noinline__ uint32_t st_attn_phase_gen(const Phase& ph, uint8_t* act_smem, uint8_t* ring, uint64_t* full_bar, uint64_t* empty_bar, int n_slots,
                                                    uint32_t seq, float* pick_v, double* red) {
   st_attn_phase<true>(ph, act_smem, ring, full_bar, empty_bar, n_slots, seq, pick_v, red);
@@ -751,14 +753,15 @@
   }
 }
 
-template <bool XC, bool Q3>
+template <bool XC, bool Q3, bool PAIR>
 __device__ __forceinline__ void st_matvec_phase(const Phase& ph, const NormPre& np, uint8_t* ring, uint8_t* act_smem, double* red, uint64_t* full_bar, uint64_t* empty_bar,
                                                 float (*mailbox)[ST_STATE * 32], int* flags, uint32_t S, uint32_t& seq, const int* tb, unsigned long long* tr,
-                                                unsigned xc_base) {
+                                                unsigned xc_base, PairX& px) {
   const MVParams& p = ph.mv;
   const int warp = threadIdx.x >> 5, lane = threadIdx.x & 31;
   const unsigned epoch = XC ? xc_base + (unsigned)ph.xc.index + 1u : 0u;
-  stage_activation<ST_NT, ST_BAR, XC>(p, np, ACT_Q8_K, act_smem, red, blockIdx.x == 0, epoch);
+  if constexpr (PAIR) stage_q8k_pair<ST_NT, ST_BAR>(p, np, act_smem, red, px, blockIdx.x < 2);
+  else stage_activation<ST_NT, ST_BAR, XC>(p, np, ACT_Q8_K, act_smem, red, blockIdx.x == 0, epoch);
   StAct a = st_act_extras<ST_NT, ST_BAR>(act_smem, p.K, ph.q6 != 0);
   a.xc = XC && ph.xc.role == 2 ? &ph.xc : nullptr;
   a.epoch = epoch;
@@ -832,7 +835,7 @@
   }
 }
 
-template <bool XC, bool GEN, bool Q3>
+template <bool XC, bool GEN, bool Q3, bool PAIR = false>
 static __global__ void __launch_bounds__(ST_THREADS, 1) k_step(const __grid_constant__ StepArgs args) {
   extern __shared__ __align__(16) uint8_t smem[];
   __shared__ __align__(8) uint64_t full_bar[ST_MAX_SLOTS];
@@ -844,10 +847,22 @@
   __shared__ int pick_i[ST_W];
   __shared__ __align__(16) Phase ph_s[2];
   __shared__ int tb_s[2][2];
+  __shared__ __align__(8) uint64_t pair_bar[PAIR ? 2 : 1];
+  __shared__ double pair_red[PAIR ? 2 * 2 * 3 * ST_W : 1];
   const int warp = threadIdx.x >> 5;
   uint8_t* ring = smem;
   uint8_t* act_smem = smem + (size_t)args.n_slots * ST_SLOT;
   ring_init(full_bar, empty_bar, args.n_slots, 1);
+  PairX px{pair_bar, pair_red, 0u, 0u};
+  if constexpr (PAIR) {
+    if (threadIdx.x == 0) {
+      mbar_init(&pair_bar[0], 1);
+      mbar_init(&pair_bar[1], 1);
+      asm volatile("fence.mbarrier_init.release.cluster;" ::: "memory");
+    }
+    px.rank = cluster_ctarank();
+    asm volatile("barrier.cluster.arrive.release.aligned;\n barrier.cluster.wait.acquire.aligned;" ::: "memory");
+  }
   pdl_trigger();
   pdl_wait();
   if (warp == ST_W) {
@@ -888,13 +903,14 @@
     const Phase& ph = ph_s[ip & 1];
     fetch_phase(ip + 1);
     NormPre np;
-    if (ph.kind == PH_MATVEC) preload_norm(np, ph.mv);
+    if (ph.kind == PH_MATVEC) preload_norm(np, ph.mv, PAIR ? pair_block0(ph.mv.K >> 8, (int)px.rank) * 256 : 0);
     if (tr && threadIdx.x == 0) tr[0] = globaltimer_ns();
     if (XC && ph.kind == PH_MATVEC && ph.xc.role == 1) xc_done++;
     if (ph.kind == PH_MATVEC) {
-      st_matvec_phase<XC, Q3>(ph, np, ring, act_smem, red, full_bar, empty_bar, mailbox, flags, (uint32_t)(args.n_slots / ST_W), seq, &tb_s[ip & 1][0], tr, xc_base);
+      st_matvec_phase<XC, Q3, PAIR>(ph, np, ring, act_smem, red, full_bar, empty_bar, mailbox, flags, (uint32_t)(args.n_slots / ST_W), seq, &tb_s[ip & 1][0], tr,
+                                    xc_base, px);
     } else if (ph.kind == PH_ATTN) {
-      if (GEN) seq = st_attn_phase_gen<Q3>(ph, act_smem, ring, full_bar, empty_bar, args.n_slots, seq, pick_v, red);
+      if (GEN) seq = st_attn_phase_gen<Q3, PAIR>(ph, act_smem, ring, full_bar, empty_bar, args.n_slots, seq, pick_v, red);
       else st_attn_phase<false>(ph, act_smem, ring, full_bar, empty_bar, args.n_slots, seq, pick_v, red);
     } else if (ph.kind == PH_EMBED) {
       if (blockIdx.x == 0) embed_row<Q3>(ph.em, ph.em.tokens[0], ph.em.out, threadIdx.x, ST_NT);
@@ -910,7 +926,7 @@
   grid_rearm(args.sync, XC, xc_base + xc_done);
 }
 
-struct StepLaunch { int grid; int n_slots; size_t smem; bool gen = false, q3 = false;  };
+struct StepLaunch { int grid; int n_slots; size_t smem; bool gen = false, q3 = false, pair = false;  };
 
 inline StepLaunch step_launch_shape(const Phase* phases, int n, int n_sm, size_t max_dyn_smem, size_t extra_act = 0) {
   size_t act = extra_act;
@@ -975,13 +991,59 @@
   return cudaSuccess;
 }
 
+inline bool step_paired(const StepLaunch& L, bool xchg) { return L.pair && !L.q3 && !xchg; }
+using StepKernel = void (*)(StepArgs);
+inline StepKernel step_kernel(const StepLaunch& L, bool xchg) {
+  if (xchg) return L.q3 ? k_step<true, false, true> : k_step<true, false, false>;
+  if (step_paired(L, xchg)) return L.gen ? k_step<false, true, false, true> : k_step<false, false, false, true>;
+  return L.q3 ? (L.gen ? k_step<false, true, true> : k_step<false, false, true>) : (L.gen ? k_step<false, true, false> : k_step<false, false, false>);
+}
+
+inline bool step_pair_fits(const Phase* phases, int n) {
+  for (int i = 0; i < n; i++)
+    if (phases[i].kind == PH_MATVEC && pair_block0(phases[i].mv.K >> 8, 1) * 16 > 2 * ST_NT) return false;
+  return true;
+}
+
+inline bool step_pair_wanted() {
+  const char* e = getenv("CTB_ST_CLUSTER");
+  return !(e && e[0] == '0');
+}
+
+inline StepLaunch step_launch_plan(const Phase* phases, int n, int n_sm, size_t extra_act = 0) {
+  StepLaunch L = step_launch_shape(phases, n, n_sm, max_dyn_smem(k_step<true, false, false>), extra_act);
+  if (!L.q3 && step_pair_wanted())
+    L = step_launch_shape(phases, n, n_sm, std::min(max_dyn_smem(k_step<false, false, false, true>), max_dyn_smem(k_step<false, true, false, true>)), extra_act);
+  return L;
+}
+
+inline bool step_pair_choose(StepLaunch& L, const Phase* phases, int n) {
+  L.pair = false;
+  if (!step_pair_wanted() || L.q3 || L.grid % 2 || !step_pair_fits(phases, n)) return false;
+  StepLaunch P = L;
+  P.pair = true;
+  const StepKernel k = step_kernel(P, false);
+  auto check = [](cudaError_t e) {
+    if (e != cudaSuccess) throw std::runtime_error(std::string("pairing the step kernel: ") + cudaGetErrorString(e));
+  };
+  check(cudaFuncSetAttribute(k, cudaFuncAttributeMaxDynamicSharedMemorySize, (int)L.smem));
+  cudaLaunchConfig_t cfg{};
+  cfg.gridDim = dim3(L.grid); cfg.blockDim = dim3(ST_THREADS); cfg.dynamicSmemBytes = L.smem;
+  cudaLaunchAttribute at[1];
+  at[0].id = cudaLaunchAttributeClusterDimension;
+  at[0].val.clusterDim.x = 2; at[0].val.clusterDim.y = 1; at[0].val.clusterDim.z = 1;
+  cfg.attrs = at; cfg.numAttrs = 1;
+  int clusters = 0;
+  check(cudaOccupancyMaxActiveClusters(&clusters, k, &cfg));
+  L.pair = clusters >= L.grid / 2;
+  return L.pair;
+}
+
 static inline cudaError_t launch_step(const StepLaunch& L, cudaStream_t st, const Phase* d_prog, const int* d_bounds, int n_phases, unsigned* d_sync, bool pdl = false,
                                       unsigned long long* trace = nullptr, bool xchg = false) {
   StepArgs a;
   a.prog = d_prog; a.bounds = d_bounds; a.n_phases = n_phases; a.n_slots = L.n_slots; a.sync = d_sync; a.trace = trace;
-  auto kernel = L.q3 ? (xchg ? k_step<true, false, true> : (L.gen ? k_step<false, true, true> : k_step<false, false, true>))
-                     : (xchg ? k_step<true, false, false> : (L.gen ? k_step<false, true, false> : k_step<false, false, false>));
-  return launch_kernel(kernel, dim3(L.grid), dim3(ST_THREADS), L.smem, st, pdl, a);
-}
-
-}
+  return launch_kernel_cluster(step_kernel(L, xchg), dim3(L.grid), dim3(ST_THREADS), L.smem, st, pdl, step_paired(L, xchg) ? 2u : 1u, a);
+}
+
+}
diff --git a/ctransformers_b200/lib.py b/ctransformers_b200/lib.py
--- a/ctransformers_b200/lib.py
+++ b/ctransformers_b200/lib.py
@@ -69,6 +69,7 @@
     "ctb_quantize_row_q8_1": (C.c_int, [_P, _P, C.c_int]),
     "ctb_norm": (C.c_int, [C.c_int, _P, _P, _P, _P, C.c_int, C.c_float]),
     "ctb_norm_path": (C.c_int, [C.c_int, C.c_int, _P, _P, _P, _P, C.c_int, C.c_float]),
+    "ctb_norm_path_cluster": (C.c_int, [C.c_int]),
     "ctb_rope": (C.c_int, [_P, C.c_int, C.c_int, C.c_int, C.c_int, C.c_float, C.c_float]),
     "ctb_attention": (C.c_int, [_P, _P, _P, _P, C.c_int, C.c_int, C.c_int, C.c_int, C.c_int, C.c_float]),
     "ctb_attention_path": (C.c_int, [C.c_int, _P, _P, _P, _P, _P, _P, C.c_int, C.c_int, C.c_int, C.c_int, C.c_int, C.c_int, _P, C.c_int,
@@ -76,8 +77,10 @@
     "ctb_prefill_mul_mat": (C.c_int, [C.c_int, _P, _P, _P, C.c_int, C.c_int, _P, _P, C.c_int, _P, _P, C.c_float, _P, _P, _P, _P, C.c_int,
                                       C.c_int, _P]),
     "ctb_llm_paths": (C.c_long, [_P, _IP, C.c_int]),
+    "ctb_llm_step_cluster": (C.c_int, [_P]),
     "ctb_ffn_gate": (C.c_int, [C.c_int, _P, _P, _P, _P, C.c_int, C.c_int]),
     "ctb_matvec_partition": (C.c_int, [_IP, _IP, C.c_int, C.c_int, C.c_int, _IP, _IP]),
+    "ctb_stage_pair_split": (C.c_int, [C.c_int, _IP]),
     "ctb_get_row": (C.c_int, [C.c_int, _P, C.c_int, C.c_int, C.c_int, _P]),
     "ctb_argmax_path": (C.c_int, [C.c_int, _P, C.c_int, _IP]),
     "ctb_sample_topk": (C.c_int, [_P, C.c_int, _IP, C.c_int, C.c_float, C.c_int, _IP, _P]),
diff --git a/include/ctransformers_b200.h b/include/ctransformers_b200.h
--- a/include/ctransformers_b200.h
+++ b/include/ctransformers_b200.h
@@ -57,6 +57,7 @@
 double ctb_llm_time_matvec_only(LLM* llm, int reps, long* launches);
 double ctb_llm_time_matvec_kinds(LLM* llm, int reps, long* launches, unsigned kind_mask);
 long ctb_llm_paths(LLM* llm, int* out, int cap);
+int ctb_llm_step_cluster(LLM* llm);
 
 typedef struct ctb_vocab ctb_vocab;
 ctb_vocab* ctb_vocab_load(const char* gguf_path);
@@ -73,6 +74,7 @@
 int ctb_quantize_row_q8_1(const float* x, void* y, int k);
 int ctb_norm(int mode, const float* x, const float* w, const float* b, float* y, int n, float eps);
 int ctb_norm_path(int path, int mode, const float* x, const float* w, const float* b, float* y, int n, float eps);
+int ctb_norm_path_cluster(int n);
 int ctb_rope(float* x, int n_heads, int head_dim, int pos, int mode, float freq_base, float freq_scale);
 int ctb_attention(const float* q, const uint16_t* kcache, const uint16_t* vcache, float* out, int n_head, int n_kv, int head_dim,
                   int T, int n_total, float kq_scale);
@@ -84,6 +86,7 @@
                         const float* res, const float* res2, float* out, int n_ctx, int head_dim, int* n_slots);
 int ctb_ffn_gate(int type, const void* w1_blocks, const void* w3_blocks, const float* x, float* out, int K, int M);
 int ctb_matvec_partition(const int* types, const int* rows, int nseg, int K, int n_sm, int* first_tile, int* meta);
+int ctb_stage_pair_split(int K, int* block0);
 
 int ctb_get_row(int type, const void* table_blocks, int K, int n_rows, int row, float* out);
 
```
